# ray-project/xgboost_ray

Hardware: NVIDIA H100
Metric: boosting rounds/sec (higher is better)
Workload: dtype int64 fixed-point histograms (int32 shared-memory cells), f64 gain

## Files before the change

### xgboost_ray_b200/build.py

```python
import os
import subprocess
import sys
from concurrent.futures import ThreadPoolExecutor

HERE = os.path.dirname(os.path.abspath(__file__))
CSRC = os.path.join(HERE, "csrc")
OUT = os.path.join(HERE, "libb2hist.so")
OBJ_DIR = os.path.join(CSRC, "build")

NVCC = os.environ.get("NVCC", "/usr/local/cuda/bin/nvcc")
COMMON = ["-gencode", "arch=compute_90a,code=sm_90a", "-O3", "-lineinfo", "-std=c++17",
          "-Xcompiler", "-fPIC,-ffp-contract=off", "-ccbin", "/usr/bin/g++"]
SOURCES = {
    "hist_kernel.cu": [],
    "hist_tma_kernel.cu": [],
    "split_kernel.cu": ["--fmad=false"],
    "partition_kernel.cu": ["--fmad=false"],
    "control_kernel.cu": ["--fmad=false"],
    "objective_kernel.cu": ["--fmad=false"],
    "sketch.cu": ["--fmad=false"],
    "auc_kernel.cu": ["--fmad=false"],
    "p2p_exchange.cu": [],
    "shap_kernel.cu": [],
    "engine.cu": [],
}


def _stale(target, deps):
    if not os.path.exists(target):
        return True
    t = os.path.getmtime(target)
    return any(os.path.getmtime(d) > t for d in deps)


def build(force=False, verbose=False):
    os.makedirs(OBJ_DIR, exist_ok=True)
    headers = [os.path.join(CSRC, "common.cuh"), os.path.join(CSRC, "hist_common.cuh"), os.path.join(CSRC, "sampling.cuh"), os.path.join(CSRC, "p2p.cuh"), os.path.join(HERE, "..", "include", "b2hist.h"), __file__]
    jobs = []
    objs = []
    for src, extra in SOURCES.items():
        sp = os.path.join(CSRC, src)
        op = os.path.join(OBJ_DIR, src.replace(".cu", ".o"))
        objs.append(op)
        if force or _stale(op, [sp] + headers):
            jobs.append([NVCC] + COMMON + extra + ["-c", sp, "-o", op])

    def run(cmd):
        if verbose:
            print(" ".join(cmd), flush=True)
        r = subprocess.run(cmd, capture_output=True, text=True)
        if r.returncode != 0:
            raise RuntimeError("nvcc failed:\n%s\n%s\n%s" % (" ".join(cmd), r.stdout, r.stderr))
        return r

    with ThreadPoolExecutor(max_workers=6) as ex:
        list(ex.map(run, jobs))
    if force or jobs or _stale(OUT, objs):
        run([NVCC, "-shared", "-o", OUT] + objs + ["-ldl", "-ccbin", "/usr/bin/g++"])
    return OUT


if __name__ == "__main__":
    print(build(force="--force" in sys.argv, verbose=True))
```

### xgboost_ray_b200/csrc/common.cuh

```cuda
#pragma once
#include <cuda_runtime.h>
#include <stdint.h>

#define B2_GROUP_SLOTS 32
#define B2_BINS 256
#define B2_MISSING_BIN 255
#define B2_PLANE_ELEMS (B2_BINS * B2_GROUP_SLOTS)
#define B2_GROUP_ELEMS (2 * B2_PLANE_ELEMS)

struct B2HistWork {
  int32_t seg_begin;
  int32_t seg_count;
  int32_t hist_index;
  int32_t chunk_begin;
};

#define B2_HIST_MAX_TYPES 8
struct B2HistPlan {
  int32_t n_types;
  int32_t cta_begin[B2_HIST_MAX_TYPES + 1];
  int32_t narrow_w;
};

struct B2SplitWork {
  int32_t seg_begin, seg_count;
  int32_t feature;
  int32_t split_bin;
  int32_t default_left;
  int32_t has_missing;
  int32_t chunk_begin;
  int32_t is_cat;
  uint32_t cat_bits[8];
};

struct B2SplitCand {
  float loss_chg;
  int32_t feature;
  int32_t bin;
  int32_t default_left;
  int64_t left_g, left_h;
  uint32_t order;
  int32_t is_cat;
  uint32_t cat_bits[8];
};

struct B2EvalNode {
  int64_t sum_g, sum_h;
  int32_t hist_index;
  float root_gain;
};

struct B2TreeNodeDev {
  int32_t left, right;
  int32_t feature;
  float cond;
  float value;
  int32_t default_left;
  int32_t cat_slot;
  int32_t pad;
};

#define B2_SHAP_MAX_PATH 16
#define B2_PATH_MISSING_OK 1u
#define B2_PATH_HAS_HI 2u
#define B2_PATH_OUTSIDE_OK 4u
struct B2PathElem {
  int32_t feature;
  int32_t cat_slot;
  float lo, hi;
  uint32_t flags;
  uint32_t pad;
  double zero_fraction;
};
struct B2PathInfo {
  int32_t elem_begin;
  int32_t len;
  int32_t cls;
  int32_t pad;
  double value;
};

__device__ __forceinline__ int b2_tree_step(const B2TreeNodeDev& nd, float v, float missing, int missing_is_nan,
                                            const uint32_t* __restrict__ cat_table) {
  const bool miss = isnan(v) || (!missing_is_nan && v == missing);
  if (miss) return nd.default_left ? nd.left : nd.right;
  if (nd.cat_slot >= 0) {
    bool in_set = false;
    if (v >= 0.0f && v < 256.0f) { const int c = (int)v; in_set = (cat_table[(size_t)nd.cat_slot * 8 + (c >> 5)] >> (c & 31)) & 1u; }
    return in_set ? nd.right : nd.left;
  }
  return v < nd.cond ? nd.left : nd.right;
}

__device__ __forceinline__ int b2_tree_leaf(const B2TreeNodeDev* __restrict__ tn, const float* __restrict__ x, float missing,
                                            int missing_is_nan, const uint32_t* __restrict__ cat_table, float* leaf_value) {
  int nid = 0;
  B2TreeNodeDev nd = tn[0];
  while (nd.feature >= 0) {
    nid = b2_tree_step(nd, x[nd.feature], missing, missing_is_nan, cat_table);
    nd = tn[nid];
  }
  *leaf_value = nd.value;
  return nid;
}

struct B2LevelCtl {
  int32_t n_nodes;
  int32_t n_split;
  int32_t part_chunks;
  int32_t hist_n_work;
  int32_t hist_total_chunks;
  int32_t hist_chunk_rows;
  int32_t n_pairs;
  int32_t leaf_base_next;
};
struct B2NodeSeg { int32_t nid, begin, count, buf; };
struct B2LeafDev { int32_t nid, buf, begin, count; };
struct B2SegWork {
  int32_t seg_begin, seg_count, id, chunk_begin;
  int32_t buf, pad0, pad1, pad2;
};
struct B2TreeDev {
  int32_t *left, *right, *parent, *feature, *split_bin, *default_left, *split_type;
  uint32_t* cat_bits;
  float* loss_chg;
  long long *sum_g, *sum_h;
  float *leaf_weight, *leaf_value;
  int32_t* n_nodes;
};
struct B2CtlParams { double mcw, lambda, alpha, max_delta_step; float gamma, eta; };

struct B2ColSample {
  const uint8_t* level_mask;
  const uint32_t* fwq;
  double bynode;
  int32_t n_level;
  int32_t n_features;
  uint32_t seed, tree;
};

#define B2_P2P_MAX_WORLD 8
enum { kSlotHist = 0, kSlotCand = 1, kSlotAbsmax = 2, kSlotLeaf = 3, kSlotClose = 4, kP2PSlots = 5 };
struct B2P2P {
  long long* build[B2_P2P_MAX_WORLD];
  B2SplitCand* cands[B2_P2P_MAX_WORLD];
  long long* misc[B2_P2P_MAX_WORLD];
  uint32_t* flags[B2_P2P_MAX_WORLD];
  uint32_t* epoch;
  uint32_t* done;
  uint32_t* err;
  const uint32_t* abort_flag;
  int32_t world, rank;
  int32_t cand_cap, misc_stride;
  long long spin_limit;
};

struct B2TrainParamDev {
  double min_child_weight, lambda, alpha;
  double inv_scale_g, inv_scale_h;
  double max_delta_step;
  int32_t max_cat_to_onehot, max_cat_threshold;
};

#ifdef __CUDACC__
__device__ __forceinline__ double b2_thr_l1(double g, double a) {
  if (g > a) return __dadd_rn(g, -a);
  if (g < -a) return __dadd_rn(g, a);
  return 0.0;
}
__device__ __forceinline__ double b2_calc_weight(double G, double H, double mcw, double lambda, double alpha, double mds) {
  if (H < mcw || H <= 0.0) return 0.0;
  const double t = (alpha == 0.0) ? G : b2_thr_l1(G, alpha);
  double dw = __ddiv_rn(-t, __dadd_rn(H, lambda));
  if (mds != 0.0 && fabs(dw) > mds) dw = copysign(mds, dw);
  return dw;
}
__device__ __forceinline__ double b2_calc_gain(double G, double H, double mcw, double lambda, double alpha, double mds) {
  if (H < mcw || H <= 0.0) return 0.0;
  if (mds == 0.0) {
    const double t = (alpha == 0.0) ? G : b2_thr_l1(G, alpha);
    return __ddiv_rn(__dmul_rn(t, t), __dadd_rn(H, lambda));
  }
  const double w = b2_calc_weight(G, H, mcw, lambda, alpha, mds);
  const double ret = -__dadd_rn(__dmul_rn(__dmul_rn(2.0, G), w), __dmul_rn(__dadd_rn(H, lambda), __dmul_rn(w, w)));
  return alpha == 0.0 ? ret : __dadd_rn(ret, __dmul_rn(alpha, fabs(w)));
}
#endif
```

### xgboost_ray_b200/csrc/control_kernel.cu

```cuda
#include <string.h>

#include <cub/block/block_scan.cuh>

#include "common.cuh"
#include "p2p.cuh"

namespace b2 {

constexpr int kCtlThreads = 1024;
constexpr int kPartChunkRows = 2048;
constexpr int kSplitChunkRows = 8192;

__device__ __forceinline__ double c_calc_gain(double G, double H, const B2CtlParams& p) {
  return b2_calc_gain(G, H, p.mcw, p.lambda, p.alpha, p.max_delta_step);
}
__device__ __forceinline__ float c_calc_weight(double G, double H, const B2CtlParams& p) {
  return __double2float_rn(b2_calc_weight(G, H, p.mcw, p.lambda, p.alpha, p.max_delta_step));
}

struct TileScan {
  typedef cub::BlockScan<int, kCtlThreads> Scan;
  Scan::TempStorage* tmp;
  int carry;
  __device__ TileScan(Scan::TempStorage* t) : tmp(t), carry(0) {}
  __device__ int step(int v) {
    int ex, total;
    Scan(*tmp).ExclusiveSum(v, ex, total);
    __syncthreads();
    int r = carry + ex;
    carry += total;
    return r;
  }
};

__global__ void __launch_bounds__(kCtlThreads)
decide_kernel(B2LevelCtl* __restrict__ ctl_cur, B2LevelCtl* __restrict__ ctl_nxt, const B2NodeSeg* __restrict__ seg_cur,
              B2NodeSeg* __restrict__ seg_nxt, const B2EvalNode* __restrict__ ev_cur, B2EvalNode* __restrict__ ev_nxt,
              const B2SplitCand* __restrict__ cands, int cands_per_node, int cand_ranks, int cand_rank_stride, int can_split,
              B2TreeDev tree,
              B2SplitWork* __restrict__ split_work, int32_t* __restrict__ pair_parent_hist, B2LeafDev* __restrict__ leaves,
              int32_t* __restrict__ n_leaves, const uint8_t* __restrict__ has_missing, const int32_t* __restrict__ qexp,
              int qbits, B2CtlParams p, int32_t* __restrict__ part_counters, const B2SplitCand* __restrict__ local_cands,
              int use_p2p, B2P2P pp) {
  __shared__ typename TileScan::Scan::TempStorage tmp;
  __shared__ int s_node_base, s_leaf_base;
  const int n = ctl_cur->n_nodes;
  if (part_counters) for (int i = threadIdx.x; i < 2 * n; i += kCtlThreads) part_counters[i] = 0;
  if (use_p2p && can_split) {
    constexpr int kWords = sizeof(B2SplitCand) / 8;
    static_assert(sizeof(B2SplitCand) % 8 == 0, "candidates are copied as 64-bit words");
    const uint32_t epoch = p2p_next_epoch(pp, kSlotCand);
    const int total = n * cands_per_node * kWords;
    for (int w = 0; w < pp.world; ++w) {
      long long* dst = reinterpret_cast<long long*>(pp.cands[w] + (size_t)pp.rank * pp.cand_cap);
      for (int t = threadIdx.x; t < total; t += kCtlThreads) st_volatile_u64(dst + t, reinterpret_cast<const long long*>(local_cands)[t]);
    }
    __syncthreads();
    p2p_signal(pp, kSlotCand, epoch);
    p2p_wait(pp, kSlotCand, epoch);
    p2p_finish_single(pp, kSlotCand, epoch);
  }
  const double inv_sg = ldexp(1.0, qexp[0] - qbits), inv_sh = ldexp(1.0, qexp[1] - qbits);
  if (threadIdx.x == 0) { s_node_base = *tree.n_nodes; s_leaf_base = *n_leaves; }
  __syncthreads();
  TileScan scan_split(&tmp), scan_leaf(&tmp), scan_chunks(&tmp);
  for (int base = 0; base < n; base += kCtlThreads) {
    const int i = base + threadIdx.x;
    const bool in = i < n;
    B2SplitCand best; best.feature = -1; best.loss_chg = 0.f; best.order = 0xffffffffu; best.bin = 0; best.default_left = 0;
    best.left_g = 0; best.left_h = 0; best.is_cat = 0;
    B2EvalNode nd; nd.sum_g = 0; nd.sum_h = 0; nd.hist_index = 0; nd.root_gain = 0.f;
    B2NodeSeg sg; sg.nid = 0; sg.begin = 0; sg.count = 0; sg.buf = 0;
    bool expand = false;
    if (in) {
      nd = ev_cur[i]; sg = seg_cur[i];
      if (can_split) {
        for (int w = 0; w < cand_ranks; ++w)
          for (int g = 0; g < cands_per_node; ++g) {
            B2SplitCand c;
            if (use_p2p) {
              constexpr int kW = sizeof(B2SplitCand) / 8;
              const long long* src = reinterpret_cast<const long long*>(cands + (size_t)w * cand_rank_stride + (size_t)i * cands_per_node + g);
#pragma unroll
              for (int t = 0; t < kW; ++t) reinterpret_cast<unsigned long long*>(&c)[t] = ld_volatile_u64(src + t);
            } else c = cands[(size_t)w * cand_rank_stride + (size_t)i * cands_per_node + g];
            if (c.feature < 0) continue;
            if (best.feature < 0 || c.loss_chg > best.loss_chg || (c.loss_chg == best.loss_chg && c.order < best.order)) best = c;
          }
        if (best.feature >= 0)
          expand = best.loss_chg > 1e-6f && best.left_h != 0 && (nd.sum_h - best.left_h) != 0 && !(best.loss_chg < p.gamma);
      }
    }
    const int rank = scan_split.step(expand ? 1 : 0);
    const int lrank = scan_leaf.step((in && !expand) ? 1 : 0);
    const int chunks = expand ? (sg.count + kSplitChunkRows - 1) / kSplitChunkRows : 0;
    const int chunk_begin = scan_chunks.step(chunks);
    if (in && !expand) {
      B2LeafDev lf; lf.nid = sg.nid; lf.buf = sg.buf; lf.begin = sg.begin; lf.count = sg.count;
      leaves[s_leaf_base + lrank] = lf;
    }
    if (expand) {
      const int l = s_node_base + 2 * rank, r = l + 1;
      const int nid = sg.nid;
      tree.left[nid] = l; tree.right[nid] = r; tree.feature[nid] = best.feature; tree.split_bin[nid] = best.bin;
      tree.default_left[nid] = best.default_left; tree.loss_chg[nid] = best.loss_chg;
      tree.split_type[nid] = best.is_cat;
      if (best.is_cat) {
#pragma unroll
        for (int w8 = 0; w8 < 8; ++w8) tree.cat_bits[(size_t)nid * 8 + w8] = best.cat_bits[w8];
      }
      tree.left[l] = -1; tree.right[l] = -1; tree.feature[l] = -1; tree.parent[l] = nid;
      tree.left[r] = -1; tree.right[r] = -1; tree.feature[r] = -1; tree.parent[r] = nid;
      const long long lg = best.left_g, lh = best.left_h, rg = nd.sum_g - lg, rh = nd.sum_h - lh;
      tree.sum_g[l] = lg; tree.sum_h[l] = lh; tree.sum_g[r] = rg; tree.sum_h[r] = rh;
      B2SplitWork sw;
      sw.seg_begin = sg.begin; sw.seg_count = sg.count; sw.feature = best.feature; sw.split_bin = best.bin;
      sw.default_left = best.default_left; sw.has_missing = has_missing[best.feature]; sw.chunk_begin = chunk_begin;
      sw.is_cat = best.is_cat;
#pragma unroll
      for (int w8 = 0; w8 < 8; ++w8) sw.cat_bits[w8] = best.is_cat ? best.cat_bits[w8] : 0u;
      split_work[rank] = sw;
      pair_parent_hist[rank] = nd.hist_index;
      const double GL = __dmul_rn(__ll2double_rn(lg), inv_sg), HL = __dmul_rn(__ll2double_rn(lh), inv_sh);
      const double GR = __dmul_rn(__ll2double_rn(rg), inv_sg), HR = __dmul_rn(__ll2double_rn(rh), inv_sh);
      B2EvalNode el, er;
      el.sum_g = lg; el.sum_h = lh; el.hist_index = -1; el.root_gain = __double2float_rn(c_calc_gain(GL, HL, p));
      er.sum_g = rg; er.sum_h = rh; er.hist_index = -1; er.root_gain = __double2float_rn(c_calc_gain(GR, HR, p));
      ev_nxt[2 * rank] = el; ev_nxt[2 * rank + 1] = er;
      B2NodeSeg sl, sr;
      sl.nid = l; sl.buf = sg.buf ^ 1; sl.begin = sg.begin; sl.count = 0;
      sr.nid = r; sr.buf = sg.buf ^ 1; sr.begin = sg.begin; sr.count = sg.count;
      seg_nxt[2 * rank] = sl; seg_nxt[2 * rank + 1] = sr;
    }
  }
  __syncthreads();
  if (threadIdx.x == 0) {
    const int n_split = scan_split.carry;
    ctl_cur->n_split = n_split; ctl_cur->part_chunks = scan_chunks.carry;
    ctl_cur->leaf_base_next = s_leaf_base + scan_leaf.carry;
    ctl_nxt->n_nodes = 2 * n_split; ctl_nxt->n_split = 0; ctl_nxt->part_chunks = 0;
    ctl_nxt->hist_n_work = 0; ctl_nxt->hist_total_chunks = 0; ctl_nxt->n_pairs = 0;
    *tree.n_nodes = s_node_base + 2 * n_split;
    *n_leaves = s_leaf_base + scan_leaf.carry;
  }
}

__global__ void __launch_bounds__(kCtlThreads)
finalize_level_kernel(const B2LevelCtl* __restrict__ ctl_cur, B2LevelCtl* __restrict__ ctl_nxt, B2NodeSeg* __restrict__ seg_nxt,
                      B2EvalNode* __restrict__ ev_nxt, const B2SplitWork* __restrict__ split_work,
                      const int32_t* __restrict__ counters, const int32_t* __restrict__ pair_parent_hist,
                      B2HistWork* __restrict__ hist_work, int32_t* __restrict__ triples, int max_pairs, int need_hist,
                      int n_streams, int window_rows, int chunk_rows_override, long long* __restrict__ stat_rows) {
  __shared__ typename TileScan::Scan::TempStorage tmp;
  __shared__ long long s_rows;
  __shared__ int s_chunk_rows;
  const int ns = ctl_cur->n_split;
  if (threadIdx.x == 0) s_rows = 0;
  __syncthreads();
  long long my_rows = 0;
  for (int j = threadIdx.x; j < ns; j += kCtlThreads) {
    const B2SplitWork sw = split_work[j];
    const int cl = counters[2 * j];
    B2NodeSeg sl = seg_nxt[2 * j], sr = seg_nxt[2 * j + 1];
    sl.begin = sw.seg_begin; sl.count = cl;
    sr.begin = sw.seg_begin + cl; sr.count = sw.seg_count - cl;
    seg_nxt[2 * j] = sl; seg_nxt[2 * j + 1] = sr;
    if (need_hist) {
      const bool build_left = ev_nxt[2 * j].sum_h < ev_nxt[2 * j + 1].sum_h;
      my_rows += build_left ? sl.count : sr.count;
    }
  }
  if (need_hist) {
    atomicAdd((unsigned long long*)&s_rows, (unsigned long long)my_rows);
    __syncthreads();
    if (threadIdx.x == 0) {
      int c = chunk_rows_override;
      if (c <= 0) {
        const long long per_stream = s_rows / n_streams;
        const long long target = per_stream >= 16384 ? per_stream / 4 : per_stream;
        c = 512;
        while (c < target && c < 8192) c <<= 1;
      }
      if (c > window_rows) c = window_rows;
      s_chunk_rows = c;
      if (stat_rows) *stat_rows = s_rows;
    }
    __syncthreads();
    const int chunk_rows = s_chunk_rows;
    TileScan scan(&tmp);
    for (int base = 0; base < ns; base += kCtlThreads) {
      const int j = base + threadIdx.x;
      int chunks = 0, begin = 0, count = 0;
      if (j < ns) {
        const bool build_left = ev_nxt[2 * j].sum_h < ev_nxt[2 * j + 1].sum_h;
        const int b = build_left ? 2 * j : 2 * j + 1, s = b ^ 1;
        begin = seg_nxt[b].begin; count = seg_nxt[b].count;
        chunks = (count + chunk_rows - 1) / chunk_rows;
        ev_nxt[b].hist_index = j; ev_nxt[s].hist_index = max_pairs + j;
        triples[3 * j] = pair_parent_hist[j]; triples[3 * j + 1] = j; triples[3 * j + 2] = max_pairs + j;
      }
      const int cb = scan.step(chunks);
      if (j < ns) { B2HistWork w; w.seg_begin = begin; w.seg_count = count; w.hist_index = j; w.chunk_begin = cb; hist_work[j] = w; }
    }
    __syncthreads();
    if (threadIdx.x == 0) {
      ctl_nxt->hist_n_work = ns; ctl_nxt->hist_total_chunks = scan.carry; ctl_nxt->hist_chunk_rows = chunk_rows;
      ctl_nxt->n_pairs = ns;
    }
  }
}

__global__ void __launch_bounds__(kCtlThreads)
leaf_plan_kernel(const B2LeafDev* __restrict__ leaves, const int32_t* __restrict__ n_leaves, B2SegWork* __restrict__ work,
                 B2LevelCtl* __restrict__ leaf_ctl) {
  __shared__ typename TileScan::Scan::TempStorage tmp;
  const int n = *n_leaves;
  TileScan scan(&tmp);
  for (int base = 0; base < n; base += kCtlThreads) {
    const int i = base + threadIdx.x;
    int chunks = 0; B2LeafDev lf; lf.nid = 0; lf.buf = 0; lf.begin = 0; lf.count = 0;
    if (i < n) { lf = leaves[i]; chunks = (lf.count + kPartChunkRows - 1) / kPartChunkRows; }
    const int cb = scan.step(chunks);
    if (i < n) {
      B2SegWork w; w.seg_begin = lf.begin; w.seg_count = lf.count; w.id = i; w.chunk_begin = cb; w.buf = lf.buf;
      w.pad0 = lf.nid == 0 ? 1 : 0;
      w.pad1 = w.pad2 = 0; work[i] = w;
    }
  }
  __syncthreads();
  if (threadIdx.x == 0) { leaf_ctl->hist_n_work = n; leaf_ctl->hist_total_chunks = scan.carry; }
}

__global__ void leaf_values_kernel(const B2LeafDev* __restrict__ leaves, const int32_t* __restrict__ n_leaves,
                                   const long long* __restrict__ sums, const int32_t* __restrict__ qexp, int leaf_bits,
                                   B2CtlParams p, float* __restrict__ leaf_value, B2TreeDev tree) {
  const int n = *n_leaves;
  const double kg = ldexp(1.0, leaf_bits - qexp[0]), kh = ldexp(1.0, leaf_bits - qexp[1]);
  for (int i = blockIdx.x * blockDim.x + threadIdx.x; i < n; i += gridDim.x * blockDim.x) {
    const double G = __ddiv_rn(__ll2double_rn(sums[2 * i]), kg), H = __ddiv_rn(__ll2double_rn(sums[2 * i + 1]), kh);
    const float w = c_calc_weight(G, H, p);
    const float v = __fmul_rn(w, p.eta);
    leaf_value[i] = v;
    tree.leaf_weight[leaves[i].nid] = w;
    tree.leaf_value[leaves[i].nid] = v;
  }
}

__global__ void tree_init_kernel(B2TreeDev tree, B2LevelCtl* ctl0, B2NodeSeg* seg0, B2EvalNode* ev0, int32_t* n_leaves,
                                 int n_rows, B2HistWork* hist_work0) {
  if (threadIdx.x == 0 && blockIdx.x == 0) {
    B2HistWork hw; hw.seg_begin = 0; hw.seg_count = n_rows; hw.hist_index = 0; hw.chunk_begin = 0; hist_work0[0] = hw;
    ctl0->leaf_base_next = 0;
    *tree.n_nodes = 1; *n_leaves = 0;
    tree.left[0] = -1; tree.right[0] = -1; tree.parent[0] = -1; tree.feature[0] = -1;
    ctl0->n_nodes = 1; ctl0->n_split = 0; ctl0->part_chunks = 0; ctl0->hist_n_work = 0; ctl0->hist_total_chunks = 0;
    ctl0->n_pairs = 0;
    B2NodeSeg s; s.nid = 0; s.buf = 0; s.begin = 0; s.count = n_rows; seg0[0] = s;
    B2EvalNode e; e.sum_g = 0; e.sum_h = 0; e.hist_index = 0; e.root_gain = 0.f; ev0[0] = e;
  }
}
__global__ void root_record_kernel(B2TreeDev tree, const B2EvalNode* ev0) {
  if (threadIdx.x == 0 && blockIdx.x == 0) { tree.sum_g[0] = ev0[0].sum_g; tree.sum_h[0] = ev0[0].sum_h; }
}

}

extern "C" {
int b2_launch_decide(B2LevelCtl* ctl_cur, B2LevelCtl* ctl_nxt, const B2NodeSeg* seg_cur, B2NodeSeg* seg_nxt,
                     const B2EvalNode* ev_cur, B2EvalNode* ev_nxt, const B2SplitCand* cands, int cands_per_node, int cand_ranks,
                     int cand_rank_stride, int can_split, B2TreeDev tree, B2SplitWork* split_work, int32_t* pair_parent_hist, B2LeafDev* leaves, int32_t* n_leaves,
                     const uint8_t* has_missing, const int32_t* qexp, int qbits, B2CtlParams p, int32_t* part_counters,
                     const B2SplitCand* local_cands, const void* p2p, cudaStream_t s) {
  B2P2P pp;
  if (p2p) pp = *reinterpret_cast<const B2P2P*>(p2p); else memset(&pp, 0, sizeof(pp));
  b2::decide_kernel<<<1, b2::kCtlThreads, 0, s>>>(ctl_cur, ctl_nxt, seg_cur, seg_nxt, ev_cur, ev_nxt, cands, cands_per_node,
                                                 cand_ranks, cand_rank_stride, can_split, tree, split_work, pair_parent_hist, leaves, n_leaves, has_missing, qexp, qbits, p,
                                                 part_counters, local_cands, p2p ? 1 : 0, pp);
  return (int)cudaGetLastError();
}
int b2_launch_finalize_level(const B2LevelCtl* ctl_cur, B2LevelCtl* ctl_nxt, B2NodeSeg* seg_nxt, B2EvalNode* ev_nxt,
                             const B2SplitWork* split_work, const int32_t* counters, const int32_t* pair_parent_hist,
                             B2HistWork* hist_work, int32_t* triples, int max_pairs, int need_hist, int n_streams,
                             int window_rows, int chunk_rows_override, long long* stat_rows, cudaStream_t s) {
  b2::finalize_level_kernel<<<1, b2::kCtlThreads, 0, s>>>(ctl_cur, ctl_nxt, seg_nxt, ev_nxt, split_work, counters,
                                                         pair_parent_hist, hist_work, triples, max_pairs, need_hist, n_streams,
                                                         window_rows, chunk_rows_override, stat_rows);
  return (int)cudaGetLastError();
}
int b2_launch_leaf_plan(const B2LeafDev* leaves, const int32_t* n_leaves, B2SegWork* work, B2LevelCtl* leaf_ctl, cudaStream_t s) {
  b2::leaf_plan_kernel<<<1, b2::kCtlThreads, 0, s>>>(leaves, n_leaves, work, leaf_ctl);
  return (int)cudaGetLastError();
}
int b2_launch_leaf_values(const B2LeafDev* leaves, const int32_t* n_leaves, const long long* sums, const int32_t* qexp,
                          int leaf_bits, B2CtlParams p, float* leaf_value, B2TreeDev tree, cudaStream_t s) {
  b2::leaf_values_kernel<<<8, 256, 0, s>>>(leaves, n_leaves, sums, qexp, leaf_bits, p, leaf_value, tree);
  return (int)cudaGetLastError();
}
int b2_launch_tree_init(B2TreeDev tree, B2LevelCtl* ctl0, B2NodeSeg* seg0, B2EvalNode* ev0, int32_t* n_leaves, int n_rows,
                        B2HistWork* hist_work0, cudaStream_t s) {
  b2::tree_init_kernel<<<1, 32, 0, s>>>(tree, ctl0, seg0, ev0, n_leaves, n_rows, hist_work0);
  return (int)cudaGetLastError();
}
int b2_launch_root_record(B2TreeDev tree, const B2EvalNode* ev0, cudaStream_t s) {
  b2::root_record_kernel<<<1, 32, 0, s>>>(tree, ev0);
  return (int)cudaGetLastError();
}
}
```

### xgboost_ray_b200/csrc/engine.cu

```cuda
#include <cuda_runtime.h>
#include <dlfcn.h>
#include <errno.h>
#include <sys/types.h>
#include <sys/uio.h>
#include <math.h>
#include <stdarg.h>
#include <stdio.h>
#include <stdlib.h>
#include <string.h>

#include <algorithm>
#include <atomic>
#include <chrono>
#include <map>
#include <mutex>
#include <set>
#include <string>
#include <thread>
#include <vector>

#include "../../include/b2hist.h"
#include "common.cuh"
#include "sampling.cuh"

extern "C" {
int b2_launch_hist(const uint8_t*, int, const int2*, const int32_t*, const B2HistWork*, int, int, int, int, int, long long*,
                   const B2LevelCtl*, int, int, int, int, cudaStream_t);
int b2_make_bins_tensor_map(void*, const uint8_t*, int64_t, int, int);
int b2_launch_hist_tma(const uint8_t*, int, const void*, const int2*, const int32_t*, const B2HistWork*, int, int, int, int, int, long long*,
                       const B2LevelCtl*, int, int, int64_t, int, cudaStream_t);
int b2_launch_hist_subtract(const long long*, long long*, const int32_t*, int, int64_t, const B2LevelCtl*, cudaStream_t);
int b2_launch_eval_splits(const long long*, int, const B2EvalNode*, int, const int32_t*, const int32_t*, const int32_t*,
                          const uint8_t*, const uint8_t*, const int32_t*, int, B2TrainParamDev, B2SplitCand*, int, const B2LevelCtl*,
                          int, int, B2ColSample, const B2NodeSeg*, cudaStream_t);
int b2_launch_subsample(float2*, int64_t, uint32_t, uint32_t, uint32_t, double, int, cudaStream_t);
int b2_p2p_flag_words(int);
int b2_launch_p2p_reduce_subtract(const void*, const long long*, long long*, const int32_t*, const B2LevelCtl*, int, int, int64_t, int,
                                  cudaStream_t);
int b2_launch_p2p_quant_exponent(const void*, const uint32_t*, int32_t*, cudaStream_t);
int b2_launch_p2p_leaf_sums(const void*, const int32_t*, long long*, cudaStream_t);
int b2_hist_variant();
int b2_launch_p2p_close(const void*, cudaStream_t);
int b2_launch_gather_interleaved_rows(const void*, float*, int, cudaStream_t);
int b2_launch_final_assign(const uint8_t*, int64_t, const int32_t*, const B2SplitWork*, const B2LevelCtl*, int, const float2*,
                           const int32_t*, int, long long*, uint16_t*, int, int, cudaStream_t);
int b2_launch_margin_update(float*, int, int, const uint16_t*, const float*, int64_t, int, cudaStream_t);
int b2_gradient_fused_max_classes();
int b2_launch_sum_fixed(const float2*, int64_t, const int32_t*, int, long long*, int, cudaStream_t);
int b2_cat_ctas();
int b2_launch_eval_cat_splits(const long long*, int, const B2EvalNode*, int, const int32_t*, int, const int32_t*, const int32_t*,
                              const int32_t*, int, B2TrainParamDev, B2SplitCand*, int, int, const B2LevelCtl*, int, int,
                              B2ColSample, const B2NodeSeg*, cudaStream_t);
int b2_launch_cat_stats(const float*, int64_t, int, float, const int32_t*, int, int32_t*, int, cudaStream_t);
int b2_launch_root_totals(const long long*, int, B2EvalNode*, const int32_t*, int, B2TrainParamDev, int, cudaStream_t);
int b2_part_chunk_rows();
int b2_split_chunk_rows();
int b2_launch_partition(const uint8_t*, int64_t, const int32_t*, int32_t*, const B2SplitWork*, const B2LevelCtl*, int, int32_t*,
                        int, int, cudaStream_t);
int b2_launch_leaf_sums(const float2*, const int32_t*, const int32_t*, const void*, const B2LevelCtl*, int, const int32_t*, int,
                        long long*, uint16_t*, int, cudaStream_t);
int b2_launch_pred_update(float*, int, int, const int32_t*, const int32_t*, const void*, const B2LevelCtl*, int, const float*, int,
                          cudaStream_t);
int b2_launch_decide(B2LevelCtl*, B2LevelCtl*, const B2NodeSeg*, B2NodeSeg*, const B2EvalNode*, B2EvalNode*, const B2SplitCand*,
                     int, int, int, int, B2TreeDev, B2SplitWork*, int32_t*, B2LeafDev*, int32_t*, const uint8_t*, const int32_t*, int,
                     B2CtlParams, int32_t*, const B2SplitCand*, const void*, cudaStream_t);
int b2_launch_finalize_level(const B2LevelCtl*, B2LevelCtl*, B2NodeSeg*, B2EvalNode*, const B2SplitWork*, const int32_t*,
                             const int32_t*, B2HistWork*, int32_t*, int, int, int, int, int, long long*, cudaStream_t);
int b2_launch_leaf_plan(const B2LeafDev*, const int32_t*, B2SegWork*, B2LevelCtl*, cudaStream_t);
int b2_launch_leaf_values(const B2LeafDev*, const int32_t*, const long long*, const int32_t*, int, B2CtlParams, float*, B2TreeDev,
                          cudaStream_t);
int b2_launch_tree_init(B2TreeDev, B2LevelCtl*, B2NodeSeg*, B2EvalNode*, int32_t*, int, B2HistWork*, cudaStream_t);
int b2_launch_root_record(B2TreeDev, const B2EvalNode*, cudaStream_t);
int b2_launch_iota(int32_t*, int64_t, cudaStream_t);
int b2_launch_gradient(int, int, const float*, const float*, const float*, int64_t, float, float, float2*, uint32_t*, uint32_t*, int,
                       cudaStream_t);
int b2_launch_label_check(int, const float*, int64_t, uint32_t*, int, cudaStream_t);
int b2_launch_pack_custom(const float*, const float*, int, int64_t, float2*, int, cudaStream_t);
int b2_launch_absmax(const float2*, int64_t, uint32_t*, int, cudaStream_t);
int b2_launch_quant_exponent(const uint32_t*, int32_t*, cudaStream_t);
int b2_launch_quantize(const float2*, int64_t, const int32_t*, int, int2*, int, cudaStream_t);
int b2_launch_metric(int, int, int, float, const float*, const float*, const float*, int64_t, double*, int, cudaStream_t);
int b2_launch_predict(const float*, int64_t, int, float, const B2TreeNodeDev*, const int32_t*, const uint32_t*, int, int, int, int,
                      float*, int, cudaStream_t);
int b2_launch_fill(float*, int64_t, float, int, cudaStream_t);
size_t b2_shap_contribs_smem(int, int, int);
int b2_launch_shap_contribs(const float*, int64_t, int64_t, int, float, const B2PathElem*, const B2PathInfo*, int, int,
                            const uint32_t*, int, const double*, const float*, float, double*, int, size_t, float*, int, cudaStream_t);
int b2_launch_shap_interactions(const float*, int64_t, int64_t, int, float, const B2PathElem*, const B2PathInfo*, int, int,
                                const uint32_t*, int, const double*, const float*, float, double*, float*, int, cudaStream_t);
int b2_launch_leaf_index(const float*, int64_t, int64_t, int, float, const B2TreeNodeDev*, const int32_t*, const uint32_t*, int, int,
                         float*, int, cudaStream_t);
size_t b2_auc_temp_bytes(int64_t);
int b2_auc_binary(const float*, const float*, const float*, int64_t, void*, size_t, double*, int, cudaStream_t);
int b2_launch_transform(int, int, float*, int64_t, int, cudaStream_t);
int b2_extract_batch();
int b2_launch_extract_keys(const float*, int64_t, int, int, int, float, uint32_t*, int64_t, int, cudaStream_t);
size_t b2_sort_temp_bytes(int64_t);
int b2_sketch_column(const uint32_t*, const int32_t*, uint32_t*, int32_t*, long long*, int64_t, long long, void*, size_t, int32_t*,
                     int32_t*, float*, long long*, int32_t*, long long*, int, float*, int32_t*, float*, int32_t*, int, cudaStream_t);
int b2_launch_weight_absmax(const float*, int64_t, uint32_t*, int, cudaStream_t);
int b2_launch_weight_quantize(const float*, int64_t, int64_t, const uint32_t*, int32_t*, int, cudaStream_t);
int b2_launch_bin(const float*, int64_t, int, float, const int32_t*, const float*, const int32_t*, const uint8_t*, int, uint8_t*,
                  uint8_t*, int64_t, int, cudaStream_t);
}

namespace {

thread_local std::string g_last_error;
struct B2Error { std::string msg; };
[[noreturn]] void fail(const char* fmt, ...) {
  char buf[1024];
  va_list ap; va_start(ap, fmt); vsnprintf(buf, sizeof(buf), fmt, ap); va_end(ap);
  throw B2Error{buf};
}
#define CUDA_CHECK(expr)                                                                       \
  do {                                                                                         \
    cudaError_t e_ = (expr);                                                                   \
    if (e_ != cudaSuccess) fail("CUDA error %s at %s:%d: %s", cudaGetErrorName(e_), __FILE__, __LINE__, cudaGetErrorString(e_)); \
  } while (0)
#define LAUNCH_CHECK(expr)                                                                     \
  do {                                                                                         \
    int e_ = (expr);                                                                           \
    if (e_ != 0) fail("kernel launch failed (%s) at %s:%d", cudaGetErrorString((cudaError_t)e_), __FILE__, __LINE__); \
  } while (0)
#define API_BEGIN try {
#define API_END                                            \
  }                                                        \
  catch (const B2Error& e) { g_last_error = e.msg; return -1; } \
  catch (const std::exception& e) { g_last_error = e.what(); return -1; } \
  return 0;

struct Ctx {
  int device = -1;
  cudaStream_t stream = nullptr;
  int num_sms = 0;
};
std::mutex g_ctx_mu;
std::map<int, Ctx*> g_ctx;
Ctx* get_ctx(int device) {
  std::lock_guard<std::mutex> lk(g_ctx_mu);
  auto it = g_ctx.find(device);
  if (it != g_ctx.end()) { CUDA_CHECK(cudaSetDevice(device)); return it->second; }
  int n = 0;
  cudaError_t e = cudaGetDeviceCount(&n);
  if (e != cudaSuccess || n == 0) fail("no CUDA device available (%s): libb2hist has no CPU fallback", cudaGetErrorString(e));
  if (device < 0 || device >= n) fail("invalid device %d (have %d)", device, n);
  CUDA_CHECK(cudaSetDevice(device));
  Ctx* c = new Ctx();
  c->device = device;
  CUDA_CHECK(cudaStreamCreateWithFlags(&c->stream, cudaStreamNonBlocking));
  cudaDeviceProp prop;
  CUDA_CHECK(cudaGetDeviceProperties(&prop, device));
  if (prop.major != 9 || prop.minor != 0)
    fail("device %d is sm_%d%d; this engine is built for sm_90a (H100) only", device, prop.major, prop.minor);
  c->num_sms = prop.multiProcessorCount;
  g_ctx[device] = c;
  return c;
}

struct DevPool {
  std::mutex mu;
  std::multimap<size_t, void*> free_blocks;
  size_t cached = 0;
};
DevPool g_dev_pool[64];
size_t pool_cap_bytes() {
  static size_t cap = 0;
  if (!cap) { const char* e = getenv("B2_POOL_MAX_GB"); double gb = e ? atof(e) : 24.0; cap = (size_t)(gb < 0 ? 0 : gb * 1e9) + 1; }
  return cap;
}
void pool_trim(DevPool& pool, size_t keep) {
  while (pool.cached > keep && !pool.free_blocks.empty()) {
    auto it = std::prev(pool.free_blocks.end());
    cudaFree(it->second);
    pool.cached -= it->first;
    pool.free_blocks.erase(it);
  }
}
void* pool_alloc(size_t bytes, size_t* got, int* dev_out) {
  int dev = 0; cudaGetDevice(&dev);
  if (dev < 0 || dev >= 64) dev = 0;
  *dev_out = dev;
  bytes = (bytes + 511) & ~(size_t)511;
  DevPool& pool = g_dev_pool[dev];
  {
    std::lock_guard<std::mutex> lk(pool.mu);
    auto it = pool.free_blocks.lower_bound(bytes);
    if (it != pool.free_blocks.end() && it->first <= bytes + bytes / 4 + ((size_t)1 << 20)) {
      void* p = it->second; *got = it->first;
      pool.cached -= it->first;
      pool.free_blocks.erase(it);
      return p;
    }
  }
  void* p = nullptr;
  cudaError_t e = cudaMalloc(&p, bytes);
  if (e != cudaSuccess) {
    cudaGetLastError();
    { std::lock_guard<std::mutex> lk(pool.mu); pool_trim(pool, 0); }
    e = cudaMalloc(&p, bytes);
  }
  if (e != cudaSuccess) { cudaGetLastError(); fail("cudaMalloc of %zu bytes failed: %s", bytes, cudaGetErrorString(e)); }
  *got = bytes;
  return p;
}
void pool_free(void* p, size_t bytes, int dev) {
  if (!p) return;
  if (dev < 0 || dev >= 64) dev = 0;
  DevPool& pool = g_dev_pool[dev];
  std::lock_guard<std::mutex> lk(pool.mu);
  if (bytes > pool_cap_bytes()) { cudaFree(p); return; }
  pool.free_blocks.emplace(bytes, p);
  pool.cached += bytes;
  if (pool.cached > pool_cap_bytes()) pool_trim(pool, pool_cap_bytes() / 2);
}

template <typename T>
struct DevBuf {
  T* p = nullptr;
  size_t cap = 0;
  size_t block_bytes = 0;
  int dev = 0;
  void ensure(size_t n) {
    if (n <= cap) return;
    release();
    size_t got = 0;
    p = (T*)pool_alloc(n * sizeof(T), &got, &dev);
    block_bytes = got;
    cap = n;
  }
  void release() { if (p) pool_free(p, block_bytes, dev); p = nullptr; cap = 0; block_bytes = 0; }
  ~DevBuf() { release(); }
};

struct PinnedPool {
  static constexpr int kWorkers = 16, kSlots = 2;
  static constexpr size_t kSlice = (size_t)8 << 20;
  void* buf[kWorkers][kSlots] = {};
  cudaStream_t stream[kWorkers] = {};
  cudaEvent_t done[kWorkers][kSlots] = {};
  bool ready = false;
  std::mutex mu;
  int n_init = 0;
  void init(int n) {
    for (int w = n_init; w < n; ++w) {
      CUDA_CHECK(cudaStreamCreateWithFlags(&stream[w], cudaStreamNonBlocking));
      for (int k = 0; k < kSlots; ++k) {
        CUDA_CHECK(cudaMallocHost(&buf[w][k], kSlice));
        CUDA_CHECK(cudaEventCreateWithFlags(&done[w][k], cudaEventDisableTiming));
      }
      n_init = w + 1;
    }
  }
};
std::map<int, PinnedPool*> g_pools;

struct UploadSource {
  const void* src = nullptr;
  long long pid = 0;
  uint64_t remote_addr = 0;
  size_t row_bytes = 0, row_stride = 0;
};
bool fetch_slice(const UploadSource& u, void* dst, size_t off, size_t len, std::string* err) {
  if (u.pid == 0) { memcpy(dst, (const char*)u.src + off, len); return true; }
  if (u.row_stride == u.row_bytes) {
    size_t done = 0;
    while (done < len) {
      struct iovec l = {(char*)dst + done, len - done}, r = {(void*)(uintptr_t)(u.remote_addr + off + done), len - done};
      const ssize_t got = process_vm_readv((pid_t)u.pid, &l, 1, &r, 1, 0);
      if (got <= 0) { if (err) *err = std::string("process_vm_readv: ") + strerror(errno); return false; }
      done += (size_t)got;
    }
    return true;
  }
  constexpr size_t kSpan = (size_t)4 << 20;
  static thread_local std::vector<char> scratch;
  if (scratch.size() < kSpan + u.row_stride) scratch.resize(kSpan + u.row_stride);
  const size_t rows_per_batch = std::max<size_t>(1, kSpan / u.row_stride);
  size_t done = 0;
  while (done < len) {
    const size_t pos = off + done, row0 = pos / u.row_bytes;
    const size_t last_byte = std::min(off + len, (row0 + rows_per_batch) * u.row_bytes) - 1;
    const size_t row1 = last_byte / u.row_bytes;
    const size_t span = (row1 - row0) * u.row_stride + u.row_bytes;
    size_t got_total = 0;
    while (got_total < span) {
      struct iovec l = {scratch.data() + got_total, span - got_total};
      struct iovec r = {(void*)(uintptr_t)(u.remote_addr + row0 * u.row_stride + got_total), span - got_total};
      const ssize_t got = process_vm_readv((pid_t)u.pid, &l, 1, &r, 1, 0);
      if (got <= 0) { if (err) *err = std::string("process_vm_readv: ") + strerror(errno); return false; }
      got_total += (size_t)got;
    }
    for (size_t row = row0; row <= row1; ++row) {
      const size_t b0 = std::max(pos, row * u.row_bytes), b1 = std::min(off + len, (row + 1) * u.row_bytes);
      memcpy((char*)dst + (b0 - off), scratch.data() + (row - row0) * u.row_stride + (b0 - row * u.row_bytes), b1 - b0);
    }
    done = std::min(off + len, (row1 + 1) * u.row_bytes) - off;
  }
  return true;
}

void upload_pipelined(Ctx* ctx, void* dst, const UploadSource& u, size_t bytes);
void upload_pipelined(Ctx* ctx, void* dst, const void* src, size_t bytes) {
  UploadSource u; u.src = src;
  upload_pipelined(ctx, dst, u, bytes);
}
void upload_pipelined(Ctx* ctx, void* dst, const UploadSource& u, size_t bytes) {
  const void* src = u.src;
  if (u.pid == 0 && bytes < ((size_t)64 << 20)) {
    if (bytes) CUDA_CHECK(cudaMemcpyAsync(dst, src, bytes, cudaMemcpyHostToDevice, ctx->stream));
    CUDA_CHECK(cudaStreamSynchronize(ctx->stream));
    return;
  }
  PinnedPool* pool;
  {
    std::lock_guard<std::mutex> lk(g_ctx_mu);
    PinnedPool*& p = g_pools[ctx->device];
    if (!p) p = new PinnedPool();
    pool = p;
  }
  std::lock_guard<std::mutex> lk(pool->mu);
  CUDA_CHECK(cudaStreamSynchronize(ctx->stream));
  const size_t n_slices = (bytes + PinnedPool::kSlice - 1) / PinnedPool::kSlice;
  static int n_workers = 0;
  if (n_workers == 0) {
    const char* e = getenv("B2_UPLOAD_WORKERS");
    n_workers = e ? atoi(e) : 8;
    if (n_workers < 1) n_workers = 1;
    if (n_workers > PinnedPool::kWorkers) n_workers = PinnedPool::kWorkers;
  }
  const int W = n_workers;
  pool->init(W);
  std::atomic<int> failed{0};
  std::mutex err_mu; std::string fetch_err;
  auto worker = [&](int w) {
    if (cudaSetDevice(ctx->device) != cudaSuccess) { failed = 1; return; }
    int use = 0;
    for (size_t i = w; i < n_slices; i += W, ++use) {
      const int k = use % PinnedPool::kSlots;
      const size_t off = i * PinnedPool::kSlice, len = std::min(PinnedPool::kSlice, bytes - off);
      if (use >= PinnedPool::kSlots && cudaEventSynchronize(pool->done[w][k]) != cudaSuccess) { failed = 1; return; }
      std::string e;
      if (!fetch_slice(u, pool->buf[w][k], off, len, &e)) { std::lock_guard<std::mutex> lk(err_mu); fetch_err = e; failed = 2; return; }
      if (cudaMemcpyAsync((char*)dst + off, pool->buf[w][k], len, cudaMemcpyHostToDevice, pool->stream[w]) != cudaSuccess ||
          cudaEventRecord(pool->done[w][k], pool->stream[w]) != cudaSuccess) { failed = 1; return; }
    }
    if (cudaStreamSynchronize(pool->stream[w]) != cudaSuccess) failed = 1;
  };
  std::vector<std::thread> th;
  for (int w = 0; w < W; ++w) th.emplace_back(worker, w);
  for (auto& t : th) t.join();
  if (failed.load() == 2) fail("reading the shard out of the driver process failed: %s", fetch_err.c_str());
  if (failed.load()) fail("pipelined host->device upload failed: %s", cudaGetErrorString(cudaGetLastError()));
}

typedef struct ncclComm* ncclComm_t;
typedef struct { char internal[128]; } ncclUniqueId;
enum { kNcclSum = 0, kNcclMax = 2, kNcclMin = 3 };
enum { kNcclUint8 = 1, kNcclInt32 = 2, kNcclUint32 = 3, kNcclInt64 = 4, kNcclUint64 = 5, kNcclFloat32 = 7, kNcclFloat64 = 8 };
struct NcclApi {
  void* lib = nullptr;
  int (*GetUniqueId)(ncclUniqueId*) = nullptr;
  int (*CommInitRank)(ncclComm_t*, int, ncclUniqueId, int) = nullptr;
  int (*AllReduce)(const void*, void*, size_t, int, int, ncclComm_t, cudaStream_t) = nullptr;
  int (*AllGather)(const void*, void*, size_t, int, ncclComm_t, cudaStream_t) = nullptr;
  int (*ReduceScatter)(const void*, void*, size_t, int, int, ncclComm_t, cudaStream_t) = nullptr;
  int (*CommAbort)(ncclComm_t) = nullptr;
  int (*CommDestroy)(ncclComm_t) = nullptr;
  const char* (*GetErrorString)(int) = nullptr;
};
NcclApi* nccl() {
  static NcclApi api;
  static std::once_flag once;
  static std::string err;
  std::call_once(once, [] {
// ... 55 lines not shown
  int F = 0;
  float missing = NAN;
  DevBuf<float> raw;
  bool has_raw = false;
  DevBuf<uint8_t> bins;
  alignas(64) unsigned char tmap_tile[128];
  bool has_tmap = false;
  DevBuf<uint8_t> bins_col;
  int64_t col_stride = 0;
  bool quantized = false;
  int n_groups = 0, row_stride = 0, max_bin = 0;
  int narrow_w = 0;
  std::vector<int32_t> group_first, group_size, feat_byte;
  std::vector<int32_t> cut_ptrs;
  std::vector<float> cut_vals, min_vals;
  std::vector<uint8_t> has_missing;
  std::vector<int32_t> nbins;
  std::vector<uint8_t> is_cat;
  std::vector<int32_t> cat_feats;
  DevBuf<int32_t> d_group_first, d_group_size, d_feat_byte, d_cut_ptrs, d_nbins, d_cat_feats;
  DevBuf<float> d_cut_vals;
  DevBuf<uint8_t> d_has_missing, d_is_cat;
  bool any_cat() const { return !cat_feats.empty(); }
  DevBuf<float> label, weight, base_margin;
  int64_t n_label = 0, n_weight = 0, n_base_margin = 0;
  std::vector<uint32_t> fwq;
  DevBuf<uint32_t> d_fwq;
};

int g_hist_narrow = -1;
void setup_groups(Matrix* m) {
  const int F = m->F;
  if (g_hist_narrow < 0) { const char* e = getenv("B2_HIST_NARROW"); g_hist_narrow = (e && atoi(e) != 0) ? 1 : 0; }
  const int narrow_on = g_hist_narrow;
  m->n_groups = (F + B2_GROUP_SLOTS - 1) / B2_GROUP_SLOTS;
  if (m->n_groups < 1) m->n_groups = 1;
  m->row_stride = m->n_groups * B2_GROUP_SLOTS;
  m->group_first.assign(m->n_groups, 0);
  m->group_size.assign(m->n_groups, 0);
  m->feat_byte.assign(F, 0);
  m->narrow_w = 0;
  const int r = F % B2_GROUP_SLOTS;
  const bool v4_layout = b2_hist_variant() == 4 && F > 96 && F <= 112;
  const bool narrow = (narrow_on || v4_layout) && r > 0 && r <= 16;
  if (narrow) { m->narrow_w = 1; while (m->narrow_w < r) m->narrow_w <<= 1; }
  const int base = F / m->n_groups, rem = F % m->n_groups;
  int f = 0;
  for (int g = 0; g < m->n_groups; ++g) {
    const int sz = narrow ? (g + 1 < m->n_groups ? B2_GROUP_SLOTS : r) : base + (g < rem ? 1 : 0);
    m->group_first[g] = f; m->group_size[g] = sz;
    for (int s = 0; s < sz; ++s) m->feat_byte[f + s] = g * B2_GROUP_SLOTS + s;
    f += sz;
  }
}

template <typename T>
void upload(DevBuf<T>& d, const std::vector<T>& h, cudaStream_t s) {
  d.ensure(h.size() ? h.size() : 1);
  if (!h.empty()) CUDA_CHECK(cudaMemcpyAsync(d.p, h.data(), h.size() * sizeof(T), cudaMemcpyHostToDevice, s));
}

void upload_cuts(Matrix* m) {
  cudaStream_t s = m->ctx->stream;
  m->nbins.resize(m->F);
  for (int f = 0; f < m->F; ++f) m->nbins[f] = m->cut_ptrs[f + 1] - m->cut_ptrs[f];
  upload(m->d_group_first, m->group_first, s); upload(m->d_group_size, m->group_size, s);
  upload(m->d_feat_byte, m->feat_byte, s); upload(m->d_cut_ptrs, m->cut_ptrs, s);
  upload(m->d_cut_vals, m->cut_vals, s); upload(m->d_nbins, m->nbins, s);
  upload(m->d_has_missing, m->has_missing, s);
  if (m->is_cat.empty()) m->is_cat.assign(m->F, 0);
  upload(m->d_is_cat, m->is_cat, s); upload(m->d_cat_feats, m->cat_feats, s);
  CUDA_CHECK(cudaStreamSynchronize(s));
}

void make_cuts(Matrix* m, Comm* comm, int max_bin) {
  Ctx* ctx = m->ctx; cudaStream_t s = ctx->stream;
  if (max_bin < 2 || max_bin > 256) fail("max_bin must be in [2, 256] (uint8 bin matrix), got %d", max_bin);
  if (!m->has_raw) fail("matrix has no raw data to sketch");
  const int world = comm ? comm->world : 1, rank = comm ? comm->rank : 0;
  DevBuf<long long> d_cnt; d_cnt.ensure(2);
  long long h_cnt[2] = {m->n, m->n};
  if (world > 1) {
    CUDA_CHECK(cudaMemcpyAsync(d_cnt.p, h_cnt, sizeof(h_cnt), cudaMemcpyHostToDevice, s));
    allreduce(comm, d_cnt.p, 1, kNcclInt64, kNcclMax, s);
    allreduce(comm, d_cnt.p + 1, 1, kNcclInt64, kNcclSum, s);
    CUDA_CHECK(cudaMemcpyAsync(h_cnt, d_cnt.p, sizeof(h_cnt), cudaMemcpyDeviceToHost, s));
    CUDA_CHECK(cudaStreamSynchronize(s));
  }
  const int64_t n_pad = h_cnt[0], n_total = n_pad * world; const long long n_global = h_cnt[1];
  const int B = b2_extract_batch(); const int F = m->F;
  DevBuf<uint32_t> keys_local, keys_all, keys_sorted;
  DevBuf<int32_t> flags, idx, m_scratch; DevBuf<float> uval; DevBuf<long long> rmin, nvalid;
  DevBuf<int32_t> d_tab;
  DevBuf<uint8_t> temp;
  const size_t nt = (size_t)std::max<int64_t>(n_total, 1);
  keys_local.ensure((size_t)std::max<int64_t>(n_pad, 1) * B);
  if (world > 1) keys_all.ensure(nt);
  keys_sorted.ensure(nt); flags.ensure(nt); idx.ensure(nt); uval.ensure(nt); rmin.ensure(nt); m_scratch.ensure(1); nvalid.ensure(2);
  DevBuf<int32_t> wq_local, wq_all, wq_sorted; DevBuf<long long> wpre; DevBuf<uint32_t> d_wmax;
  const int32_t* wq = nullptr;
  {
    long long h_has[1] = {m->n_weight > 0 ? 1 : 0};
    if (world > 1) {
      CUDA_CHECK(cudaMemcpyAsync(d_cnt.p, h_has, sizeof(h_has), cudaMemcpyHostToDevice, s));
      allreduce(comm, d_cnt.p, 1, kNcclInt64, kNcclMax, s);
      CUDA_CHECK(cudaMemcpyAsync(h_has, d_cnt.p, sizeof(h_has), cudaMemcpyDeviceToHost, s));
      CUDA_CHECK(cudaStreamSynchronize(s));
    }
    if (h_has[0]) {
      if (m->n_weight != m->n) fail("sample weights are set on some ranks only (this rank has %lld for %lld rows)", (long long)m->n_weight, (long long)m->n);
      d_wmax.ensure(2);
      CUDA_CHECK(cudaMemsetAsync(d_wmax.p, 0, 2 * sizeof(uint32_t), s));
      LAUNCH_CHECK(b2_launch_weight_absmax(m->weight.p, m->n, d_wmax.p, ctx->num_sms, s));
      allreduce(comm, d_wmax.p, 2, kNcclUint32, kNcclMax, s);
      uint32_t h_w[2];
      CUDA_CHECK(cudaMemcpyAsync(h_w, d_wmax.p, sizeof(h_w), cudaMemcpyDeviceToHost, s));
      CUDA_CHECK(cudaStreamSynchronize(s));
      if (h_w[1]) fail("sample weights must be finite and non-negative");
      wq_local.ensure((size_t)std::max<int64_t>(n_pad, 1));
      LAUNCH_CHECK(b2_launch_weight_quantize(m->weight.p, m->n, n_pad, d_wmax.p, wq_local.p, ctx->num_sms, s));
      wq = wq_local.p;
      if (world > 1) {
        wq_all.ensure(nt);
        NCCL_CHECK(nccl()->AllGather(wq_local.p, wq_all.p, (size_t)n_pad, kNcclInt32, comm->comm, s));
        wq = wq_all.p;
      }
      wq_sorted.ensure(nt); wpre.ensure(nt);
    }
  }
  const size_t temp_bytes = b2_sort_temp_bytes(n_total > 0 ? n_total : 1);
  temp.ensure(temp_bytes ? temp_bytes : 1);
  const size_t tab_n = (size_t)F * 256 + 3 * (size_t)F;
  d_tab.ensure(tab_n);
  CUDA_CHECK(cudaMemsetAsync(d_tab.p, 0, tab_n * sizeof(int32_t), s));
  float* d_cuts = (float*)d_tab.p; int32_t* d_ncuts = d_tab.p + (size_t)F * 256;
  float* d_mins = (float*)(d_ncuts + F); int32_t* d_hasmiss = d_ncuts + 2 * (size_t)F;
  if (m->is_cat.empty()) m->is_cat.assign(F, 0);
  for (int f0 = 0; f0 < F; f0 += B) {
    const int nf = std::min(B, F - f0);
    bool any_numeric = false;
    for (int j = 0; j < nf; ++j) any_numeric = any_numeric || !m->is_cat[f0 + j];
    if (!any_numeric) continue;
    LAUNCH_CHECK(b2_launch_extract_keys(m->raw.p, m->n, F, f0, nf, m->missing, keys_local.p, n_pad, ctx->num_sms, s));
    for (int j = 0; j < nf; ++j) {
      const int f = f0 + j;
      if (m->is_cat[f]) continue;
      const uint32_t* kin = keys_local.p + (size_t)j * n_pad;
      if (world > 1) {
        NCCL_CHECK(nccl()->AllGather(kin, keys_all.p, (size_t)n_pad, kNcclUint32, comm->comm, s));
        kin = keys_all.p;
        if (f % world != rank) continue;
      }
      LAUNCH_CHECK(b2_sketch_column(kin, wq, keys_sorted.p, wq_sorted.p, wpre.p, n_total, n_global, temp.p, temp_bytes, flags.p, idx.p, uval.p, rmin.p,
                                    m_scratch.p, nvalid.p, max_bin, d_cuts + (size_t)f * 256, d_ncuts + f, d_mins + f,
                                    d_hasmiss + f, ctx->num_sms, s));
    }
  }
  allreduce(comm, d_tab.p, tab_n, kNcclInt32, kNcclSum, s);
  std::vector<int32_t> h_tab(tab_n);
  CUDA_CHECK(cudaMemcpyAsync(h_tab.data(), d_tab.p, tab_n * sizeof(int32_t), cudaMemcpyDeviceToHost, s));
  const int n_cat = (int)m->cat_feats.size();
  std::vector<int32_t> h_cat((size_t)std::max(n_cat, 1) * 3, 0);
  DevBuf<int32_t> d_cat, d_catf;
  if (n_cat > 0) {
    for (int i = 0; i < n_cat; ++i) { h_cat[i * 3] = -1; h_cat[i * 3 + 1] = 0; h_cat[i * 3 + 2] = 0; }
    d_cat.ensure((size_t)n_cat * 3); d_catf.ensure((size_t)n_cat);
    CUDA_CHECK(cudaMemcpyAsync(d_cat.p, h_cat.data(), (size_t)n_cat * 3 * sizeof(int32_t), cudaMemcpyHostToDevice, s));
    CUDA_CHECK(cudaMemcpyAsync(d_catf.p, m->cat_feats.data(), (size_t)n_cat * sizeof(int32_t), cudaMemcpyHostToDevice, s));
    LAUNCH_CHECK(b2_launch_cat_stats(m->raw.p, m->n, F, m->missing, d_catf.p, n_cat, d_cat.p, ctx->num_sms, s));
    allreduce(comm, d_cat.p, (size_t)n_cat * 3, kNcclInt32, kNcclMax, s);
    CUDA_CHECK(cudaMemcpyAsync(h_cat.data(), d_cat.p, (size_t)n_cat * 3 * sizeof(int32_t), cudaMemcpyDeviceToHost, s));
  }
  CUDA_CHECK(cudaStreamSynchronize(s));
  for (int i = 0; i < n_cat; ++i) {
    const int f = m->cat_feats[i], mx = h_cat[i * 3], miss = h_cat[i * 3 + 1];
    if (h_cat[i * 3 + 2] || (miss && mx > 254))
      fail("categorical feature %d: category codes must be integers in [0, %d]%s", f, miss ? 254 : 255,
           miss ? " (the feature has missing values; bin 255 is the missing sentinel)" : "");
    int32_t* t = h_tab.data();
    float* cuts_f = (float*)t + (size_t)f * 256;
    const int nc = mx < 0 ? 1 : mx + 1;
    for (int k = 0; k < nc; ++k) cuts_f[k] = (float)k;
    t[(size_t)F * 256 + f] = nc;
    ((float*)(t + (size_t)F * 256 + F))[f] = -1e-5f;
    t[(size_t)F * 256 + 2 * (size_t)F + f] = miss;
  }
  const float* h_cuts = (const float*)h_tab.data(); const int32_t* h_nc = h_tab.data() + (size_t)F * 256;
  const float* h_mins = (const float*)(h_nc + F); const int32_t* h_hm = h_nc + 2 * (size_t)F;
  m->cut_ptrs.assign(F + 1, 0);
  m->cut_vals.clear(); m->min_vals.assign(h_mins, h_mins + F); m->has_missing.assign(F, 0);
  for (int f = 0; f < F; ++f) {
    if (h_nc[f] < 1 || h_nc[f] > 256) fail("sketch produced %d cuts for feature %d", h_nc[f], f);
    m->cut_ptrs[f + 1] = m->cut_ptrs[f] + h_nc[f];
    m->cut_vals.insert(m->cut_vals.end(), h_cuts + (size_t)f * 256, h_cuts + (size_t)f * 256 + h_nc[f]);
    m->has_missing[f] = h_hm[f] ? 1 : 0;
  }
  m->max_bin = max_bin;
}

void bin_matrix(Matrix* m) {
  Ctx* ctx = m->ctx; cudaStream_t s = ctx->stream;
  setup_groups(m);
  upload_cuts(m);
  m->bins.ensure((size_t)std::max<int64_t>(m->n, 1) * m->row_stride);
  CUDA_CHECK(cudaMemsetAsync(m->bins.p, 0, (size_t)std::max<int64_t>(m->n, 1) * m->row_stride, s));
  m->col_stride = (std::max<int64_t>(m->n, 1) + 127) & ~(int64_t)127;
  m->bins_col.ensure((size_t)m->col_stride * m->F);
  LAUNCH_CHECK(b2_launch_bin(m->raw.p, m->n, m->F, m->missing, m->d_cut_ptrs.p, m->d_cut_vals.p, m->d_feat_byte.p,
                             m->any_cat() ? m->d_is_cat.p : nullptr, m->row_stride, m->bins.p, m->bins_col.p, m->col_stride,
                             ctx->num_sms, s));
  CUDA_CHECK(cudaStreamSynchronize(s));
  m->has_tmap = b2_make_bins_tensor_map(m->tmap_tile, m->bins.p, m->n, m->row_stride, 64) == 0;
  m->quantized = true;
}

enum { kObjSquaredError = 0, kObjLogistic = 1, kObjSoftprob = 2, kObjRegLogistic = 3, kObjLogitRaw = 4, kObjSquaredLog = 5,
       kObjPseudoHuber = 6, kObjPoisson = 7, kObjGamma = 8, kObjTweedie = 9 };
bool obj_log_link(int o) { return o == kObjPoisson || o == kObjGamma || o == kObjTweedie; }
bool obj_sigmoid(int o) { return o == kObjLogistic || o == kObjRegLogistic; }
bool obj_checks_finite(int o) { return o >= kObjSquaredLog; }
struct Params {
  int objective = kObjSquaredError;
  std::string objective_name = "reg:squarederror";
  int num_class = 1;
  int num_parallel_tree = 1;
  int max_depth = 6;
  float eta = 0.3f, gamma = 0.0f, min_child_weight = 1.0f, lambda = 1.0f, alpha = 0.0f, base_score = 0.5f;
  int qbits = 18;
  int hist_chunk_rows = 0;
  int profile = 1;
  int num_feature = 0;
  int device = 0;
  int max_cat_to_onehot = 4, max_cat_threshold = 64;
  float scale_pos_weight = 1.0f, max_delta_step = 0.0f;
  bool max_delta_step_set = false;
  float huber_slope = 1.0f;
  float tweedie_variance_power = 1.5f;
  float subsample = 1.0f, colsample_bytree = 1.0f, colsample_bylevel = 1.0f, colsample_bynode = 1.0f;
  int seed = 0;
  bool base_score_set = false;
  bool use_cols() const { return colsample_bytree < 1.0f || colsample_bylevel < 1.0f || colsample_bynode < 1.0f; }
};

struct TreeHost {
  std::vector<int32_t> left, right, parent, feature, split_bin;
  std::vector<float> cond, value, base_weight, loss_chg;
  std::vector<double> sum_hess;
  std::vector<uint8_t> default_left;
  std::vector<uint8_t> split_type;
  std::vector<uint32_t> cat_bits;
  bool any_cat = false;
  int add(int par) {
    int id = (int)left.size();
    left.push_back(-1); right.push_back(-1); parent.push_back(par); feature.push_back(-1); split_bin.push_back(-1);
    cond.push_back(0.f); value.push_back(0.f); base_weight.push_back(0.f); loss_chg.push_back(0.f); sum_hess.push_back(0.0);
    default_left.push_back(0); split_type.push_back(0); cat_bits.insert(cat_bits.end(), 8, 0u);
    return id;
  }
  int size() const { return (int)left.size(); }
};


struct Timers {
  double hist_ms = 0, round_ms = 0;
  double shap_ms = 0;
  long long shap_rows = 0;
  double phase_ms[8] = {0, 0, 0, 0, 0, 0, 0, 0};
  long long hist_launches = 0, hist_rows = 0, kernel_launches = 0, rounds = 0;
  double hist_bytes = 0, allreduce_bytes = 0;
  void reset() { *this = Timers(); }
};

struct EvalCache { DevBuf<float> margin; int n_trees_applied = 0; int64_t n = 0; uint64_t margin_version = 0; };

struct Booster : HandleBase {
  Ctx* ctx = nullptr;
  Params p;
  Matrix* train = nullptr;
  int n_features = 0;
  Comm* comm = nullptr;
  std::vector<TreeHost> trees;
  std::atomic<bool> cancel{false};
  DevBuf<B2TreeNodeDev> d_nodes; DevBuf<int32_t> d_tree_offset; int d_trees_synced = 0;
  std::vector<B2TreeNodeDev> h_nodes; std::vector<int32_t> h_tree_offset;
  DevBuf<uint32_t> d_cat_table; std::vector<uint32_t> h_cat_table;
  DevBuf<B2PathElem> d_path_elems; DevBuf<B2PathInfo> d_paths; DevBuf<uint32_t> d_path_cats;
  std::vector<int32_t> tree_path_offset;
  std::vector<double> tree_expected;
  int paths_synced = -1;
  bool margin_ready = false;
  DevBuf<float> margin;
  DevBuf<float2> gh;
  DevBuf<float2> gh_round;
  DevBuf<int2> q;
  DevBuf<int32_t> ridx[2];
  DevBuf<long long> hist[2];
  template <typename T> struct View { T* p = nullptr; };
  DevBuf<uint8_t> xarena;
  size_t xoff_cands = 0, xoff_misc = 0, xoff_flags = 0, x_misc_stride = 0;
  View<long long> hist_build;
  View<B2SplitCand> d_cands_all;
  int shards = 1, log2_shards = 0, sp = 32, cpn = 1;
  int cpn_num = 1;
  DevBuf<uint32_t> t_cat;
  DevBuf<uint8_t> d_col_masks;
  struct P2PState {
    bool enabled = false, tried = false;
    B2P2P pp;
    DevBuf<uint32_t> words;
    uint32_t* flags = nullptr;
    long long* misc = nullptr;
    std::vector<void*> opened;
    int cand_cap = 0;
  } p2p;
  struct TreeGraph {
    cudaGraphExec_t exec = nullptr;
    std::vector<std::pair<cudaEvent_t, cudaEvent_t>> hist_ev;
    long long hist_launches = 0, kernel_launches = 0;
    double allreduce_bytes = 0;
  };
  std::map<int, TreeGraph> graphs;
  std::map<int, int> direct_trees;
  bool graph_failed = false;
  bool absmax_fused = false;
  bool labels_checked = false;
  DevBuf<uint32_t> d_grad_err;
  uint32_t* h_grad_err = nullptr;
  DevBuf<uint16_t> pos;
  size_t slice_elems = 0;
  size_t node_elems = 0;
  DevBuf<uint32_t> d_absmax; DevBuf<int32_t> d_qexp;
  int ctl_depth = 0;
  DevBuf<int32_t> t_i32;
  DevBuf<float> t_f32;
  DevBuf<long long> t_i64;
  DevBuf<B2LevelCtl> d_ctl;
  DevBuf<B2NodeSeg> d_seg[2]; DevBuf<B2EvalNode> d_ev[2];
  DevBuf<B2HistWork> d_hist_work; DevBuf<B2SplitWork> d_split_work; DevBuf<B2SegWork> d_seg_work;
  DevBuf<B2SplitCand> d_cands; DevBuf<int32_t> d_counters, d_triples, d_pair_parent;
  DevBuf<B2LeafDev> d_leaves;
  DevBuf<long long> d_leaf_sums; DevBuf<float> d_leaf_values; DevBuf<double> d_metric;
  std::vector<void*> staging;
  size_t staging_bytes = 0;
  DevBuf<float> d_custom_g, d_custom_h;
  std::map<uint64_t, EvalCache*> eval_cache;
  Timers t;
  std::vector<cudaEvent_t> ev_pool; size_t ev_used = 0;
  std::vector<std::pair<cudaEvent_t, cudaEvent_t>> hist_events;
  std::vector<std::pair<int, cudaEvent_t>> phase_marks;
  cudaEvent_t round_start = nullptr, round_stop = nullptr;
  ~Booster() {
    for (auto& kv : graphs) {
      if (kv.second.exec) cudaGraphExecDestroy(kv.second.exec);
      for (auto& pr : kv.second.hist_ev) { cudaEventDestroy(pr.first); cudaEventDestroy(pr.second); }
    }
    if (ctx) cudaStreamSynchronize(ctx->stream);
    for (void* q : p2p.opened) cudaIpcCloseMemHandle(q);
    for (auto e : ev_pool) cudaEventDestroy(e);
    if (round_start) cudaEventDestroy(round_start);
    if (round_stop) cudaEventDestroy(round_stop);
    for (auto& kv : eval_cache) delete kv.second;
    for (void* h : staging) cudaFreeHost(h);
    if (h_grad_err) cudaFreeHost(h_grad_err);
  }
};

cudaEvent_t get_event(Booster* b) {
  if (b->ev_used == b->ev_pool.size()) { cudaEvent_t e; CUDA_CHECK(cudaEventCreate(&e)); b->ev_pool.push_back(e); }
  return b->ev_pool[b->ev_used++];
}
void mark_phase(Booster* b, int phase) {
  if (b->p.profile < 2) return;
  cudaEvent_t e = get_event(b);
  CUDA_CHECK(cudaEventRecord(e, b->ctx->stream));
  b->phase_marks.push_back({phase, e});
}
void resolve_events(Booster* b) {
  for (size_t i = 1; i < b->phase_marks.size(); ++i) {
    float ms = 0.f;
    if (b->phase_marks[i].first >= 0 && cudaEventElapsedTime(&ms, b->phase_marks[i - 1].second, b->phase_marks[i].second) == cudaSuccess)
      b->t.phase_ms[b->phase_marks[i].first] += ms;
  }
  b->phase_marks.clear();
  for (auto& pr : b->hist_events) {
    float ms = 0.f;
    if (cudaEventElapsedTime(&ms, pr.first, pr.second) == cudaSuccess) b->t.hist_ms += ms;
  }
  b->hist_events.clear();
  b->ev_used = 0;
}

void parse_params(const char* text, Params* p, int* max_bin_out) {
  std::string s(text ? text : "");
  size_t pos = 0;
  while (pos < s.size()) {
    size_t nl = s.find('\n', pos);
    if (nl == std::string::npos) nl = s.size();
    std::string line = s.substr(pos, nl - pos);
    pos = nl + 1;
    size_t eq = line.find('=');
    if (eq == std::string::npos) continue;
    std::string k = line.substr(0, eq), v = line.substr(eq + 1);
    auto f = [&]() { return (float)atof(v.c_str()); };
    auto i = [&]() { return atoi(v.c_str()); };
    if (k == "objective") {
      p->objective_name = v;
      if (v == "reg:squarederror" || v == "reg:linear") p->objective = kObjSquaredError;
      else if (v == "binary:logistic") p->objective = kObjLogistic;
      else if (v == "multi:softprob" || v == "multi:softmax") p->objective = kObjSoftprob;
      else if (v == "reg:logistic") p->objective = kObjRegLogistic;
      else if (v == "binary:logitraw") p->objective = kObjLogitRaw;
      else if (v == "reg:squaredlogerror") p->objective = kObjSquaredLog;
      else if (v == "reg:pseudohubererror") p->objective = kObjPseudoHuber;
      else if (v == "count:poisson") p->objective = kObjPoisson;
      else if (v == "reg:gamma") p->objective = kObjGamma;
      else if (v == "reg:tweedie") p->objective = kObjTweedie;
      else fail("unsupported objective '%s' (supported: reg:squarederror, reg:logistic, binary:logistic, binary:logitraw, "
                "reg:squaredlogerror, reg:pseudohubererror, count:poisson, reg:gamma, reg:tweedie, multi:softprob, "
                "multi:softmax)", v.c_str());
    } else if (k == "num_class") p->num_class = i();
    else if (k == "num_parallel_tree") p->num_parallel_tree = i();
    else if (k == "max_depth") p->max_depth = i();
    else if (k == "eta" || k == "learning_rate") p->eta = f();
    else if (k == "gamma" || k == "min_split_loss") p->gamma = f();
    else if (k == "min_child_weight") p->min_child_weight = f();
    else if (k == "lambda" || k == "reg_lambda") p->lambda = f();
    else if (k == "alpha" || k == "reg_alpha") p->alpha = f();
    else if (k == "base_score") { p->base_score = f(); p->base_score_set = true; }
    else if (k == "hist_qbits") p->qbits = i();
    else if (k == "hist_chunk_rows") p->hist_chunk_rows = i();
    else if (k == "profile") p->profile = i();
    else if (k == "num_feature") p->num_feature = i();
    else if (k == "device") p->device = i();
    else if (k == "subsample") p->subsample = f();
    else if (k == "colsample_bytree") p->colsample_bytree = f();
    else if (k == "colsample_bylevel") p->colsample_bylevel = f();
    else if (k == "colsample_bynode") p->colsample_bynode = f();
    else if (k == "seed" || k == "random_state") p->seed = i();
    else if (k == "scale_pos_weight") p->scale_pos_weight = f();
    else if (k == "max_delta_step") { p->max_delta_step = f(); p->max_delta_step_set = true; }
    else if (k == "huber_slope") p->huber_slope = f();
    else if (k == "tweedie_variance_power") p->tweedie_variance_power = f();
    else if (k == "max_cat_to_onehot") p->max_cat_to_onehot = i();
    else if (k == "max_cat_threshold") p->max_cat_threshold = i();
    else if (k == "max_bin") { if (max_bin_out) *max_bin_out = i(); }
  }
  if (p->objective != kObjSoftprob) p->num_class = 1;
  if (p->objective == kObjSoftprob && p->num_class < 2) fail("multi:softprob needs num_class >= 2");
  if (p->max_depth < 1 || p->max_depth > 14) fail("max_depth must be in [1, 14], got %d", p->max_depth);
  if (p->num_parallel_tree < 1 || p->num_parallel_tree > 4096) fail("num_parallel_tree must be in [1, 4096], got %d", p->num_parallel_tree);
  if (p->qbits < 8 || p->qbits > 24) fail("hist_qbits must be in [8, 24], got %d", p->qbits);
  for (float v : {p->subsample, p->colsample_bytree, p->colsample_bylevel, p->colsample_bynode})
    if (!(v > 0.0f && v <= 1.0f)) fail("subsample / colsample_* must be in (0, 1], got %g", (double)v);
  if (p->max_cat_to_onehot < 1) fail("max_cat_to_onehot must be >= 1, got %d", p->max_cat_to_onehot);
  if (p->max_cat_threshold < 1) fail("max_cat_threshold must be >= 1, got %d", p->max_cat_threshold);
  if (p->objective == kObjPoisson) {
    if (!p->max_delta_step_set) p->max_delta_step = 0.7f;
    if (!(p->max_delta_step >= 0.0f)) fail("max_delta_step must be >= 0 for count:poisson, got %g", (double)p->max_delta_step);
  }
  if (p->objective == kObjPseudoHuber && !(p->huber_slope > 0.0f))
    fail("huber_slope must be > 0 for reg:pseudohubererror, got %g", (double)p->huber_slope);
  if (p->objective == kObjTweedie && !(p->tweedie_variance_power >= 1.0f && p->tweedie_variance_power < 2.0f))
    fail("tweedie_variance_power must be in [1, 2), got %g", (double)p->tweedie_variance_power);
  if (p->base_score_set) {
    if (p->objective == kObjRegLogistic && !(p->base_score > 0.0f && p->base_score < 1.0f))
      fail("base_score must be in (0, 1) for reg:logistic, got %g", (double)p->base_score);
    if (obj_log_link(p->objective) && !(p->base_score > 0.0f))
      fail("base_score must be > 0 for %s, got %g", p->objective_name.c_str(), (double)p->base_score);
  }
}

float objective_param(const Params& p) {
  if (p.objective == kObjPseudoHuber) return p.huber_slope;
  if (p.objective == kObjPoisson) return p.max_delta_step;
  if (p.objective == kObjTweedie) return p.tweedie_variance_power;
  return 0.0f;
}

float base_margin_value(const Params& p) {
  if (obj_sigmoid(p.objective)) return -logf(1.0f / p.base_score - 1.0f);
  if (obj_log_link(p.objective)) return logf(p.base_score);
  return p.base_score;
}

double h_thr_l1(double g, double a) { if (g > a) return g - a; if (g < -a) return g + a; return 0.0; }
float h_calc_weight(const Params& p, double G, double H) {
  if (H < (double)p.min_child_weight || H <= 0.0) return 0.0f;
  double t = p.alpha == 0.0f ? G : h_thr_l1(G, (double)p.alpha);
  double dw = -t / (H + (double)p.lambda);
  if (p.max_delta_step != 0.0f && fabs(dw) > (double)p.max_delta_step) dw = copysign((double)p.max_delta_step, dw);
  return (float)dw;
}

int window_rows_for(int qbits) {
  return 1 << (30 - qbits);
}

int pick_chunk_rows(Booster* b, int64_t rows) {
  if (b->p.hist_chunk_rows > 0) return b->p.hist_chunk_rows;
  const int n_streams = std::max(1, b->ctx->num_sms * 3 / b->train->n_groups);
  const int64_t per_stream = rows / n_streams;
  int64_t target = per_stream >= 16384 ? per_stream / 4 : per_stream;
  int c = 512;
  while (c < target && c < 8192) c <<= 1;
  const int w = window_rows_for(b->p.qbits);
  if (c > w) c = w;
  return c;
}

struct TreeLayout {
  size_t max_nodes, i32_count, f32_count, i64_count, bytes;
  size_t off_f32, off_i64, off_qexp, off_cat;
};
TreeLayout tree_layout(int max_depth) {
  TreeLayout L;
  L.max_nodes = ((size_t)1 << (max_depth + 1));
  L.i32_count = 7 * L.max_nodes + 2;
  L.f32_count = 3 * L.max_nodes;
  L.i64_count = 2 * L.max_nodes + (size_t)max_depth + 2;
  L.off_f32 = L.i32_count * 4;
  L.off_i64 = (L.off_f32 + L.f32_count * 4 + 7) & ~(size_t)7;
  L.off_qexp = L.off_i64 + L.i64_count * 8;
  L.off_cat = L.off_qexp + 16;
  L.bytes = L.off_cat + L.max_nodes * 8 * sizeof(uint32_t);
  return L;
}
B2TreeDev tree_dev(Booster* b) {
  const TreeLayout L = tree_layout(b->ctl_depth);
  B2TreeDev t;
  int32_t* i = b->t_i32.p; const size_t m = L.max_nodes;
  t.left = i; t.right = i + m; t.parent = i + 2 * m; t.feature = i + 3 * m; t.split_bin = i + 4 * m; t.default_left = i + 5 * m;
  t.split_type = i + 6 * m;
  t.n_nodes = i + 7 * m;
  t.cat_bits = b->t_cat.p;
  t.loss_chg = b->t_f32.p; t.leaf_weight = b->t_f32.p + m; t.leaf_value = b->t_f32.p + 2 * m;
  t.sum_g = b->t_i64.p; t.sum_h = b->t_i64.p + m;
  return t;
}

int p2p_timeout_seconds() {
  const char* e = getenv("B2_P2P_TIMEOUT_S");
  int v = e ? atoi(e) : 60;
  return v < 1 ? 1 : v;
}
void p2p_setup(Booster* b) {
  Booster::P2PState& st = b->p2p;
  if (st.tried || b->shards <= 1) return;
  st.tried = true;
  const char* env = getenv("B2_EXCHANGE");
  if (env && (strcmp(env, "nccl") == 0 || strcmp(env, "NCCL") == 0)) return;
  Comm* c = b->comm; cudaStream_t s = b->ctx->stream; const int W = c->world;
  if (W > B2_P2P_MAX_WORLD) return;
  const size_t misc_stride = b->x_misc_stride;
  const size_t n_flags = (size_t)b2_p2p_flag_words(W), n_words = 2 * (size_t)kP2PSlots + 2;
  st.words.ensure(n_words);
  CUDA_CHECK(cudaMemsetAsync(st.flags, 0, n_flags * sizeof(uint32_t), s));
  CUDA_CHECK(cudaMemsetAsync(st.words.p, 0, n_words * sizeof(uint32_t), s));
  CUDA_CHECK(cudaMemsetAsync(st.misc, 0, (size_t)W * misc_stride * sizeof(long long), s));
  cudaIpcMemHandle_t mine; int ok = 1;
  if (cudaIpcGetMemHandle(&mine, b->xarena.p) != cudaSuccess) { ok = 0; cudaGetLastError(); memset(&mine, 0, sizeof(mine)); }
  DevBuf<uint8_t> d_mine, d_all; d_mine.ensure(sizeof(mine)); d_all.ensure(sizeof(mine) * (size_t)W);
  CUDA_CHECK(cudaMemcpyAsync(d_mine.p, &mine, sizeof(mine), cudaMemcpyHostToDevice, s));
  NCCL_CHECK(nccl()->AllGather(d_mine.p, d_all.p, sizeof(mine), kNcclUint8, c->comm, s));
  std::vector<cudaIpcMemHandle_t> all((size_t)W);
  CUDA_CHECK(cudaMemcpyAsync(all.data(), d_all.p, sizeof(mine) * (size_t)W, cudaMemcpyDeviceToHost, s));
  CUDA_CHECK(cudaStreamSynchronize(s));
  memset(&st.pp, 0, sizeof(st.pp));
  st.pp.world = W; st.pp.rank = c->rank; st.pp.cand_cap = st.cand_cap; st.pp.misc_stride = (int32_t)misc_stride;
  st.pp.epoch = st.words.p; st.pp.done = st.words.p + kP2PSlots; st.pp.err = st.words.p + 2 * kP2PSlots;
  st.pp.abort_flag = c->d_abort ? c->d_abort : st.words.p + 2 * kP2PSlots + 1;
  st.pp.spin_limit = (long long)p2p_timeout_seconds() * 1000000LL;
  for (int w = 0; w < W && ok; ++w) {
    uint8_t* base = b->xarena.p;
    if (w != c->rank) {
      void* q = nullptr;
      if (cudaIpcOpenMemHandle(&q, all[w], cudaIpcMemLazyEnablePeerAccess) != cudaSuccess) { ok = 0; cudaGetLastError(); break; }
      st.opened.push_back(q);
      base = (uint8_t*)q;
    }
    st.pp.build[w] = (long long*)base; st.pp.cands[w] = (B2SplitCand*)(base + b->xoff_cands);
    st.pp.misc[w] = (long long*)(base + b->xoff_misc); st.pp.flags[w] = (uint32_t*)(base + b->xoff_flags);
  }
  DevBuf<int32_t> d_ok; d_ok.ensure(1);
  int32_t neg = ok ? 0 : 1;
  CUDA_CHECK(cudaMemcpyAsync(d_ok.p, &neg, sizeof(neg), cudaMemcpyHostToDevice, s));
  allreduce(c, d_ok.p, 1, kNcclInt32, kNcclMax, s);
  CUDA_CHECK(cudaMemcpyAsync(&neg, d_ok.p, sizeof(neg), cudaMemcpyDeviceToHost, s));
  CUDA_CHECK(cudaStreamSynchronize(s));
  if (neg) {
    for (void* q : st.opened) cudaIpcCloseMemHandle(q);
    st.opened.clear();
    if (getenv("B2_EXCHANGE")) fprintf(stderr, "[b2hist] peer mapping failed on some rank; histogram exchange stays on NCCL\n");
    return;
  }
  st.enabled = true;
}

void ensure_ctl_tables(Booster* b) {
  const int D = b->p.max_depth; const int G = b->train->n_groups;
  if (b->ctl_depth == D) return;
  if (b->ctl_depth != 0 && b->p2p.enabled) fail("max_depth cannot change while the peer-memory exchange is mapped");
  for (auto& kv : b->graphs) {
    if (kv.second.exec) cudaGraphExecDestroy(kv.second.exec);
    for (auto& pr : kv.second.hist_ev) { cudaEventDestroy(pr.first); cudaEventDestroy(pr.second); }
  }
  b->graphs.clear(); b->direct_trees.clear();
  b->ctl_depth = D;
  const TreeLayout L = tree_layout(D);
  const size_t lcap = (size_t)1 << D, half = (size_t)1 << (D > 0 ? D - 1 : 0);
  b->t_i32.ensure(L.i32_count); b->t_f32.ensure(L.f32_count); b->t_i64.ensure(L.i64_count);
  b->t_cat.ensure(b->train->any_cat() ? L.max_nodes * 8 : 8);
  b->d_ctl.ensure(3);
  for (int k = 0; k < 2; ++k) { b->d_seg[k].ensure(lcap); b->d_ev[k].ensure(lcap); }
  b->d_hist_work.ensure(half); b->d_split_work.ensure(half);
  b->d_counters.ensure(2 * half); b->d_triples.ensure(3 * half); b->d_pair_parent.ensure(half);
  b->d_leaves.ensure(L.max_nodes); b->d_seg_work.ensure(L.max_nodes);
  b->d_leaf_sums.ensure(2 * lcap); b->d_leaf_values.ensure(lcap);
  b->node_elems = (size_t)G * B2_GROUP_ELEMS;
  const int world = b->comm ? b->comm->world : 1;
  b->shards = (world > 1 && world <= 32 && (32 % world) == 0) ? world : 1;
  b->log2_shards = 0; while ((1 << b->log2_shards) < b->shards) b->log2_shards++;
  b->sp = B2_GROUP_SLOTS / b->shards;
  b->slice_elems = (size_t)G * 2 * B2_BINS * b->sp;
  b->cpn_num = (G * b->sp + 31) / 32;
  b->cpn = b->cpn_num + (b->train->any_cat() ? b2_cat_ctas() : 0);
  b->hist[0].ensure(half * b->slice_elems); b->hist[1].ensure(half * b->slice_elems);
  if (b->shards > 1) {
    auto up = [](size_t v) { return (v + 255) & ~(size_t)255; };
    const size_t build_bytes = up(half * b->node_elems * sizeof(long long));
    const size_t cands_bytes = up(half * b->cpn * b->shards * sizeof(B2SplitCand));
    b->x_misc_stride = 2 + 2 * lcap;
    const size_t misc_bytes = up((size_t)b->shards * b->x_misc_stride * sizeof(long long));
    const size_t flag_bytes = up((size_t)b2_p2p_flag_words(b->shards) * sizeof(uint32_t));
    b->xoff_cands = build_bytes; b->xoff_misc = b->xoff_cands + cands_bytes; b->xoff_flags = b->xoff_misc + misc_bytes;
    b->xarena.ensure(b->xoff_flags + flag_bytes);
    b->hist_build.p = (long long*)b->xarena.p;
    b->d_cands_all.p = (B2SplitCand*)(b->xarena.p + b->xoff_cands);
    b->p2p.misc = (long long*)(b->xarena.p + b->xoff_misc);
    b->p2p.flags = (uint32_t*)(b->xarena.p + b->xoff_flags);
  }
  b->d_cands.ensure(half * b->cpn);
  CUDA_CHECK(cudaMemsetAsync(b->t_i64.p, 0, L.i64_count * 8, b->ctx->stream));
  b->p2p.cand_cap = (int)(half * b->cpn);
  p2p_setup(b);
}

struct TreeStats {
  long long hist_launches = 0, kernel_launches = 0;
  double allreduce_bytes = 0;
  std::vector<std::pair<cudaEvent_t, cudaEvent_t>> hist_ev;
  bool capturing = false;
};
void record_hist_launch(Booster* b, TreeStats& st, cudaEvent_t& e0, cudaEvent_t& e1, bool begin) {
  if (!b->p.profile) return;
  cudaStream_t s = b->ctx->stream;
  if (begin) {
    if (st.capturing) { CUDA_CHECK(cudaEventCreate(&e0)); CUDA_CHECK(cudaEventCreate(&e1)); }
    else { e0 = get_event(b); e1 = get_event(b); }
    CUDA_CHECK(cudaEventRecordWithFlags(e0, s, st.capturing ? cudaEventRecordExternal : cudaEventRecordDefault));
  } else {
    CUDA_CHECK(cudaEventRecordWithFlags(e1, s, st.capturing ? cudaEventRecordExternal : cudaEventRecordDefault));
    st.hist_ev.push_back({e0, e1});
  }
}

bool use_tma_hist() {
  static int v = -1;
  if (v < 0) { const char* e = getenv("B2_HIST_TMA"); v = (e && atoi(e) != 0) ? 1 : 0; }
  return v == 1;
}
bool env_flag(const char* name, bool dflt) {
  const char* e = getenv(name);
  return e ? atoi(e) != 0 : dflt;
}

long long* build_target(Booster* b, long long* level_buf) { return b->shards > 1 ? b->hist_build.p : level_buf; }

void exchange_and_subtract(Booster* b, TreeStats& st, const long long* parent_level, long long* level_buf, const int32_t* triples,
                           const B2LevelCtl* ctl_nxt, int nb, int node_cap) {
  cudaStream_t s = b->ctx->stream;
  const bool multi = b->comm && b->comm->world > 1;
  if (multi && b->comm->aborted.load()) fail("communicator aborted");
  if (multi && b->p2p.enabled) {
    LAUNCH_CHECK(b2_launch_p2p_reduce_subtract(&b->p2p.pp, parent_level, level_buf, triples, ctl_nxt, nb, node_cap,
                                               (int64_t)b->slice_elems, b->ctx->num_sms, s));
    st.allreduce_bytes += (double)nb * b->node_elems * 8 * (b->shards - 1) / b->shards;
    st.kernel_launches++;
    mark_phase(b, 2);
    return;
  }
  if (multi && b->shards > 1) {
    NCCL_CHECK(nccl()->ReduceScatter(b->hist_build.p, level_buf, (size_t)nb * b->slice_elems, kNcclInt64, kNcclSum, b->comm->comm, s));
    st.allreduce_bytes += (double)nb * b->node_elems * 8 * (b->shards - 1) / b->shards;
  } else if (multi) {
    NCCL_CHECK(nccl()->AllReduce(level_buf, level_buf, (size_t)nb * b->node_elems, kNcclInt64, kNcclSum, b->comm->comm, s));
    st.allreduce_bytes += (double)nb * b->node_elems * 8;
  }
  mark_phase(b, 2);
  if (triples) {
    LAUNCH_CHECK(b2_launch_hist_subtract(parent_level, level_buf, triples, nb, (int64_t)b->slice_elems, ctl_nxt, s));
    st.kernel_launches++;
  }
  mark_phase(b, 3);
}

void grow_tree(Booster* b, int k, int slot, TreeStats& st) {
  Matrix* m = b->train; Ctx* ctx = b->ctx; cudaStream_t s = ctx->stream; const Params& p = b->p;
  const int64_t n = m->n; const int K = p.num_class; const int G = m->n_groups; const int D = p.max_depth;
  const float2* gh = b->gh.p + (size_t)k * n;
  ensure_ctl_tables(b);
  const TreeLayout L = tree_layout(D);
  const bool multi = b->comm && b->comm->world > 1;
  const bool p2p = multi && b->p2p.enabled;
  static const bool leaf_fused = env_flag("B2_LEAF_FUSED", true);
  mark_phase(b, -1);
  const uint32_t tree_index = (uint32_t)b->trees.size() + (uint32_t)slot;
  uint32_t* d_absmax = b->d_absmax.p + 2 * k;
  if (p.subsample < 1.0f) {
    LAUNCH_CHECK(b2_launch_subsample(b->gh.p + (size_t)k * n, n, (uint32_t)p.seed, tree_index, b->comm ? (uint32_t)b->comm->rank : 0u,
                                     (double)p.subsample, ctx->num_sms, s));
    st.kernel_launches++;
  }
  std::vector<int> n_level_feats(D > 0 ? D : 1, m->F);
  if (p.use_cols()) {
    const int F = m->F;
    const uint32_t* fwq = m->fwq.empty() ? nullptr : m->fwq.data();
    std::vector<uint8_t> mask_tree(F), masks((size_t)std::max(D, 1) * F);
    for (int f = 0; f < F; ++f)
      mask_tree[f] = b2_col_selected((uint32_t)p.seed, tree_index, B2_SCOPE_TREE, f, nullptr, fwq, F, b2_sample_count((double)p.colsample_bytree, F));
    int n_tree = 0; for (int f = 0; f < F; ++f) n_tree += mask_tree[f];
    for (int d = 0; d < D; ++d) {
      int cnt = 0;
      for (int f = 0; f < F; ++f) {
        masks[(size_t)d * F + f] = b2_col_selected((uint32_t)p.seed, tree_index, B2_SCOPE_LEVEL(d), f, mask_tree.data(), fwq, F,
                                                   b2_sample_count((double)p.colsample_bylevel, n_tree));
        cnt += masks[(size_t)d * F + f];
      }
      n_level_feats[d] = cnt;
    }
    b->d_col_masks.ensure(masks.size());
    CUDA_CHECK(cudaMemcpyAsync(b->d_col_masks.p, masks.data(), masks.size(), cudaMemcpyHostToDevice, s));
  }
  if (!b->absmax_fused) {
    CUDA_CHECK(cudaMemsetAsync(d_absmax, 0, 2 * sizeof(uint32_t), s));
    LAUNCH_CHECK(b2_launch_absmax(gh, n, d_absmax, ctx->num_sms, s));
    st.kernel_launches++;
  }
  if (p2p) LAUNCH_CHECK(b2_launch_p2p_quant_exponent(&b->p2p.pp, d_absmax, b->d_qexp.p, s));
  else {
    allreduce(b->comm, d_absmax, 2, kNcclUint32, kNcclMax, s);
    LAUNCH_CHECK(b2_launch_quant_exponent(d_absmax, b->d_qexp.p, s));
  }
  LAUNCH_CHECK(b2_launch_quantize(gh, n, b->d_qexp.p, p.qbits, b->q.p, ctx->num_sms, s));
  st.kernel_launches += 2;

  B2TrainParamDev dp;
  dp.min_child_weight = (double)p.min_child_weight; dp.lambda = (double)p.lambda; dp.alpha = (double)p.alpha;
  dp.inv_scale_g = dp.inv_scale_h = 1.0;
  dp.max_cat_to_onehot = p.max_cat_to_onehot; dp.max_cat_threshold = p.max_cat_threshold;
  dp.max_delta_step = (double)p.max_delta_step;
  B2CtlParams cp; cp.mcw = dp.min_child_weight; cp.lambda = dp.lambda; cp.alpha = dp.alpha; cp.max_delta_step = dp.max_delta_step; cp.gamma = p.gamma; cp.eta = p.eta / (float)p.num_parallel_tree;
  const B2TreeDev tree = tree_dev(b);
  int32_t* d_n_leaves = tree.n_nodes + 1;
  long long* d_level_rows = b->t_i64.p + 2 * L.max_nodes;
  B2LevelCtl* ctl = b->d_ctl.p;
  const int window = window_rows_for(p.qbits);
  const int n_streams = std::max(1, ctx->num_sms * 3 / G);
  const int pchunk = b2_split_chunk_rows(), lchunk = b2_part_chunk_rows();
  const int max_part_chunks_total = (int)((n + pchunk - 1) / pchunk);
  const size_t lcap = (size_t)1 << D;
  const int max_leaf_chunks = (int)((n + lchunk - 1) / lchunk) + (int)lcap;

  LAUNCH_CHECK(b2_launch_tree_init(tree, ctl, b->d_seg[0].p, b->d_ev[0].p, d_n_leaves, (int)n, b->d_hist_work.p, s));
  CUDA_CHECK(cudaMemsetAsync(b->d_leaf_sums.p, 0, 2 * lcap * sizeof(long long), s));
  mark_phase(b, 0);
  const int sh = b->log2_shards;
  const int shard_rank = b->shards > 1 ? b->comm->rank : 0;
  CUDA_CHECK(cudaMemsetAsync(build_target(b, b->hist[0].p), 0, b->node_elems * sizeof(long long), s));
  {
    const int chunk_rows = pick_chunk_rows(b, n);
    const int chunks = (int)((n + chunk_rows - 1) / chunk_rows);
    if (n > 0) {
      cudaEvent_t e0 = nullptr, e1 = nullptr;
      record_hist_launch(b, st, e0, e1, true);
      if (use_tma_hist() && m->has_tmap)
        LAUNCH_CHECK(b2_launch_hist_tma(m->bins.p, m->row_stride, m->tmap_tile, b->q.p, nullptr, b->d_hist_work.p, 1, chunks, chunk_rows, window, G,
                                        build_target(b, b->hist[0].p), nullptr, sh, 1, n, ctx->num_sms, s));
      else
        LAUNCH_CHECK(b2_launch_hist(m->bins.p, m->row_stride, b->q.p, nullptr, b->d_hist_work.p, 1, chunks, chunk_rows, window, G,
                                    build_target(b, b->hist[0].p), nullptr, sh, 1, m->narrow_w, ctx->num_sms, s));
      record_hist_launch(b, st, e0, e1, false);
      st.hist_launches++; st.kernel_launches++;
    }
  }
  mark_phase(b, 1);
  exchange_and_subtract(b, st, nullptr, b->hist[0].p, nullptr, nullptr, 1, 1);
  LAUNCH_CHECK(b2_launch_root_totals(b->hist[0].p, G, b->d_ev[0].p, b->d_qexp.p, p.qbits, dp, sh, s));
  LAUNCH_CHECK(b2_launch_root_record(tree, b->d_ev[0].p, s));
  st.kernel_launches += 3;
  int hb = 0;
  for (int d = 0; d <= D; ++d) {
    const int cur = d & 1, nxt = cur ^ 1;
    const int max_nodes_level = 1 << d;
    const bool can_split = d < D;
    const bool last_split_level = d == D - 1;
    const B2SplitCand* cands_for_decide = b->d_cands.p;
    int cand_rank_stride = max_nodes_level * b->cpn;
    if (can_split) {
      B2ColSample cs;
      cs.level_mask = p.use_cols() ? b->d_col_masks.p + (size_t)d * m->F : nullptr;
      cs.fwq = m->fwq.empty() ? nullptr : m->d_fwq.p;
      cs.bynode = (double)p.colsample_bynode; cs.n_level = n_level_feats[d]; cs.n_features = m->F;
      cs.seed = (uint32_t)p.seed; cs.tree = p.use_cols() ? tree_index : 0u;
      LAUNCH_CHECK(b2_launch_eval_splits(b->hist[hb].p, G, b->d_ev[cur].p, max_nodes_level, m->d_group_first.p, m->d_group_size.p,
                                         m->d_nbins.p, m->d_has_missing.p, m->any_cat() ? m->d_is_cat.p : nullptr, b->d_qexp.p,
                                         p.qbits, dp, b->d_cands.p, b->cpn, ctl + cur, sh, shard_rank, cs, b->d_seg[cur].p, s));
      st.kernel_launches++;
      if (m->any_cat()) {
        LAUNCH_CHECK(b2_launch_eval_cat_splits(b->hist[hb].p, G, b->d_ev[cur].p, max_nodes_level, m->d_cat_feats.p,
                                               (int)m->cat_feats.size(), m->d_feat_byte.p, m->d_nbins.p, b->d_qexp.p, p.qbits, dp,
                                               b->d_cands.p, b->cpn, b->cpn_num, ctl + cur, sh, shard_rank, cs, b->d_seg[cur].p, s));
        st.kernel_launches++;
      }
      if (p2p) {
        cands_for_decide = b->d_cands_all.p;
        cand_rank_stride = b->p2p.cand_cap;
      } else if (b->shards > 1) {
        const size_t bytes = (size_t)max_nodes_level * b->cpn * sizeof(B2SplitCand);
        NCCL_CHECK(nccl()->AllGather(b->d_cands.p, b->d_cands_all.p, bytes, kNcclUint8, b->comm->comm, s));
        cands_for_decide = b->d_cands_all.p;
      }
    }
    LAUNCH_CHECK(b2_launch_decide(ctl + cur, ctl + nxt, b->d_seg[cur].p, b->d_seg[nxt].p, b->d_ev[cur].p, b->d_ev[nxt].p,
                                  cands_for_decide, b->cpn, b->shards, cand_rank_stride, can_split ? 1 : 0, tree,
                                  b->d_split_work.p, b->d_pair_parent.p, b->d_leaves.p,
                                  d_n_leaves, m->d_has_missing.p, b->d_qexp.p, p.qbits, cp, can_split ? b->d_counters.p : nullptr, b->d_cands.p,
                                  (p2p && can_split) ? &b->p2p.pp : nullptr, s));
    st.kernel_launches++;
    mark_phase(b, 4);
    if (!can_split) break;
    const int32_t* ridx_in = d == 0 ? nullptr : b->ridx[cur].p;
    if (last_split_level && leaf_fused) {
      LAUNCH_CHECK(b2_launch_leaf_plan(b->d_leaves.p, &ctl[cur].leaf_base_next, b->d_seg_work.p, ctl + 2, s));
      LAUNCH_CHECK(b2_launch_leaf_sums(gh, b->ridx[0].p, b->ridx[1].p, b->d_seg_work.p, ctl + 2, max_leaf_chunks, b->d_qexp.p, 40,
                                       b->d_leaf_sums.p, b->pos.p, ctx->num_sms, s));
      LAUNCH_CHECK(b2_launch_final_assign(m->bins_col.p, m->col_stride, ridx_in, b->d_split_work.p, ctl + cur,
                                          max_part_chunks_total + max_nodes_level, gh, b->d_qexp.p, 40, b->d_leaf_sums.p, b->pos.p,
                                          m->any_cat() ? 1 : 0, ctx->num_sms, s));
      st.kernel_launches += 3;
      mark_phase(b, 5);
      continue;
    }
    LAUNCH_CHECK(b2_launch_partition(m->bins_col.p, m->col_stride, ridx_in, b->ridx[nxt].p, b->d_split_work.p, ctl + cur,
                                     max_part_chunks_total + max_nodes_level, b->d_counters.p, m->any_cat() ? 1 : 0,
                                     ctx->num_sms, s));
    const bool need_hist = d + 1 < D;
    LAUNCH_CHECK(b2_launch_finalize_level(ctl + cur, ctl + nxt, b->d_seg[nxt].p, b->d_ev[nxt].p, b->d_split_work.p, b->d_counters.p,
                                          b->d_pair_parent.p, b->d_hist_work.p, b->d_triples.p, max_nodes_level, need_hist ? 1 : 0,
                                          n_streams, window, p.hist_chunk_rows, d_level_rows + d + 1, s));
    st.kernel_launches += 2;
    mark_phase(b, 5);
    if (need_hist) {
      const int nh = hb ^ 1;
      long long* tgt = build_target(b, b->hist[nh].p);
      CUDA_CHECK(cudaMemsetAsync(tgt, 0, (size_t)max_nodes_level * b->node_elems * sizeof(long long), s));
      cudaEvent_t e0 = nullptr, e1 = nullptr;
      record_hist_launch(b, st, e0, e1, true);
      if (use_tma_hist() && m->has_tmap)
        LAUNCH_CHECK(b2_launch_hist_tma(m->bins.p, m->row_stride, m->tmap_tile, b->q.p, b->ridx[nxt].p, b->d_hist_work.p, 0, 0, 0, window, G, tgt, ctl + nxt, sh,
                                        max_nodes_level, n, ctx->num_sms, s));
      else
        LAUNCH_CHECK(b2_launch_hist(m->bins.p, m->row_stride, b->q.p, b->ridx[nxt].p, b->d_hist_work.p, 0, 0, 0, window, G, tgt,
                                    ctl + nxt, sh, max_nodes_level, m->narrow_w, ctx->num_sms, s));
      record_hist_launch(b, st, e0, e1, false);
      st.hist_launches++; st.kernel_launches++;
      mark_phase(b, 1);
      exchange_and_subtract(b, st, b->hist[hb].p, b->hist[nh].p, b->d_triples.p, ctl + nxt, max_nodes_level, max_nodes_level);
      hb = nh;
    }
  }
  if (!leaf_fused) {
    LAUNCH_CHECK(b2_launch_leaf_plan(b->d_leaves.p, d_n_leaves, b->d_seg_work.p, ctl + 2, s));
    LAUNCH_CHECK(b2_launch_leaf_sums(gh, b->ridx[0].p, b->ridx[1].p, b->d_seg_work.p, ctl + 2, max_leaf_chunks, b->d_qexp.p, 40,
                                     b->d_leaf_sums.p, nullptr, ctx->num_sms, s));
    st.kernel_launches += 2;
  }
  if (p2p) { LAUNCH_CHECK(b2_launch_p2p_leaf_sums(&b->p2p.pp, d_n_leaves, b->d_leaf_sums.p, s)); st.kernel_launches++; }
  else allreduce(b->comm, b->d_leaf_sums.p, 2 * lcap, kNcclInt64, kNcclSum, s);
  LAUNCH_CHECK(b2_launch_leaf_values(b->d_leaves.p, d_n_leaves, b->d_leaf_sums.p, b->d_qexp.p, 40, cp, b->d_leaf_values.p, tree, s));
  if (leaf_fused)
    LAUNCH_CHECK(b2_launch_margin_update(b->margin.p, K, k, b->pos.p, b->d_leaf_values.p, n, ctx->num_sms, s));
  else
    LAUNCH_CHECK(b2_launch_pred_update(b->margin.p, K, k, b->ridx[0].p, b->ridx[1].p, b->d_seg_work.p, ctl + 2, max_leaf_chunks,
                                       b->d_leaf_values.p, ctx->num_sms, s));
  st.kernel_launches += 2;
  mark_phase(b, 6);
  char* stg = (char*)b->staging[slot];
  CUDA_CHECK(cudaMemcpyAsync(stg, b->t_i32.p, L.i32_count * 4, cudaMemcpyDeviceToHost, s));
  CUDA_CHECK(cudaMemcpyAsync(stg + L.off_f32, b->t_f32.p, L.f32_count * 4, cudaMemcpyDeviceToHost, s));
  CUDA_CHECK(cudaMemcpyAsync(stg + L.off_i64, b->t_i64.p, L.i64_count * 8, cudaMemcpyDeviceToHost, s));
  CUDA_CHECK(cudaMemcpyAsync(stg + L.off_qexp, b->d_qexp.p, 2 * sizeof(int32_t), cudaMemcpyDeviceToHost, s));
  if (m->any_cat()) CUDA_CHECK(cudaMemcpyAsync(stg + L.off_cat, b->t_cat.p, L.max_nodes * 8 * sizeof(uint32_t), cudaMemcpyDeviceToHost, s));
}

void apply_tree_stats(Booster* b, long long hist_launches, long long kernel_launches, double allreduce_bytes,
                      const std::vector<std::pair<cudaEvent_t, cudaEvent_t>>& ev) {
  b->t.hist_launches += hist_launches; b->t.kernel_launches += kernel_launches; b->t.allreduce_bytes += allreduce_bytes;
  for (auto& pr : ev) b->hist_events.push_back(pr);
}

void prepare_tree_buffers(Booster* b, int slot) {
  Matrix* m = b->train; const int64_t n = m->n;
  ensure_ctl_tables(b);
  const TreeLayout L = tree_layout(b->p.max_depth);
  const size_t rows = (size_t)std::max<int64_t>(n, 1);
  b->d_absmax.ensure(2 * (size_t)b->p.num_class); b->d_qexp.ensure(2);
  b->q.ensure(rows); b->ridx[0].ensure(rows); b->ridx[1].ensure(rows); b->pos.ensure(rows);
  if (b->staging_bytes != L.bytes) {
    for (void* h : b->staging) cudaFreeHost(h);
    b->staging.clear(); b->staging_bytes = L.bytes;
  }
  while ((int)b->staging.size() <= slot) { void* h = nullptr; CUDA_CHECK(cudaMallocHost(&h, L.bytes)); b->staging.push_back(h); }
}

void run_tree(Booster* b, int k, int slot) {
  cudaStream_t s = b->ctx->stream; const Params& p = b->p;
  prepare_tree_buffers(b, slot);
  static const bool want_graph = env_flag("B2_GRAPH", true);
  const bool eligible = want_graph && !b->graph_failed && b->absmax_fused && p.subsample >= 1.0f && !p.use_cols() &&
                        p.profile < 2 && !use_tma_hist() && p.num_parallel_tree == 1;
  auto direct = [&]() {
    TreeStats st;
    grow_tree(b, k, slot, st);
    apply_tree_stats(b, st.hist_launches, st.kernel_launches, st.allreduce_bytes, st.hist_ev);
    b->direct_trees[k]++;
  };
  if (!eligible) { direct(); return; }
  auto it = b->graphs.find(k);
  if (it == b->graphs.end()) {
    if (b->direct_trees[k] == 0) { direct(); return; }
    TreeStats st; st.capturing = true;
    cudaGraph_t graph = nullptr; cudaGraphExec_t exec = nullptr;
    bool ok = cudaStreamBeginCapture(s, cudaStreamCaptureModeThreadLocal) == cudaSuccess;
    if (ok) {
      try { grow_tree(b, k, slot, st); }
      catch (const B2Error& e) { cudaStreamEndCapture(s, &graph); if (graph) cudaGraphDestroy(graph); cudaGetLastError(); throw; }
      ok = cudaStreamEndCapture(s, &graph) == cudaSuccess && graph != nullptr;
    }
    if (ok) ok = cudaGraphInstantiate(&exec, graph, 0) == cudaSuccess;
    if (graph) cudaGraphDestroy(graph);
    if (!ok) {
      cudaGetLastError();
      for (auto& pr : st.hist_ev) { cudaEventDestroy(pr.first); cudaEventDestroy(pr.second); }
      b->graph_failed = true;
      fprintf(stderr, "[b2hist] CUDA graph capture of the tree failed; continuing with direct launches\n");
      direct();
      return;
    }
    Booster::TreeGraph g;
    g.exec = exec; g.hist_ev = st.hist_ev; g.hist_launches = st.hist_launches; g.kernel_launches = st.kernel_launches;
    g.allreduce_bytes = st.allreduce_bytes;
    it = b->graphs.emplace(k, std::move(g)).first;
  }
  CUDA_CHECK(cudaGraphLaunch(it->second.exec, s));
  apply_tree_stats(b, it->second.hist_launches, it->second.kernel_launches, it->second.allreduce_bytes, it->second.hist_ev);
}

void materialize_tree(Booster* b, int slot) {
  Matrix* m = b->train; const Params& p = b->p;
  const TreeLayout L = tree_layout(p.max_depth);
  const char* st = (const char*)b->staging[slot];
  const int32_t* i32 = (const int32_t*)st; const size_t mx = L.max_nodes;
  const float* f32 = (const float*)(st + L.off_f32);
  const long long* i64 = (const long long*)(st + L.off_i64);
  const int32_t* qexp = (const int32_t*)(st + L.off_qexp);
  const int nn = i32[7 * mx];
  const uint32_t* cat = (const uint32_t*)(st + L.off_cat);
  if (nn < 1 || (size_t)nn > mx) fail("corrupt tree read-back (n_nodes=%d)", nn);
  const double inv_sg = ldexp(1.0, qexp[0] - p.qbits), inv_sh = ldexp(1.0, qexp[1] - p.qbits);
  TreeHost t;
  for (int i = 0; i < nn; ++i) {
    t.add(i32[2 * mx + i]);
    t.left[i] = i32[i]; t.right[i] = i32[mx + i]; t.feature[i] = i32[3 * mx + i];
    const double G = (double)i64[i] * inv_sg, H = (double)i64[mx + i] * inv_sh;
    t.sum_hess[i] = H;
    if (t.feature[i] >= 0) {
      const int f = t.feature[i], bin = i32[4 * mx + i];
      t.split_bin[i] = bin; t.default_left[i] = (uint8_t)i32[5 * mx + i]; t.loss_chg[i] = f32[i];
      if (m->any_cat() && i32[6 * mx + i]) {
        t.split_type[i] = 1; t.any_cat = true;
        for (int w8 = 0; w8 < 8; ++w8) t.cat_bits[(size_t)i * 8 + w8] = cat[(size_t)i * 8 + w8];
        t.cond[i] = bin >= 0 ? (float)bin : NAN;
      } else
      t.cond[i] = bin < 0 ? m->min_vals[f] : m->cut_vals[m->cut_ptrs[f] + bin];
      t.base_weight[i] = h_calc_weight(p, G, H);
      t.value[i] = t.base_weight[i];
    } else {
      t.base_weight[i] = f32[mx + i];
      t.value[i] = f32[2 * mx + i];
    }
  }
  const long long* level_rows = i64 + 2 * mx;
  long long rows = m->n; int launches_nonempty = m->n > 0 ? 1 : 0;
  for (int d = 1; d < p.max_depth; ++d) { rows += level_rows[d]; if (level_rows[d] > 0) launches_nonempty++; }
  long long gathered = rows - m->n;
  int built_nodes = 0;
  for (int i = 0; i < nn; ++i) if (t.feature[i] >= 0) built_nodes++;
  b->t.hist_rows += rows;
  b->t.hist_bytes += (double)rows * (m->F + 8) + (double)gathered * 4 + (double)(built_nodes + 1) * m->F * 256.0 * 16.0;
  b->trees.push_back(std::move(t));
}

void sync_device_trees(Booster* b) {
  if (b->d_trees_synced == (int)b->trees.size()) return;
  b->h_nodes.clear(); b->h_tree_offset.clear(); b->h_cat_table.clear();
  for (auto& t : b->trees) {
    b->h_tree_offset.push_back((int32_t)b->h_nodes.size());
    for (int i = 0; i < t.size(); ++i) {
      int32_t cat_slot = -1;
      if (t.feature[i] >= 0 && t.split_type[i]) {
        cat_slot = (int32_t)(b->h_cat_table.size() / 8);
        b->h_cat_table.insert(b->h_cat_table.end(), t.cat_bits.begin() + (size_t)i * 8, t.cat_bits.begin() + (size_t)i * 8 + 8);
      }
      b->h_nodes.push_back(B2TreeNodeDev{t.left[i], t.right[i], t.feature[i], t.cond[i], t.value[i], (int32_t)t.default_left[i],
                                         cat_slot, 0});
    }
  }
  cudaStream_t s = b->ctx->stream;
  upload(b->d_nodes, b->h_nodes, s); upload(b->d_tree_offset, b->h_tree_offset, s); upload(b->d_cat_table, b->h_cat_table, s);
  CUDA_CHECK(cudaStreamSynchronize(s));
  b->d_trees_synced = (int)b->trees.size();
}

struct PathBuildElem {
  int32_t feature; bool is_cat; float lo, hi; uint32_t flags; uint32_t bits[8]; double z;
};
void walk_paths(const TreeHost& t, int nid, std::vector<PathBuildElem>& path, int tree, int cls, Booster* b,
                std::vector<B2PathElem>& elems, std::vector<B2PathInfo>& infos, std::vector<uint32_t>& cats, double* expected) {
  if (t.feature[nid] < 0) {
    if (path.size() + 1 > B2_SHAP_MAX_PATH)
      fail("tree %d has a leaf below %d distinct features; TreeSHAP supports at most %d (max_depth <= 14)", tree,
           (int)path.size(), B2_SHAP_MAX_PATH - 1);
    B2PathInfo pi{(int32_t)elems.size(), (int32_t)path.size() + 1, cls, 0, (double)t.value[nid]};
    elems.push_back(B2PathElem{-1, -1, 0.f, 0.f, 0u, 0u, 1.0});
    double zprod = 1.0;
    for (const PathBuildElem& e : path) {
      int32_t slot = -1;
      if (e.is_cat) { slot = (int32_t)(cats.size() / 8); cats.insert(cats.end(), e.bits, e.bits + 8); }
      elems.push_back(B2PathElem{e.feature, slot, e.lo, e.hi, e.flags, 0u, e.z});
      zprod *= e.z;
    }
    *expected += (double)t.value[nid] * zprod;
    infos.push_back(pi);
    return;
  }
  const int f = t.feature[nid];
  const bool is_cat = t.split_type[nid] != 0;
  const double cover = t.sum_hess[nid];
  for (int side = 0; side < 2; ++side) {
    const int child = side == 0 ? t.left[nid] : t.right[nid];
    const bool left = side == 0;
    std::vector<PathBuildElem> next = path;
    PathBuildElem* e = nullptr;
    for (auto& x : next) if (x.feature == f) e = &x;
    if (!e) {
      PathBuildElem ne;
      ne.feature = f; ne.is_cat = is_cat; ne.lo = -INFINITY; ne.hi = INFINITY;
      ne.flags = B2_PATH_MISSING_OK | B2_PATH_OUTSIDE_OK; ne.z = 1.0;
      for (int w = 0; w < 8; ++w) ne.bits[w] = 0xffffffffu;
      next.push_back(ne); e = &next.back();
    }
    e->z *= cover > 0.0 ? t.sum_hess[child] / cover : 0.0;
    if ((t.default_left[nid] != 0) != left) e->flags &= ~B2_PATH_MISSING_OK;
    if (is_cat) {
      e->is_cat = true;
      for (int w = 0; w < 8; ++w) e->bits[w] &= left ? ~t.cat_bits[(size_t)nid * 8 + w] : t.cat_bits[(size_t)nid * 8 + w];
      if (!left) e->flags &= ~B2_PATH_OUTSIDE_OK;
    } else if (left) {
      if (!(e->flags & B2_PATH_HAS_HI) || t.cond[nid] < e->hi) e->hi = t.cond[nid];
      e->flags |= B2_PATH_HAS_HI;
    } else if (t.cond[nid] > e->lo) {
      e->lo = t.cond[nid];
    }
    walk_paths(t, child, next, tree, cls, b, elems, infos, cats, expected);
  }
}

void build_paths(Booster* b) {
  if (b->paths_synced == (int)b->trees.size()) return;
  std::vector<B2PathElem> elems; std::vector<B2PathInfo> infos; std::vector<uint32_t> cats;
  b->tree_path_offset.assign(1, 0); b->tree_expected.clear();
  const int K = b->p.num_class, npt = std::max(1, b->p.num_parallel_tree);
  for (int t = 0; t < (int)b->trees.size(); ++t) {
    std::vector<PathBuildElem> path;
    double expected = 0.0;
    walk_paths(b->trees[t], 0, path, t, (t / npt) % K, b, elems, infos, cats, &expected);
    b->tree_path_offset.push_back((int32_t)infos.size());
    b->tree_expected.push_back(expected);
  }
  cudaStream_t s = b->ctx->stream;
  upload(b->d_path_elems, elems, s); upload(b->d_paths, infos, s); upload(b->d_path_cats, cats, s);
  CUDA_CHECK(cudaStreamSynchronize(s));
  b->paths_synced = (int)b->trees.size();
}

void init_margin(Booster* b, float* margin, Matrix* m) {
  const int K = b->p.num_class; cudaStream_t s = b->ctx->stream;
  if (m->n_base_margin > 0) {
    if (m->n_base_margin != m->n * K) fail("base_margin has %lld values, expected %lld", (long long)m->n_base_margin, (long long)(m->n * K));
    CUDA_CHECK(cudaMemcpyAsync(margin, m->base_margin.p, (size_t)m->n * K * sizeof(float), cudaMemcpyDeviceToDevice, s));
  } else {
    LAUNCH_CHECK(b2_launch_fill(margin, m->n * K, base_margin_value(b->p), b->ctx->num_sms, s));
  }
}

void estimate_base_score(Booster* b) {
  Matrix* m = b->train; cudaStream_t s = b->ctx->stream; Params& p = b->p;
  if (p.base_score_set || p.objective == kObjSoftprob) { p.base_score_set = true; return; }
  if (!b->trees.empty()) fail("continuing from existing trees needs an explicit base_score (the source model's intercept)");
  if (m->n_label != m->n) fail("train matrix has %lld labels for %lld rows", (long long)m->n_label, (long long)m->n);
  const int64_t n = m->n;
  DevBuf<float> zeros; DevBuf<float2> gh; DevBuf<long long> sums;
  zeros.ensure((size_t)std::max<int64_t>(n, 1)); gh.ensure((size_t)std::max<int64_t>(n, 1)); sums.ensure(2);
  CUDA_CHECK(cudaMemsetAsync(zeros.p, 0, (size_t)std::max<int64_t>(n, 1) * sizeof(float), s));
  LAUNCH_CHECK(b2_launch_gradient(p.objective, 1, zeros.p, m->label.p, m->n_weight ? m->weight.p : nullptr, n, p.scale_pos_weight,
                                  objective_param(p), gh.p, nullptr, nullptr, b->ctx->num_sms, s));
  b->d_absmax.ensure(2); b->d_qexp.ensure(2);
  CUDA_CHECK(cudaMemsetAsync(b->d_absmax.p, 0, 2 * sizeof(uint32_t), s));
  LAUNCH_CHECK(b2_launch_absmax(gh.p, n, b->d_absmax.p, b->ctx->num_sms, s));
  allreduce(b->comm, b->d_absmax.p, 2, kNcclUint32, kNcclMax, s);
  LAUNCH_CHECK(b2_launch_quant_exponent(b->d_absmax.p, b->d_qexp.p, s));
  CUDA_CHECK(cudaMemsetAsync(sums.p, 0, 2 * sizeof(long long), s));
  LAUNCH_CHECK(b2_launch_sum_fixed(gh.p, n, b->d_qexp.p, 40, sums.p, b->ctx->num_sms, s));
  allreduce(b->comm, sums.p, 2, kNcclInt64, kNcclSum, s);
  long long h_s[2]; int32_t h_e[2];
  CUDA_CHECK(cudaMemcpyAsync(h_s, sums.p, sizeof(h_s), cudaMemcpyDeviceToHost, s));
  CUDA_CHECK(cudaMemcpyAsync(h_e, b->d_qexp.p, sizeof(h_e), cudaMemcpyDeviceToHost, s));
  CUDA_CHECK(cudaStreamSynchronize(s));
  const double G = (double)h_s[0] / ldexp(1.0, 40 - h_e[0]), H = (double)h_s[1] / ldexp(1.0, 40 - h_e[1]);
  const float stump = H <= 1e-6 ? 0.0f : (float)(-G / H);
  if (obj_sigmoid(p.objective) || obj_log_link(p.objective)) {
    DevBuf<float> one; one.ensure(1);
    CUDA_CHECK(cudaMemcpyAsync(one.p, &stump, sizeof(float), cudaMemcpyHostToDevice, s));
    LAUNCH_CHECK(b2_launch_transform(p.objective, 1, one.p, 1, b->ctx->num_sms, s));
    float prob = 0.5f;
    CUDA_CHECK(cudaMemcpyAsync(&prob, one.p, sizeof(float), cudaMemcpyDeviceToHost, s));
    CUDA_CHECK(cudaStreamSynchronize(s));
    p.base_score = prob;
  } else {
    p.base_score = stump;
  }
  p.base_score_set = true;
}

void check_labels(Booster* b) {
  Matrix* m = b->train; const int o = b->p.objective; cudaStream_t s = b->ctx->stream;
  if (o == kObjSquaredError || o == kObjLogistic || o == kObjSoftprob || o == kObjPseudoHuber || b->labels_checked) return;
  if (m->n_label != m->n) fail("train matrix has %lld labels for %lld rows", (long long)m->n_label, (long long)m->n);
  DevBuf<uint32_t> bad; bad.ensure(1);
  CUDA_CHECK(cudaMemsetAsync(bad.p, 0, sizeof(uint32_t), s));
  LAUNCH_CHECK(b2_launch_label_check(o, m->label.p, m->n, bad.p, b->ctx->num_sms, s));
  allreduce(b->comm, bad.p, 1, kNcclUint32, kNcclMax, s);
  uint32_t h = 0;
  CUDA_CHECK(cudaMemcpyAsync(&h, bad.p, sizeof(h), cudaMemcpyDeviceToHost, s));
  CUDA_CHECK(cudaStreamSynchronize(s));
  if (h) {
    const char* cond = (o == kObjRegLogistic || o == kObjLogitRaw) ? "label must be in [0, 1]"
                       : o == kObjSquaredLog ? "label must be greater than -1"
                       : o == kObjGamma ? "label must be positive" : "label must be nonnegative";
    fail("%s for %s", cond, b->p.objective_name.c_str());
  }
  b->labels_checked = true;
}

void ensure_train_margin(Booster* b) {
  if (b->margin_ready) return;
  Matrix* m = b->train;
  check_labels(b);
  estimate_base_score(b);
  b->margin.ensure((size_t)std::max<int64_t>(m->n * b->p.num_class, 1));
  init_margin(b, b->margin.p, m);
  if (!b->trees.empty()) {
    if (!m->has_raw) fail("continuing training from existing trees needs the raw data of the train matrix (B2_MatrixEnsureRaw)");
    sync_device_trees(b);
    LAUNCH_CHECK(b2_launch_predict(m->raw.p, m->n, m->F, m->missing, b->d_nodes.p, b->d_tree_offset.p, b->d_cat_table.p, 0, (int)b->trees.size(),
                                   b->p.num_class, b->p.num_parallel_tree, b->margin.p, b->ctx->num_sms, b->ctx->stream));
  }
  b->margin_ready = true;
}

void boost_round(Booster* b, const float* custom_g, const float* custom_h, int64_t len) {
  if (!b->train) fail("this booster has no train matrix (prediction-only)");
  Matrix* m = b->train; cudaStream_t s = b->ctx->stream; const int K = b->p.num_class; const int64_t n = m->n;
  CUDA_CHECK(cudaSetDevice(b->ctx->device));
  if (b->cancel.load()) fail("training cancelled");
  if (!b->round_start) { CUDA_CHECK(cudaEventCreate(&b->round_start)); CUDA_CHECK(cudaEventCreate(&b->round_stop)); }
  if (b->p.profile) CUDA_CHECK(cudaEventRecord(b->round_start, s));
  ensure_train_margin(b);
  b->gh.ensure((size_t)std::max<int64_t>(n * K, 1));
  b->d_absmax.ensure(2 * (size_t)K); b->d_qexp.ensure(2);
  b->absmax_fused = false;
  bool check_finite = false;
  if (custom_g) {
    if (len != n * K) fail("custom gradient has %lld values, expected %lld", (long long)len, (long long)(n * K));
    b->d_custom_g.ensure((size_t)std::max<int64_t>(len, 1)); b->d_custom_h.ensure((size_t)std::max<int64_t>(len, 1));
// ... 885 lines not shown
```

### xgboost_ray_b200/csrc/partition_kernel.cu

```cuda
#include <stdlib.h>

#include "common.cuh"

namespace b2 {

constexpr int kPartThreads = 256;
constexpr int kPartChunk = 2048;

typedef B2SegWork SegWork;

constexpr int kSplitChunk = 8192;
constexpr int kSplitPasses = kSplitChunk / kPartChunk;

template <int kMode, bool kRoot>
__global__ void __launch_bounds__(kPartThreads)
partition_kernel(const uint8_t* __restrict__ bins_col, int64_t col_stride, const int32_t* __restrict__ ridx_in,
                 int32_t* __restrict__ ridx_out, const B2SplitWork* __restrict__ work, const B2LevelCtl* __restrict__ ctl,
                 int32_t* __restrict__ counters ) {
  const int n_work = ctl->n_split, total_chunks = ctl->part_chunks;
  constexpr int kIters = kPartChunk / kPartThreads;
  constexpr int kWarps = kPartThreads / 32;
  constexpr int kCounts = kSplitPasses * kIters * kWarps;
  __shared__ uint32_t s_rid[kSplitChunk];
  __shared__ int s_cnt[kCounts];
  __shared__ int s_base_left, s_base_right;
  __shared__ uint32_t s_cat[8];
  const int lane = threadIdx.x & 31, warp = threadIdx.x >> 5;
  for (int chunk = blockIdx.x; chunk < total_chunks; chunk += gridDim.x) {
    int lo = 0, hi = n_work - 1;
    while (lo < hi) {
      int mid = (lo + hi + 1) >> 1;
      if (__ldg(&work[mid].chunk_begin) <= chunk) lo = mid; else hi = mid - 1;
    }
    const B2SplitWork w = work[lo];
    const int row0 = (chunk - w.chunk_begin) * kSplitChunk;
    const int nrows = min(kSplitChunk, w.seg_count - row0);
    constexpr bool kCat = kMode != 0;
    if (kMode == 1) {
      if (threadIdx.x < 8) s_cat[threadIdx.x] = w.is_cat ? __ldg(&work[lo].cat_bits[threadIdx.x]) : 0u;
      __syncthreads();
    }
    const bool is_cat = kCat && w.is_cat != 0, has_missing = w.has_missing != 0, default_left = w.default_left != 0;
#pragma unroll 1
    for (int pass = 0; pass < kSplitPasses; ++pass) {
      const int pbase = pass * kPartChunk;
      if (pbase >= nrows) {
        if (threadIdx.x < kIters * kWarps) s_cnt[pass * kIters * kWarps + threadIdx.x] = 0;
        continue;
      }
      int rid[kIters]; bool left[kIters]; int bin[kIters];
      const int32_t* rsrc = kRoot ? nullptr : ridx_in + w.seg_begin + row0 + pbase + threadIdx.x;
#pragma unroll
      for (int it = 0; it < kIters; ++it) {
        const int r = pbase + it * kPartThreads + threadIdx.x;
        rid[it] = kRoot ? (r < nrows ? w.seg_begin + row0 + r : 0) : (r < nrows ? __ldg(rsrc + it * kPartThreads) : 0);
      }
      const uint8_t* col = bins_col + (int64_t)w.feature * col_stride;
#pragma unroll
      for (int it = 0; it < kIters; ++it) bin[it] = (int)__ldg(col + rid[it]);
#pragma unroll
      for (int it = 0; it < kIters; ++it) {
        const int r = pbase + it * kPartThreads + threadIdx.x;
        const bool valid = r < nrows;
        const int b = bin[it];
        bool l;
        if (kCat) {
          const uint32_t word = s_cat[b >> 5];
          const bool in_set = ((word >> (b & 31)) & 1u) != 0u;
          const bool go_left = is_cat ? !in_set : (b <= w.split_bin);
          l = (has_missing && b == B2_MISSING_BIN) ? default_left : go_left;
        } else {
          l = (w.has_missing && b == B2_MISSING_BIN) ? (w.default_left != 0) : (b <= w.split_bin);
        }
        left[it] = valid && l;
      }
#pragma unroll
      for (int it = 0; it < kIters; ++it) {
        const unsigned bal = __ballot_sync(0xffffffffu, left[it]);
        if (lane == 0) s_cnt[(pass * kIters + it) * kWarps + warp] = __popc(bal);
        s_rid[pbase + it * kPartThreads + threadIdx.x] = (uint32_t)rid[it] | (left[it] ? 0x80000000u : 0u);
      }
    }
    __syncthreads();
    if (warp == 0) {
      int c[kCounts / 32], sum = 0;
#pragma unroll
      for (int k = 0; k < kCounts / 32; ++k) { c[k] = s_cnt[lane * (kCounts / 32) + k]; sum += c[k]; }
      int incl = sum;
#pragma unroll
      for (int o = 1; o < 32; o <<= 1) { const int v = __shfl_up_sync(0xffffffffu, incl, o); if (lane >= o) incl += v; }
      int run = incl - sum;
#pragma unroll
      for (int k = 0; k < kCounts / 32; ++k) { s_cnt[lane * (kCounts / 32) + k] = run; run += c[k]; }
      if (lane == 31) {
        const unsigned long long old = atomicAdd(reinterpret_cast<unsigned long long*>(counters + 2 * lo),
                                                 ((unsigned long long)(unsigned)nrows << 32) | (unsigned long long)(unsigned)incl);
        s_base_left = (int)(unsigned)(old & 0xffffffffull);
        s_base_right = (int)(unsigned)(old >> 32) - s_base_left;
      }
    }
    __syncthreads();
    const int base_l = s_base_left, base_r = s_base_right;
#pragma unroll 1
    for (int pass = 0; pass < kSplitPasses; ++pass) {
      const int pbase = pass * kPartChunk;
      if (pbase >= nrows) break;
#pragma unroll
      for (int it = 0; it < kIters; ++it) {
        const int r = pbase + it * kPartThreads + threadIdx.x;
        const uint32_t v = s_rid[r];
        const bool l = (v & 0x80000000u) != 0u;
        const unsigned bal = __ballot_sync(0xffffffffu, l);
        if (r < nrows) {
          const int lrank = s_cnt[(pass * kIters + it) * kWarps + warp] + __popc(bal & ((1u << lane) - 1u));
          if (l) ridx_out[w.seg_begin + base_l + lrank] = (int32_t)(v & 0x7fffffffu);
          else {
            const int rrank = r - lrank;
            ridx_out[w.seg_begin + w.seg_count - 1 - (base_r + rrank)] = (int32_t)v;
          }
        }
      }
    }
    __syncthreads();
  }
}

__global__ void __launch_bounds__(256)
leaf_sums_kernel(const float2* __restrict__ gh, const int32_t* __restrict__ ridx0, const int32_t* __restrict__ ridx1,
                 const SegWork* __restrict__ work, const B2LevelCtl* __restrict__ ctl, const int32_t* __restrict__ qexp,
                 int leaf_bits, long long* __restrict__ sums ,
                 uint16_t* __restrict__ pos ) {
  const int n_work = ctl->hist_n_work, total_chunks = ctl->hist_total_chunks;
  __shared__ long long sg[8], sh[8];
  const double kg = ldexp(1.0, leaf_bits - qexp[0]), kh = ldexp(1.0, leaf_bits - qexp[1]);
  for (int chunk = blockIdx.x; chunk < total_chunks; chunk += gridDim.x) {
    int lo = 0, hi = n_work - 1;
    while (lo < hi) {
      int mid = (lo + hi + 1) >> 1;
      if (__ldg(&work[mid].chunk_begin) <= chunk) lo = mid; else hi = mid - 1;
    }
    const SegWork w = work[lo];
    const int32_t* ridx = w.pad0 ? nullptr : (w.buf ? ridx1 : ridx0);
    const int row0 = (chunk - w.chunk_begin) * kPartChunk;
    const int nrows = min(kPartChunk, w.seg_count - row0);
    long long ag = 0, ah = 0;
    for (int r = threadIdx.x; r < nrows; r += blockDim.x) {
      const int row = ridx ? __ldg(ridx + w.seg_begin + row0 + r) : (w.seg_begin + row0 + r);
      if (pos) pos[row] = (uint16_t)w.id;
      const float2 v = __ldg(gh + row);
      ag += __double2ll_rn(__dmul_rn((double)v.x, kg));
      ah += __double2ll_rn(__dmul_rn((double)v.y, kh));
    }
#pragma unroll
    for (int o = 16; o > 0; o >>= 1) { ag += __shfl_xor_sync(0xffffffffu, ag, o); ah += __shfl_xor_sync(0xffffffffu, ah, o); }
    if ((threadIdx.x & 31) == 0) { sg[threadIdx.x >> 5] = ag; sh[threadIdx.x >> 5] = ah; }
    __syncthreads();
    if (threadIdx.x == 0) {
      long long tg = 0, th = 0;
      for (int i = 0; i < 8; ++i) { tg += sg[i]; th += sh[i]; }
      atomicAdd((unsigned long long*)&sums[2 * w.id], (unsigned long long)tg);
      atomicAdd((unsigned long long*)&sums[2 * w.id + 1], (unsigned long long)th);
    }
    __syncthreads();
  }
}

__global__ void __launch_bounds__(256)
pred_update_kernel(float* __restrict__ margin, int K, int k, const int32_t* __restrict__ ridx0,
                   const int32_t* __restrict__ ridx1, const SegWork* __restrict__ work, const B2LevelCtl* __restrict__ ctl,
                   const float* __restrict__ leaf_value) {
  const int n_work = ctl->hist_n_work, total_chunks = ctl->hist_total_chunks;
  for (int chunk = blockIdx.x; chunk < total_chunks; chunk += gridDim.x) {
    int lo = 0, hi = n_work - 1;
    while (lo < hi) {
      int mid = (lo + hi + 1) >> 1;
      if (__ldg(&work[mid].chunk_begin) <= chunk) lo = mid; else hi = mid - 1;
    }
    const SegWork w = work[lo];
    const int32_t* ridx = w.pad0 ? nullptr : (w.buf ? ridx1 : ridx0);
    const int row0 = (chunk - w.chunk_begin) * kPartChunk;
    const int nrows = min(kPartChunk, w.seg_count - row0);
    const float v = __ldg(leaf_value + w.id);
    for (int r = threadIdx.x; r < nrows; r += blockDim.x) {
      const int64_t row = ridx ? __ldg(ridx + w.seg_begin + row0 + r) : (w.seg_begin + row0 + r);
      margin[row * K + k] += v;
    }
  }
}

template <bool kCat, bool kRoot>
__global__ void __launch_bounds__(kPartThreads)
final_assign_kernel(const uint8_t* __restrict__ bins_col, int64_t col_stride, const int32_t* __restrict__ ridx_in,
                    const B2SplitWork* __restrict__ work, const B2LevelCtl* __restrict__ ctl, const float2* __restrict__ gh,
                    const int32_t* __restrict__ qexp, int leaf_bits, long long* __restrict__ sums,
                    uint16_t* __restrict__ pos) {
  const int n_work = ctl->n_split, total_chunks = ctl->part_chunks, leaf_base = ctl->leaf_base_next;
  __shared__ long long s_acc[kPartThreads / 32][4];
  const double kg = ldexp(1.0, leaf_bits - qexp[0]), kh = ldexp(1.0, leaf_bits - qexp[1]);
  const int lane = threadIdx.x & 31, warp = threadIdx.x >> 5;
  for (int chunk = blockIdx.x; chunk < total_chunks; chunk += gridDim.x) {
    int lo = 0, hi = n_work - 1;
    while (lo < hi) {
      int mid = (lo + hi + 1) >> 1;
      if (__ldg(&work[mid].chunk_begin) <= chunk) lo = mid; else hi = mid - 1;
    }
    const B2SplitWork w = work[lo];
    const int row0 = (chunk - w.chunk_begin) * kSplitChunk;
    const int nrows = min(kSplitChunk, w.seg_count - row0);
    const bool is_cat = kCat && w.is_cat != 0;
    const int leaf_l = leaf_base + 2 * lo;
    long long lg = 0, lh = 0, rg = 0, rh = 0;
    constexpr int kBatch = 4;
    const uint8_t* col = bins_col + (int64_t)w.feature * col_stride;
    for (int r0 = threadIdx.x; r0 < nrows; r0 += kBatch * kPartThreads) {
      int rid[kBatch]; int bin[kBatch]; float2 v[kBatch];
#pragma unroll
      for (int k = 0; k < kBatch; ++k) {
        const int r = r0 + k * kPartThreads;
        rid[k] = r < nrows ? (kRoot ? w.seg_begin + row0 + r : __ldg(ridx_in + w.seg_begin + row0 + r)) : -1;
      }
#pragma unroll
      for (int k = 0; k < kBatch; ++k) { bin[k] = (int)__ldg(col + (rid[k] < 0 ? 0 : rid[k])); v[k] = __ldg(gh + (rid[k] < 0 ? 0 : rid[k])); }
#pragma unroll
      for (int k = 0; k < kBatch; ++k) {
        if (rid[k] < 0) continue;
        const int b = bin[k];
        bool go_left = b <= w.split_bin;
        if (kCat && is_cat) go_left = ((__ldg(&work[lo].cat_bits[b >> 5]) >> (b & 31)) & 1u) == 0u;
        const bool l = (w.has_missing && b == B2_MISSING_BIN) ? (w.default_left != 0) : go_left;
        const long long qg = __double2ll_rn(__dmul_rn((double)v[k].x, kg)), qh = __double2ll_rn(__dmul_rn((double)v[k].y, kh));
        if (l) { lg += qg; lh += qh; } else { rg += qg; rh += qh; }
        pos[rid[k]] = (uint16_t)(leaf_l + (l ? 0 : 1));
      }
    }
#pragma unroll
    for (int o = 16; o > 0; o >>= 1) {
      lg += __shfl_xor_sync(0xffffffffu, lg, o); lh += __shfl_xor_sync(0xffffffffu, lh, o);
      rg += __shfl_xor_sync(0xffffffffu, rg, o); rh += __shfl_xor_sync(0xffffffffu, rh, o);
    }
    if (lane == 0) { s_acc[warp][0] = lg; s_acc[warp][1] = lh; s_acc[warp][2] = rg; s_acc[warp][3] = rh; }
    __syncthreads();
    if (threadIdx.x < 4) {
      long long t = 0;
      for (int i = 0; i < kPartThreads / 32; ++i) t += s_acc[i][threadIdx.x];
      atomicAdd((unsigned long long*)&sums[2 * leaf_l + threadIdx.x], (unsigned long long)t);
    }
    __syncthreads();
  }
}

__global__ void __launch_bounds__(256)
margin_update_kernel(float* __restrict__ margin, int K, int k, const uint16_t* __restrict__ pos,
                     const float* __restrict__ leaf_value, int64_t n) {
  for (int64_t i = (int64_t)blockIdx.x * blockDim.x + threadIdx.x; i < n; i += (int64_t)gridDim.x * blockDim.x)
    margin[i * K + k] += __ldg(leaf_value + pos[i]);
}

__global__ void iota_kernel(int32_t* out, int64_t n) {
  for (int64_t i = (int64_t)blockIdx.x * blockDim.x + threadIdx.x; i < n; i += (int64_t)gridDim.x * blockDim.x) out[i] = (int32_t)i;
}

}

extern "C" {
int b2_part_chunk_rows() { return b2::kPartChunk; }
int b2_split_chunk_rows() { return b2::kSplitChunk; }

int b2_launch_partition(const uint8_t* bins_col, int64_t col_stride, const int32_t* ridx_in, int32_t* ridx_out,
                        const B2SplitWork* work, const B2LevelCtl* ctl, int max_chunks, int32_t* counters, int any_categorical,
                        int num_sms, cudaStream_t stream) {
  if (max_chunks <= 0) return 0;
  int grid = max_chunks < num_sms * 6 ? max_chunks : num_sms * 6;
#define B2_PART_LAUNCH(MODE)                                                                                                  \
  do {                                                                                                                        \
    if (ridx_in) b2::partition_kernel<MODE, false><<<grid, b2::kPartThreads, 0, stream>>>(bins_col, col_stride, ridx_in, ridx_out, work, ctl, counters); \
    else b2::partition_kernel<MODE, true><<<grid, b2::kPartThreads, 0, stream>>>(bins_col, col_stride, ridx_in, ridx_out, work, ctl, counters);         \
  } while (0)
  if (any_categorical) B2_PART_LAUNCH(1);
  else B2_PART_LAUNCH(0);
#undef B2_PART_LAUNCH
  return (int)cudaGetLastError();
}
int b2_launch_leaf_sums(const float2* gh, const int32_t* ridx0, const int32_t* ridx1, const void* work, const B2LevelCtl* ctl,
                        int max_chunks, const int32_t* qexp, int leaf_bits, long long* sums, uint16_t* pos, int num_sms,
                        cudaStream_t stream) {
  if (max_chunks <= 0) return 0;
  int grid = max_chunks < num_sms * 8 ? max_chunks : num_sms * 8;
  b2::leaf_sums_kernel<<<grid, 256, 0, stream>>>(gh, ridx0, ridx1, (const b2::SegWork*)work, ctl, qexp, leaf_bits, sums, pos);
  return (int)cudaGetLastError();
}
int b2_launch_final_assign(const uint8_t* bins_col, int64_t col_stride, const int32_t* ridx_in, const B2SplitWork* work,
                           const B2LevelCtl* ctl, int max_chunks, const float2* gh, const int32_t* qexp, int leaf_bits,
                           long long* sums, uint16_t* pos, int any_categorical, int num_sms, cudaStream_t stream) {
  if (max_chunks <= 0) return 0;
  int grid = max_chunks < num_sms * 8 ? max_chunks : num_sms * 8;
#define B2_FA_LAUNCH(CAT, ROOT) b2::final_assign_kernel<CAT, ROOT><<<grid, b2::kPartThreads, 0, stream>>>(bins_col, col_stride, ridx_in, work, ctl, gh, qexp, leaf_bits, sums, pos)
  if (any_categorical) { if (ridx_in) B2_FA_LAUNCH(true, false); else B2_FA_LAUNCH(true, true); }
  else { if (ridx_in) B2_FA_LAUNCH(false, false); else B2_FA_LAUNCH(false, true); }
#undef B2_FA_LAUNCH
  return (int)cudaGetLastError();
}
int b2_launch_margin_update(float* margin, int K, int k, const uint16_t* pos, const float* leaf_value, int64_t n, int num_sms,
                            cudaStream_t stream) {
  if (n <= 0) return 0;
  int64_t want = (n + 255) / 256;
  int grid = (int)(want < (int64_t)num_sms * 16 ? want : (int64_t)num_sms * 16);
  b2::margin_update_kernel<<<grid, 256, 0, stream>>>(margin, K, k, pos, leaf_value, n);
  return (int)cudaGetLastError();
}
int b2_launch_pred_update(float* margin, int K, int k, const int32_t* ridx0, const int32_t* ridx1, const void* work,
                          const B2LevelCtl* ctl, int max_chunks, const float* leaf_value, int num_sms, cudaStream_t stream) {
  if (max_chunks <= 0) return 0;
  int grid = max_chunks < num_sms * 8 ? max_chunks : num_sms * 8;
  b2::pred_update_kernel<<<grid, 256, 0, stream>>>(margin, K, k, ridx0, ridx1, (const b2::SegWork*)work, ctl, leaf_value);
  return (int)cudaGetLastError();
}
int b2_launch_iota(int32_t* out, int64_t n, cudaStream_t stream) {
  if (n <= 0) return 0;
  int grid = (int)((n + 1023) / 1024);
  if (grid > 4096) grid = 4096;
  b2::iota_kernel<<<grid, 256, 0, stream>>>(out, n);
  return (int)cudaGetLastError();
}
}
```

### xgboost_ray_b200/csrc/split_kernel.cu

```cuda
#include <cub/block/block_scan.cuh>

#include "common.cuh"
#include "sampling.cuh"

namespace b2 {

__device__ __forceinline__ double calc_gain(double G, double H, const B2TrainParamDev& p) {
  return b2_calc_gain(G, H, p.min_child_weight, p.lambda, p.alpha, p.max_delta_step);
}

struct Best {
  unsigned long long key;
  int32_t bin, default_left;
  long long lg, lh;
};

__device__ __forceinline__ void consider(Best& b, float chg, uint32_t order, int bin, int dl, long long lg, long long lh) {
  if (!(chg > 0.0f) || isinf(chg)) return;
  unsigned long long key = ((unsigned long long)__float_as_uint(chg) << 32) | (unsigned long long)(0xffffffffu - order);
  if (key > b.key) { b.key = key; b.bin = bin; b.default_left = dl; b.lg = lg; b.lh = lh; }
}

constexpr int kEvalChunks = 32;
constexpr int kEvalBinsPerChunk = 256 / kEvalChunks;

__global__ void __launch_bounds__(32 * kEvalChunks)
eval_splits_kernel(const long long* __restrict__ level_hist, int n_groups, const B2EvalNode* __restrict__ nodes,
                   const int32_t* __restrict__ group_first, const int32_t* __restrict__ group_size,
                   const int32_t* __restrict__ nbins, const uint8_t* __restrict__ has_missing,
                   const uint8_t* __restrict__ is_cat ,
                   const int32_t* __restrict__ qexp, int qbits, B2TrainParamDev p, B2SplitCand* __restrict__ cands,
                   int cand_stride, const B2LevelCtl* __restrict__ ctl, int log2_shards, int shard_rank, B2ColSample cs,
                   const B2NodeSeg* __restrict__ seg) {
  const int sp = B2_GROUP_SLOTS >> log2_shards;
  const int cpn = (n_groups * sp + 31) >> 5;
  const int node = blockIdx.x / cpn, cta_in_node = blockIdx.x % cpn;
  if (ctl && node >= ctl->n_nodes) return;
  const int s = threadIdx.x & 31, q = threadIdx.x >> 5;
  __shared__ long long cs_g[kEvalChunks][32], cs_h[kEvalChunks][32];
  __shared__ unsigned long long wkey[kEvalChunks];
  const B2EvalNode nd = nodes[node];
  p.inv_scale_g = ldexp(1.0, qexp[0] - qbits);
  p.inv_scale_h = ldexp(1.0, qexp[1] - qbits);
  const int v = cta_in_node * 32 + s;
  const bool v_ok = v < n_groups * sp;
  const int group = v_ok ? v / sp : 0, sl = v_ok ? v % sp : 0;
  const int slot = (sl << log2_shards) + shard_rank;
  const size_t slice_elems = (size_t)n_groups * 2 * B2_BINS * sp;
  const long long* hg = level_hist + (size_t)nd.hist_index * slice_elems + (size_t)(group * 2) * B2_BINS * sp + sl;
  const long long* hh = hg + (size_t)B2_BINS * sp;
  const int f = group_first[group] + slot;
  bool active = v_ok && slot < group_size[group] && !(is_cat && is_cat[f]);
  if (active && cs.level_mask) active = cs.level_mask[f] != 0;
  if (cs.bynode < 1.0) {
    __shared__ uint8_t s_allowed[32];
    if (q == 0)
      s_allowed[s] = active && b2_col_selected(cs.seed, cs.tree, B2_SCOPE_NODE(seg[node].nid), f, cs.level_mask, cs.fwq,
                                               cs.n_features, b2_sample_count(cs.bynode, cs.n_level));
    __syncthreads();
    active = active && s_allowed[s];
  }
  const int nf = active ? nbins[f] : 0;
  const bool fmiss = active ? (has_missing[f] != 0) : false;

  long long sg = 0, sh = 0;
  if (active) {
#pragma unroll
    for (int i = 0; i < kEvalBinsPerChunk; ++i) {
      int b = q * kEvalBinsPerChunk + i;
      if (b < nf) { sg += hg[b * sp]; sh += hh[b * sp]; }
    }
  }
  cs_g[q][s] = sg; cs_h[q][s] = sh;
  __syncthreads();
  long long pg = 0, ph = 0, real_g = 0, real_h = 0;
#pragma unroll 8
  for (int k = 0; k < kEvalChunks; ++k) {
    long long a = cs_g[k][s], b = cs_h[k][s];
    if (k < q) { pg += a; ph += b; }
    real_g += a; real_h += b;
  }
  const long long tot_g = nd.sum_g, tot_h = nd.sum_h;
  const double G = __dmul_rn(__ll2double_rn(tot_g), p.inv_scale_g), H = __dmul_rn(__ll2double_rn(tot_h), p.inv_scale_h);
  const double root_gain = (double)nd.root_gain;
  const bool node_has_missing = fmiss && (real_g != tot_g || real_h != tot_h);
  Best best; best.key = 0; best.bin = 0; best.default_left = 0; best.lg = 0; best.lh = 0;
  if (active) {
#pragma unroll 2
    for (int i = 0; i < kEvalBinsPerChunk; ++i) {
      const int b = q * kEvalBinsPerChunk + i;
      if (b >= nf) break;
      const long long eg_excl = pg, eh_excl = ph;
      pg += hg[b * sp]; ph += hh[b * sp];
      {
        const double lh_d = __dmul_rn(__ll2double_rn(ph), p.inv_scale_h);
        if (lh_d >= p.min_child_weight) {
          const double rh_d = __dadd_rn(H, -lh_d);
          if (rh_d >= p.min_child_weight) {
            const double lg_d = __dmul_rn(__ll2double_rn(pg), p.inv_scale_g);
            const double rg_d = __dadd_rn(G, -lg_d);
            const double gain = __dadd_rn(__dadd_rn(calc_gain(lg_d, lh_d, p), calc_gain(rg_d, rh_d, p)), -root_gain);
            consider(best, __double2float_rn(gain), (uint32_t)f * 1024u + (uint32_t)b, b, 0, pg, ph);
          }
        }
      }
      if (node_has_missing) {
        const long long rg_i = real_g - eg_excl, rh_i = real_h - eh_excl;
        const double rh_d = __dmul_rn(__ll2double_rn(rh_i), p.inv_scale_h);
        if (rh_d >= p.min_child_weight) {
          const double lh_d = __dadd_rn(H, -rh_d);
          if (lh_d >= p.min_child_weight) {
            const double rg_d = __dmul_rn(__ll2double_rn(rg_i), p.inv_scale_g);
            const double lg_d = __dadd_rn(G, -rg_d);
            const double gain = __dadd_rn(__dadd_rn(calc_gain(lg_d, lh_d, p), calc_gain(rg_d, rh_d, p)), -root_gain);
            consider(best, __double2float_rn(gain), (uint32_t)f * 1024u + 512u + (uint32_t)(255 - b), b - 1, 1,
                     tot_g - rg_i, tot_h - rh_i);
          }
        }
      }
    }
  }
  unsigned long long k = best.key;
#pragma unroll
  for (int o = 16; o > 0; o >>= 1) {
    unsigned long long other = __shfl_xor_sync(0xffffffffu, k, o);
    k = other > k ? other : k;
  }
  if (s == 0) wkey[q] = k;
  __syncthreads();
  unsigned long long kmax = 0;
#pragma unroll 8
  for (int i = 0; i < kEvalChunks; ++i) kmax = wkey[i] > kmax ? wkey[i] : kmax;
  B2SplitCand* out = cands + (size_t)node * cand_stride + cta_in_node;
  if (kmax == 0) {
    if (threadIdx.x == 0) {
      out->loss_chg = 0.0f; out->feature = -1; out->bin = 0; out->default_left = 0; out->left_g = 0; out->left_h = 0;
      out->order = 0xffffffffu; out->is_cat = 0;
    }
  } else if (best.key == kmax) {
    out->loss_chg = __uint_as_float((uint32_t)(kmax >> 32));
    out->feature = f; out->bin = best.bin; out->default_left = best.default_left;
    out->left_g = best.lg; out->left_h = best.lh; out->order = 0xffffffffu - (uint32_t)(kmax & 0xffffffffu); out->is_cat = 0;
  }
}

constexpr int kCatCtas = 4;

__device__ __forceinline__ float calc_weight_f(double G, double H, const B2TrainParamDev& p) {
  return __double2float_rn(b2_calc_weight(G, H, p.min_child_weight, p.lambda, p.alpha, p.max_delta_step));
}

__global__ void __launch_bounds__(256)
eval_cat_splits_kernel(const long long* __restrict__ level_hist, int n_groups, const B2EvalNode* __restrict__ nodes,
                       const int32_t* __restrict__ cat_feats, int n_cat, const int32_t* __restrict__ feat_byte,
                       const int32_t* __restrict__ nbins, const int32_t* __restrict__ qexp, int qbits, B2TrainParamDev p,
                       B2SplitCand* __restrict__ cands, int cand_stride, int cand_offset, const B2LevelCtl* __restrict__ ctl,
                       int log2_shards, int shard_rank, B2ColSample cs, const B2NodeSeg* __restrict__ seg) {
  const int node = blockIdx.x / kCatCtas, j = blockIdx.x % kCatCtas;
  if (ctl && node >= ctl->n_nodes) return;
  typedef cub::BlockScan<long long, 256> Scan;
  __shared__ typename Scan::TempStorage scan_tmp;
  __shared__ float s_w[256];
  __shared__ long long s_g[256], s_h[256];
  __shared__ long long s_red[2][8];
  __shared__ unsigned long long s_wkey[8];
  __shared__ unsigned long long s_best_key;
  __shared__ uint32_t s_bits[8];
  __shared__ int s_mode, s_part;
  __shared__ int s_skip;
  __shared__ B2SplitCand s_best;
  const int b = threadIdx.x, lane = b & 31, warp = b >> 5;
  const int sp = B2_GROUP_SLOTS >> log2_shards, shards = 1 << log2_shards;
  const size_t slice_elems = (size_t)n_groups * 2 * B2_BINS * sp;
  const B2EvalNode nd = nodes[node];
  p.inv_scale_g = ldexp(1.0, qexp[0] - qbits);
  p.inv_scale_h = ldexp(1.0, qexp[1] - qbits);
  const long long tot_g = nd.sum_g, tot_h = nd.sum_h;
  const double G = __dmul_rn(__ll2double_rn(tot_g), p.inv_scale_g), H = __dmul_rn(__ll2double_rn(tot_h), p.inv_scale_h);
  const double root_gain = (double)nd.root_gain;
  if (b == 0) s_best_key = 0;
  __syncthreads();
  for (int ci = j; ci < n_cat; ci += kCatCtas) {
    const int f = cat_feats[ci];
    const int fb = feat_byte[f], group = fb >> 5, slot = fb & 31;
    if ((slot & (shards - 1)) != shard_rank) continue;
    if (cs.level_mask || cs.bynode < 1.0) {
      if (b == 0) {
        bool ok = !cs.level_mask || cs.level_mask[f] != 0;
        if (ok && cs.bynode < 1.0)
          ok = b2_col_selected(cs.seed, cs.tree, B2_SCOPE_NODE(seg[node].nid), f, cs.level_mask, cs.fwq, cs.n_features,
                               b2_sample_count(cs.bynode, cs.n_level));
        s_skip = ok ? 0 : 1;
      }
      __syncthreads();
      const bool skip = s_skip != 0;
      __syncthreads();
      if (skip) continue;
    }
    const int sl = slot >> log2_shards;
    const long long* hg = level_hist + (size_t)nd.hist_index * slice_elems + (size_t)(group * 2) * B2_BINS * sp + sl;
    const long long* hh = hg + (size_t)B2_BINS * sp;
    const int nf = nbins[f];
    long long g = 0, h = 0;
    if (b < nf) { g = hg[b * sp]; h = hh[b * sp]; }
    long long rg = g, rh = h;
#pragma unroll
    for (int o = 16; o > 0; o >>= 1) { rg += __shfl_xor_sync(0xffffffffu, rg, o); rh += __shfl_xor_sync(0xffffffffu, rh, o); }
    if (lane == 0) { s_red[0][warp] = rg; s_red[1][warp] = rh; }
    __syncthreads();
    long long real_g = 0, real_h = 0;
#pragma unroll
    for (int k = 0; k < 8; ++k) { real_g += s_red[0][k]; real_h += s_red[1][k]; }
    Best best; best.key = 0; best.bin = 0; best.default_left = 0; best.lg = 0; best.lh = 0;
    int my_mode = 0, my_part = 0, rank = 0;
    if (nf < p.max_cat_to_onehot) {
      if (b < nf) {
        const long long mg = tot_g - real_g, mh = tot_h - real_h;
#pragma unroll
        for (int pass = 0; pass < 2; ++pass) {
          const long long rgi = pass ? g + mg : g, rhi = pass ? h + mh : h;
          const double rh_d = __dmul_rn(__ll2double_rn(rhi), p.inv_scale_h), lh_d = __dadd_rn(H, -rh_d);
          if (lh_d >= p.min_child_weight && rh_d >= p.min_child_weight) {
            const double rg_d = __dmul_rn(__ll2double_rn(rgi), p.inv_scale_g), lg_d = __dadd_rn(G, -rg_d);
            const double gain = __dadd_rn(__dadd_rn(calc_gain(lg_d, lh_d, p), calc_gain(rg_d, rh_d, p)), -root_gain);
            const unsigned long long before = best.key;
            consider(best, __double2float_rn(gain), (uint32_t)f * 1024u + (uint32_t)(2 * b + pass), b, pass ? 0 : 1,
                     tot_g - rgi, tot_h - rhi);
            if (best.key != before) { my_mode = 0; my_part = b; }
          }
        }
      }
    } else {
      const float w = b < nf ? calc_weight_f(__dmul_rn(__ll2double_rn(g), p.inv_scale_g), __dmul_rn(__ll2double_rn(h), p.inv_scale_h), p)
                             : 0.0f;
      s_w[b] = w; s_g[b] = 0; s_h[b] = 0;
      __syncthreads();
      if (b < nf) {
        for (int k = 0; k < nf; ++k) { const float wk = s_w[k]; rank += (wk < w || (wk == w && k < b)) ? 1 : 0; }
        s_g[rank] = g; s_h[rank] = h;
      }
      __syncthreads();
      long long pg, ph;
      Scan(scan_tmp).InclusiveSum(s_g[b], pg);
      __syncthreads();
      Scan(scan_tmp).InclusiveSum(s_h[b], ph);
      __syncthreads();
      s_g[b] = pg; s_h[b] = ph;
      __syncthreads();
      const int n_iter = min(p.max_cat_threshold, nf) - 1;
      const int k = b;
      if (k < n_iter) {
        const double rh_d = __dmul_rn(__ll2double_rn(ph), p.inv_scale_h), lh_d = __dadd_rn(H, -rh_d);
        if (lh_d >= p.min_child_weight && rh_d >= p.min_child_weight) {
          const double rg_d = __dmul_rn(__ll2double_rn(pg), p.inv_scale_g), lg_d = __dadd_rn(G, -rg_d);
          const double gain = __dadd_rn(__dadd_rn(calc_gain(lg_d, lh_d, p), calc_gain(rg_d, rh_d, p)), -root_gain);
          const unsigned long long before = best.key;
          consider(best, __double2float_rn(gain), (uint32_t)f * 1024u + (uint32_t)k, -1, 1, tot_g - pg, tot_h - ph);
          if (best.key != before) { my_mode = 1; my_part = k + 1; }
        }
      }
      if (n_iter > 0 && k >= nf - n_iter && k < nf) {
        const long long lgi = real_g - s_g[k - 1], lhi = real_h - s_h[k - 1];
        const double lh_d = __dmul_rn(__ll2double_rn(lhi), p.inv_scale_h), rh_d = __dadd_rn(H, -lh_d);
        if (lh_d >= p.min_child_weight && rh_d >= p.min_child_weight) {
          const double lg_d = __dmul_rn(__ll2double_rn(lgi), p.inv_scale_g), rg_d = __dadd_rn(G, -lg_d);
          const double gain = __dadd_rn(__dadd_rn(calc_gain(lg_d, lh_d, p), calc_gain(rg_d, rh_d, p)), -root_gain);
          const unsigned long long before = best.key;
          consider(best, __double2float_rn(gain), (uint32_t)f * 1024u + 512u + (uint32_t)(nf - 1 - k), -1, 0, lgi, lhi);
          if (best.key != before) { my_mode = 1; my_part = k; }
        }
      }
    }
    unsigned long long key = best.key;
#pragma unroll
    for (int o = 16; o > 0; o >>= 1) { unsigned long long other = __shfl_xor_sync(0xffffffffu, key, o); key = other > key ? other : key; }
    if (lane == 0) s_wkey[warp] = key;
    __syncthreads();
    unsigned long long kmax = 0;
#pragma unroll
    for (int i = 0; i < 8; ++i) kmax = s_wkey[i] > kmax ? s_wkey[i] : kmax;
    const bool better = kmax != 0 && (uint32_t)(kmax >> 32) > (uint32_t)(s_best_key >> 32);
    __syncthreads();
    if (better) {
      if (best.key == kmax) {
        s_best.loss_chg = __uint_as_float((uint32_t)(kmax >> 32)); s_best.feature = f; s_best.bin = best.bin;
        s_best.default_left = best.default_left; s_best.left_g = best.lg; s_best.left_h = best.lh;
        s_best.order = 0xffffffffu - (uint32_t)(kmax & 0xffffffffu); s_best.is_cat = 1;
        s_mode = my_mode; s_part = my_part; s_best_key = kmax;
      }
      if (b < 8) s_bits[b] = 0;
      __syncthreads();
      if (b < nf && (s_mode == 0 ? (b == s_part) : (rank < s_part))) atomicOr(&s_bits[b >> 5], 1u << (b & 31));
      __syncthreads();
    }
  }
  if (b == 0) {
    B2SplitCand* out = cands + (size_t)node * cand_stride + cand_offset + j;
    if (s_best_key == 0) {
      out->loss_chg = 0.0f; out->feature = -1; out->bin = 0; out->default_left = 0; out->left_g = 0; out->left_h = 0;
      out->order = 0xffffffffu; out->is_cat = 0;
    } else {
      *out = s_best;
#pragma unroll
      for (int i = 0; i < 8; ++i) out->cat_bits[i] = s_bits[i];
    }
  }
}

__global__ void root_totals_kernel(const long long* __restrict__ level_hist, int n_groups, B2EvalNode* nodes,
                                   const int32_t* __restrict__ qexp, int qbits, B2TrainParamDev p, int log2_shards) {
  __shared__ long long sg[256], sh[256];
  const int sp = B2_GROUP_SLOTS >> log2_shards;
  const size_t slice_elems = (size_t)n_groups * 2 * B2_BINS * sp;
  const long long* hg = level_hist + (size_t)nodes[0].hist_index * slice_elems;
  sg[threadIdx.x] = hg[(size_t)threadIdx.x * sp];
  sh[threadIdx.x] = hg[(size_t)(B2_BINS + threadIdx.x) * sp];
  __syncthreads();
  for (int o = 128; o > 0; o >>= 1) {
    if ((int)threadIdx.x < o) { sg[threadIdx.x] += sg[threadIdx.x + o]; sh[threadIdx.x] += sh[threadIdx.x + o]; }
    __syncthreads();
  }
  if (threadIdx.x == 0) {
    p.inv_scale_g = ldexp(1.0, qexp[0] - qbits);
    p.inv_scale_h = ldexp(1.0, qexp[1] - qbits);
    nodes[0].sum_g = sg[0]; nodes[0].sum_h = sh[0];
    double G = __dmul_rn(__ll2double_rn(sg[0]), p.inv_scale_g), H = __dmul_rn(__ll2double_rn(sh[0]), p.inv_scale_h);
    nodes[0].root_gain = __double2float_rn(calc_gain(G, H, p));
  }
}

}

extern "C" {
int b2_launch_eval_splits(const long long* level_hist, int n_groups, const B2EvalNode* nodes, int n_nodes,
                          const int32_t* group_first, const int32_t* group_size, const int32_t* nbins,
                          const uint8_t* has_missing, const uint8_t* is_cat, const int32_t* qexp, int qbits, B2TrainParamDev p,
                          B2SplitCand* cands, int cand_stride, const B2LevelCtl* ctl, int log2_shards, int shard_rank,
                          B2ColSample cs, const B2NodeSeg* seg, cudaStream_t stream) {
  if (n_nodes <= 0) return 0;
  const int sp = B2_GROUP_SLOTS >> log2_shards, cpn = (n_groups * sp + 31) >> 5;
  b2::eval_splits_kernel<<<n_nodes * cpn, 32 * b2::kEvalChunks, 0, stream>>>(level_hist, n_groups, nodes, group_first, group_size,
                                                                         nbins, has_missing, is_cat, qexp, qbits, p, cands,
                                                                         cand_stride, ctl, log2_shards, shard_rank, cs, seg);
  return (int)cudaGetLastError();
}
int b2_cat_ctas() { return b2::kCatCtas; }
int b2_launch_eval_cat_splits(const long long* level_hist, int n_groups, const B2EvalNode* nodes, int n_nodes,
                              const int32_t* cat_feats, int n_cat, const int32_t* feat_byte, const int32_t* nbins,
                              const int32_t* qexp, int qbits, B2TrainParamDev p, B2SplitCand* cands, int cand_stride,
                              int cand_offset, const B2LevelCtl* ctl, int log2_shards, int shard_rank, B2ColSample cs,
                              const B2NodeSeg* seg, cudaStream_t stream) {
  if (n_nodes <= 0 || n_cat <= 0) return 0;
  b2::eval_cat_splits_kernel<<<n_nodes * b2::kCatCtas, 256, 0, stream>>>(level_hist, n_groups, nodes, cat_feats, n_cat, feat_byte,
                                                                        nbins, qexp, qbits, p, cands, cand_stride, cand_offset,
                                                                        ctl, log2_shards, shard_rank, cs, seg);
  return (int)cudaGetLastError();
}
int b2_launch_root_totals(const long long* level_hist, int n_groups, B2EvalNode* nodes, const int32_t* qexp, int qbits,
                          B2TrainParamDev p, int log2_shards, cudaStream_t stream) {
  b2::root_totals_kernel<<<1, 256, 0, stream>>>(level_hist, n_groups, nodes, qexp, qbits, p, log2_shards);
  return (int)cudaGetLastError();
}
}
```

Measured before the change: 230.0.

## Fuse sibling subtraction, level finalize and leaf accumulation into existing kernels

Sibling histograms are now computed inside the split-evaluation kernel (parent minus built child) and written out only when deeper levels need them, so the separate subtraction pass goes away. The level-finalize kernel moves into the partition kernel behind a done-counter, root-record is folded into root_totals, and a streaming leaf accumulation kernel is added for shallow trees. Tree scratch buffers are merged into one block allocation. Together these cut kernel launches and extra histogram passes per level, at the cost of more complex kernels and last-block completion logic.

```diff
diff --git a/xgboost_ray_b200/build.py b/xgboost_ray_b200/build.py
--- a/xgboost_ray_b200/build.py
+++ b/xgboost_ray_b200/build.py
@@ -35,7 +35,7 @@
 
 def build(force=False, verbose=False):
     os.makedirs(OBJ_DIR, exist_ok=True)
-    headers = [os.path.join(CSRC, "common.cuh"), os.path.join(CSRC, "hist_common.cuh"), os.path.join(CSRC, "sampling.cuh"), os.path.join(CSRC, "p2p.cuh"), os.path.join(HERE, "..", "include", "b2hist.h"), __file__]
+    headers = [os.path.join(CSRC, "common.cuh"), os.path.join(CSRC, "hist_common.cuh"), os.path.join(CSRC, "sampling.cuh"), os.path.join(CSRC, "p2p.cuh"), os.path.join(CSRC, "level_finalize.cuh"), os.path.join(HERE, "..", "include", "b2hist.h"), __file__]
     jobs = []
     objs = []
     for src, extra in SOURCES.items():
diff --git a/xgboost_ray_b200/csrc/common.cuh b/xgboost_ray_b200/csrc/common.cuh
--- a/xgboost_ray_b200/csrc/common.cuh
+++ b/xgboost_ray_b200/csrc/common.cuh
@@ -137,6 +137,25 @@
   int32_t n_level;
   int32_t n_features;
   uint32_t seed, tree;
+};
+
+struct B2FinalizeArgs {
+  B2LevelCtl* ctl_nxt;
+  B2NodeSeg* seg_nxt;
+  B2EvalNode* ev_nxt;
+  const int32_t* pair_parent_hist;
+  B2HistWork* hist_work;
+  int32_t* triples;
+  long long* stat_rows;
+  uint32_t* done;
+  int32_t max_pairs, need_hist, n_streams, window_rows, chunk_rows_override;
+};
+
+struct B2SiblingSub {
+  const long long* parent_level;
+  const int32_t* triples;
+  long long* sib_out;
+  int32_t sib_base;
 };
 
 #define B2_P2P_MAX_WORLD 8
diff --git a/xgboost_ray_b200/csrc/control_kernel.cu b/xgboost_ray_b200/csrc/control_kernel.cu
--- a/xgboost_ray_b200/csrc/control_kernel.cu
+++ b/xgboost_ray_b200/csrc/control_kernel.cu
@@ -146,71 +146,6 @@
 }
 
 __global__ void __launch_bounds__(kCtlThreads)
-finalize_level_kernel(const B2LevelCtl* __restrict__ ctl_cur, B2LevelCtl* __restrict__ ctl_nxt, B2NodeSeg* __restrict__ seg_nxt,
-                      B2EvalNode* __restrict__ ev_nxt, const B2SplitWork* __restrict__ split_work,
-                      const int32_t* __restrict__ counters, const int32_t* __restrict__ pair_parent_hist,
-                      B2HistWork* __restrict__ hist_work, int32_t* __restrict__ triples, int max_pairs, int need_hist,
-                      int n_streams, int window_rows, int chunk_rows_override, long long* __restrict__ stat_rows) {
-  __shared__ typename TileScan::Scan::TempStorage tmp;
-  __shared__ long long s_rows;
-  __shared__ int s_chunk_rows;
-  const int ns = ctl_cur->n_split;
-  if (threadIdx.x == 0) s_rows = 0;
-  __syncthreads();
-  long long my_rows = 0;
-  for (int j = threadIdx.x; j < ns; j += kCtlThreads) {
-    const B2SplitWork sw = split_work[j];
-    const int cl = counters[2 * j];
-    B2NodeSeg sl = seg_nxt[2 * j], sr = seg_nxt[2 * j + 1];
-    sl.begin = sw.seg_begin; sl.count = cl;
-    sr.begin = sw.seg_begin + cl; sr.count = sw.seg_count - cl;
-    seg_nxt[2 * j] = sl; seg_nxt[2 * j + 1] = sr;
-    if (need_hist) {
-      const bool build_left = ev_nxt[2 * j].sum_h < ev_nxt[2 * j + 1].sum_h;
-      my_rows += build_left ? sl.count : sr.count;
-    }
-  }
-  if (need_hist) {
-    atomicAdd((unsigned long long*)&s_rows, (unsigned long long)my_rows);
-    __syncthreads();
-    if (threadIdx.x == 0) {
-      int c = chunk_rows_override;
-      if (c <= 0) {
-        const long long per_stream = s_rows / n_streams;
-        const long long target = per_stream >= 16384 ? per_stream / 4 : per_stream;
-        c = 512;
-        while (c < target && c < 8192) c <<= 1;
-      }
-      if (c > window_rows) c = window_rows;
-      s_chunk_rows = c;
-      if (stat_rows) *stat_rows = s_rows;
-    }
-    __syncthreads();
-    const int chunk_rows = s_chunk_rows;
-    TileScan scan(&tmp);
-    for (int base = 0; base < ns; base += kCtlThreads) {
-      const int j = base + threadIdx.x;
-      int chunks = 0, begin = 0, count = 0;
-      if (j < ns) {
-        const bool build_left = ev_nxt[2 * j].sum_h < ev_nxt[2 * j + 1].sum_h;
-        const int b = build_left ? 2 * j : 2 * j + 1, s = b ^ 1;
-        begin = seg_nxt[b].begin; count = seg_nxt[b].count;
-        chunks = (count + chunk_rows - 1) / chunk_rows;
-        ev_nxt[b].hist_index = j; ev_nxt[s].hist_index = max_pairs + j;
-        triples[3 * j] = pair_parent_hist[j]; triples[3 * j + 1] = j; triples[3 * j + 2] = max_pairs + j;
-      }
-      const int cb = scan.step(chunks);
-      if (j < ns) { B2HistWork w; w.seg_begin = begin; w.seg_count = count; w.hist_index = j; w.chunk_begin = cb; hist_work[j] = w; }
-    }
-    __syncthreads();
-    if (threadIdx.x == 0) {
-      ctl_nxt->hist_n_work = ns; ctl_nxt->hist_total_chunks = scan.carry; ctl_nxt->hist_chunk_rows = chunk_rows;
-      ctl_nxt->n_pairs = ns;
-    }
-  }
-}
-
-__global__ void __launch_bounds__(kCtlThreads)
 leaf_plan_kernel(const B2LeafDev* __restrict__ leaves, const int32_t* __restrict__ n_leaves, B2SegWork* __restrict__ work,
                  B2LevelCtl* __restrict__ leaf_ctl) {
   __shared__ typename TileScan::Scan::TempStorage tmp;
@@ -233,8 +168,9 @@
 
 __global__ void leaf_values_kernel(const B2LeafDev* __restrict__ leaves, const int32_t* __restrict__ n_leaves,
                                    const long long* __restrict__ sums, const int32_t* __restrict__ qexp, int leaf_bits,
-                                   B2CtlParams p, float* __restrict__ leaf_value, B2TreeDev tree) {
+                                   B2CtlParams p, float* __restrict__ leaf_value, B2TreeDev tree, int32_t* __restrict__ qexp_out) {
   const int n = *n_leaves;
+  if (blockIdx.x == 0 && threadIdx.x < 2) qexp_out[threadIdx.x] = qexp[threadIdx.x];
   const double kg = ldexp(1.0, leaf_bits - qexp[0]), kh = ldexp(1.0, leaf_bits - qexp[1]);
   for (int i = blockIdx.x * blockDim.x + threadIdx.x; i < n; i += gridDim.x * blockDim.x) {
     const double G = __ddiv_rn(__ll2double_rn(sums[2 * i]), kg), H = __ddiv_rn(__ll2double_rn(sums[2 * i + 1]), kh);
@@ -259,9 +195,6 @@
     B2EvalNode e; e.sum_g = 0; e.sum_h = 0; e.hist_index = 0; e.root_gain = 0.f; ev0[0] = e;
   }
 }
-__global__ void root_record_kernel(B2TreeDev tree, const B2EvalNode* ev0) {
-  if (threadIdx.x == 0 && blockIdx.x == 0) { tree.sum_g[0] = ev0[0].sum_g; tree.sum_h[0] = ev0[0].sum_h; }
-}
 
 }
 
@@ -278,22 +211,13 @@
                                                  part_counters, local_cands, p2p ? 1 : 0, pp);
   return (int)cudaGetLastError();
 }
-int b2_launch_finalize_level(const B2LevelCtl* ctl_cur, B2LevelCtl* ctl_nxt, B2NodeSeg* seg_nxt, B2EvalNode* ev_nxt,
-                             const B2SplitWork* split_work, const int32_t* counters, const int32_t* pair_parent_hist,
-                             B2HistWork* hist_work, int32_t* triples, int max_pairs, int need_hist, int n_streams,
-                             int window_rows, int chunk_rows_override, long long* stat_rows, cudaStream_t s) {
-  b2::finalize_level_kernel<<<1, b2::kCtlThreads, 0, s>>>(ctl_cur, ctl_nxt, seg_nxt, ev_nxt, split_work, counters,
-                                                         pair_parent_hist, hist_work, triples, max_pairs, need_hist, n_streams,
-                                                         window_rows, chunk_rows_override, stat_rows);
-  return (int)cudaGetLastError();
-}
 int b2_launch_leaf_plan(const B2LeafDev* leaves, const int32_t* n_leaves, B2SegWork* work, B2LevelCtl* leaf_ctl, cudaStream_t s) {
   b2::leaf_plan_kernel<<<1, b2::kCtlThreads, 0, s>>>(leaves, n_leaves, work, leaf_ctl);
   return (int)cudaGetLastError();
 }
 int b2_launch_leaf_values(const B2LeafDev* leaves, const int32_t* n_leaves, const long long* sums, const int32_t* qexp,
-                          int leaf_bits, B2CtlParams p, float* leaf_value, B2TreeDev tree, cudaStream_t s) {
-  b2::leaf_values_kernel<<<8, 256, 0, s>>>(leaves, n_leaves, sums, qexp, leaf_bits, p, leaf_value, tree);
+                          int leaf_bits, B2CtlParams p, float* leaf_value, B2TreeDev tree, int32_t* qexp_out, cudaStream_t s) {
+  b2::leaf_values_kernel<<<8, 256, 0, s>>>(leaves, n_leaves, sums, qexp, leaf_bits, p, leaf_value, tree, qexp_out);
   return (int)cudaGetLastError();
 }
 int b2_launch_tree_init(B2TreeDev tree, B2LevelCtl* ctl0, B2NodeSeg* seg0, B2EvalNode* ev0, int32_t* n_leaves, int n_rows,
@@ -301,8 +225,4 @@
   b2::tree_init_kernel<<<1, 32, 0, s>>>(tree, ctl0, seg0, ev0, n_leaves, n_rows, hist_work0);
   return (int)cudaGetLastError();
 }
-int b2_launch_root_record(B2TreeDev tree, const B2EvalNode* ev0, cudaStream_t s) {
-  b2::root_record_kernel<<<1, 32, 0, s>>>(tree, ev0);
-  return (int)cudaGetLastError();
-}
-}
+}
diff --git a/xgboost_ray_b200/csrc/engine.cu b/xgboost_ray_b200/csrc/engine.cu
--- a/xgboost_ray_b200/csrc/engine.cu
+++ b/xgboost_ray_b200/csrc/engine.cu
@@ -32,7 +32,7 @@
 int b2_launch_hist_subtract(const long long*, long long*, const int32_t*, int, int64_t, const B2LevelCtl*, cudaStream_t);
 int b2_launch_eval_splits(const long long*, int, const B2EvalNode*, int, const int32_t*, const int32_t*, const int32_t*,
                           const uint8_t*, const uint8_t*, const int32_t*, int, B2TrainParamDev, B2SplitCand*, int, const B2LevelCtl*,
-                          int, int, B2ColSample, const B2NodeSeg*, cudaStream_t);
+                          int, int, B2ColSample, const B2NodeSeg*, B2SiblingSub, cudaStream_t);
 int b2_launch_subsample(float2*, int64_t, uint32_t, uint32_t, uint32_t, double, int, cudaStream_t);
 int b2_p2p_flag_words(int);
 int b2_launch_p2p_reduce_subtract(const void*, const long long*, long long*, const int32_t*, const B2LevelCtl*, int, int, int64_t, int,
@@ -45,6 +45,8 @@
 int b2_launch_final_assign(const uint8_t*, int64_t, const int32_t*, const B2SplitWork*, const B2LevelCtl*, int, const float2*,
                            const int32_t*, int, long long*, uint16_t*, int, int, cudaStream_t);
 int b2_launch_margin_update(float*, int, int, const uint16_t*, const float*, int64_t, int, cudaStream_t);
+int b2_leaf_acc_max_depth();
+int b2_launch_leaf_accumulate(const float2*, const uint16_t*, int64_t, int, const int32_t*, int, long long*, int, cudaStream_t);
 int b2_gradient_fused_max_classes();
 int b2_launch_sum_fixed(const float2*, int64_t, const int32_t*, int, long long*, int, cudaStream_t);
 int b2_cat_ctas();
@@ -52,11 +54,12 @@
                               const int32_t*, int, B2TrainParamDev, B2SplitCand*, int, int, const B2LevelCtl*, int, int,
                               B2ColSample, const B2NodeSeg*, cudaStream_t);
 int b2_launch_cat_stats(const float*, int64_t, int, float, const int32_t*, int, int32_t*, int, cudaStream_t);
-int b2_launch_root_totals(const long long*, int, B2EvalNode*, const int32_t*, int, B2TrainParamDev, int, cudaStream_t);
+int b2_launch_root_totals(const long long*, int, B2EvalNode*, const int32_t*, int, B2TrainParamDev, int, long long*, long long*,
+                          cudaStream_t);
 int b2_part_chunk_rows();
 int b2_split_chunk_rows();
 int b2_launch_partition(const uint8_t*, int64_t, const int32_t*, int32_t*, const B2SplitWork*, const B2LevelCtl*, int, int32_t*,
-                        int, int, cudaStream_t);
+                        int, B2FinalizeArgs, int, cudaStream_t);
 int b2_launch_leaf_sums(const float2*, const int32_t*, const int32_t*, const void*, const B2LevelCtl*, int, const int32_t*, int,
                         long long*, uint16_t*, int, cudaStream_t);
 int b2_launch_pred_update(float*, int, int, const int32_t*, const int32_t*, const void*, const B2LevelCtl*, int, const float*, int,
@@ -64,13 +67,10 @@
 int b2_launch_decide(B2LevelCtl*, B2LevelCtl*, const B2NodeSeg*, B2NodeSeg*, const B2EvalNode*, B2EvalNode*, const B2SplitCand*,
                      int, int, int, int, B2TreeDev, B2SplitWork*, int32_t*, B2LeafDev*, int32_t*, const uint8_t*, const int32_t*, int,
                      B2CtlParams, int32_t*, const B2SplitCand*, const void*, cudaStream_t);
-int b2_launch_finalize_level(const B2LevelCtl*, B2LevelCtl*, B2NodeSeg*, B2EvalNode*, const B2SplitWork*, const int32_t*,
-                             const int32_t*, B2HistWork*, int32_t*, int, int, int, int, int, long long*, cudaStream_t);
 int b2_launch_leaf_plan(const B2LeafDev*, const int32_t*, B2SegWork*, B2LevelCtl*, cudaStream_t);
 int b2_launch_leaf_values(const B2LeafDev*, const int32_t*, const long long*, const int32_t*, int, B2CtlParams, float*, B2TreeDev,
-                          cudaStream_t);
+                          int32_t*, cudaStream_t);
 int b2_launch_tree_init(B2TreeDev, B2LevelCtl*, B2NodeSeg*, B2EvalNode*, int32_t*, int, B2HistWork*, cudaStream_t);
-int b2_launch_root_record(B2TreeDev, const B2EvalNode*, cudaStream_t);
 int b2_launch_iota(int32_t*, int64_t, cudaStream_t);
 int b2_launch_gradient(int, int, const float*, const float*, const float*, int64_t, float, float, float2*, uint32_t*, uint32_t*, int,
                        cudaStream_t);
@@ -732,7 +732,7 @@
   View<B2SplitCand> d_cands_all;
   int shards = 1, log2_shards = 0, sp = 32, cpn = 1;
   int cpn_num = 1;
-  DevBuf<uint32_t> t_cat;
+  View<uint32_t> t_cat;
   DevBuf<uint8_t> d_col_masks;
   struct P2PState {
     bool enabled = false, tried = false;
@@ -761,13 +761,16 @@
   size_t node_elems = 0;
   DevBuf<uint32_t> d_absmax; DevBuf<int32_t> d_qexp;
   int ctl_depth = 0;
-  DevBuf<int32_t> t_i32;
-  DevBuf<float> t_f32;
-  DevBuf<long long> t_i64;
+  DevBuf<uint8_t> t_block;
+  View<int32_t> t_i32;
+  View<float> t_f32;
+  View<long long> t_i64;
+  View<int32_t> t_qexp;
   DevBuf<B2LevelCtl> d_ctl;
   DevBuf<B2NodeSeg> d_seg[2]; DevBuf<B2EvalNode> d_ev[2];
   DevBuf<B2HistWork> d_hist_work; DevBuf<B2SplitWork> d_split_work; DevBuf<B2SegWork> d_seg_work;
   DevBuf<B2SplitCand> d_cands; DevBuf<int32_t> d_counters, d_triples, d_pair_parent;
+  DevBuf<uint32_t> d_part_done;
   DevBuf<B2LeafDev> d_leaves;
   DevBuf<long long> d_leaf_sums; DevBuf<float> d_leaf_values; DevBuf<double> d_metric;
   std::vector<void*> staging;
@@ -1038,12 +1041,15 @@
   b->ctl_depth = D;
   const TreeLayout L = tree_layout(D);
   const size_t lcap = (size_t)1 << D, half = (size_t)1 << (D > 0 ? D - 1 : 0);
-  b->t_i32.ensure(L.i32_count); b->t_f32.ensure(L.f32_count); b->t_i64.ensure(L.i64_count);
-  b->t_cat.ensure(b->train->any_cat() ? L.max_nodes * 8 : 8);
+  b->t_block.ensure(L.bytes);
+  b->t_i32.p = (int32_t*)b->t_block.p; b->t_f32.p = (float*)(b->t_block.p + L.off_f32);
+  b->t_i64.p = (long long*)(b->t_block.p + L.off_i64); b->t_qexp.p = (int32_t*)(b->t_block.p + L.off_qexp);
+  b->t_cat.p = (uint32_t*)(b->t_block.p + L.off_cat);
   b->d_ctl.ensure(3);
   for (int k = 0; k < 2; ++k) { b->d_seg[k].ensure(lcap); b->d_ev[k].ensure(lcap); }
   b->d_hist_work.ensure(half); b->d_split_work.ensure(half);
   b->d_counters.ensure(2 * half); b->d_triples.ensure(3 * half); b->d_pair_parent.ensure(half);
+  if (!b->d_part_done.p) { b->d_part_done.ensure(1); CUDA_CHECK(cudaMemsetAsync(b->d_part_done.p, 0, sizeof(uint32_t), b->ctx->stream)); }
   b->d_leaves.ensure(L.max_nodes); b->d_seg_work.ensure(L.max_nodes);
   b->d_leaf_sums.ensure(2 * lcap); b->d_leaf_values.ensure(lcap);
   b->node_elems = (size_t)G * B2_GROUP_ELEMS;
@@ -1143,6 +1149,8 @@
   const bool multi = b->comm && b->comm->world > 1;
   const bool p2p = multi && b->p2p.enabled;
   static const bool leaf_fused = env_flag("B2_LEAF_FUSED", true);
+  const bool leaf_stream = leaf_fused && D >= 1 && D <= b2_leaf_acc_max_depth();
+  const bool sub_in_scan = !p2p && !m->any_cat();
   mark_phase(b, -1);
   const uint32_t tree_index = (uint32_t)b->trees.size() + (uint32_t)slot;
   uint32_t* d_absmax = b->d_absmax.p + 2 * k;
@@ -1225,9 +1233,8 @@
   }
   mark_phase(b, 1);
   exchange_and_subtract(b, st, nullptr, b->hist[0].p, nullptr, nullptr, 1, 1);
-  LAUNCH_CHECK(b2_launch_root_totals(b->hist[0].p, G, b->d_ev[0].p, b->d_qexp.p, p.qbits, dp, sh, s));
-  LAUNCH_CHECK(b2_launch_root_record(tree, b->d_ev[0].p, s));
-  st.kernel_launches += 3;
+  LAUNCH_CHECK(b2_launch_root_totals(b->hist[0].p, G, b->d_ev[0].p, b->d_qexp.p, p.qbits, dp, sh, tree.sum_g, tree.sum_h, s));
+  st.kernel_launches += 2;
   int hb = 0;
   for (int d = 0; d <= D; ++d) {
     const int cur = d & 1, nxt = cur ^ 1;
@@ -1242,9 +1249,14 @@
       cs.fwq = m->fwq.empty() ? nullptr : m->d_fwq.p;
       cs.bynode = (double)p.colsample_bynode; cs.n_level = n_level_feats[d]; cs.n_features = m->F;
       cs.seed = (uint32_t)p.seed; cs.tree = p.use_cols() ? tree_index : 0u;
+      B2SiblingSub sub{nullptr, nullptr, nullptr, 0};
+      if (sub_in_scan && d > 0) {
+        sub.parent_level = b->hist[hb ^ 1].p; sub.triples = b->d_triples.p;
+        sub.sib_out = d + 1 < D ? b->hist[hb].p : nullptr; sub.sib_base = max_nodes_level / 2;
+      }
       LAUNCH_CHECK(b2_launch_eval_splits(b->hist[hb].p, G, b->d_ev[cur].p, max_nodes_level, m->d_group_first.p, m->d_group_size.p,
                                          m->d_nbins.p, m->d_has_missing.p, m->any_cat() ? m->d_is_cat.p : nullptr, b->d_qexp.p,
-                                         p.qbits, dp, b->d_cands.p, b->cpn, ctl + cur, sh, shard_rank, cs, b->d_seg[cur].p, s));
+                                         p.qbits, dp, b->d_cands.p, b->cpn, ctl + cur, sh, shard_rank, cs, b->d_seg[cur].p, sub, s));
       st.kernel_launches++;
       if (m->any_cat()) {
         LAUNCH_CHECK(b2_launch_eval_cat_splits(b->hist[hb].p, G, b->d_ev[cur].p, max_nodes_level, m->d_cat_feats.p,
@@ -1271,24 +1283,27 @@
     if (!can_split) break;
     const int32_t* ridx_in = d == 0 ? nullptr : b->ridx[cur].p;
     if (last_split_level && leaf_fused) {
+      long long* sums = leaf_stream ? nullptr : b->d_leaf_sums.p;
       LAUNCH_CHECK(b2_launch_leaf_plan(b->d_leaves.p, &ctl[cur].leaf_base_next, b->d_seg_work.p, ctl + 2, s));
       LAUNCH_CHECK(b2_launch_leaf_sums(gh, b->ridx[0].p, b->ridx[1].p, b->d_seg_work.p, ctl + 2, max_leaf_chunks, b->d_qexp.p, 40,
-                                       b->d_leaf_sums.p, b->pos.p, ctx->num_sms, s));
+                                       sums, b->pos.p, ctx->num_sms, s));
       LAUNCH_CHECK(b2_launch_final_assign(m->bins_col.p, m->col_stride, ridx_in, b->d_split_work.p, ctl + cur,
-                                          max_part_chunks_total + max_nodes_level, gh, b->d_qexp.p, 40, b->d_leaf_sums.p, b->pos.p,
+                                          max_part_chunks_total + max_nodes_level, gh, b->d_qexp.p, 40, sums, b->pos.p,
                                           m->any_cat() ? 1 : 0, ctx->num_sms, s));
       st.kernel_launches += 3;
       mark_phase(b, 5);
       continue;
     }
+    const bool need_hist = d + 1 < D;
+    B2FinalizeArgs fin;
+    fin.ctl_nxt = ctl + nxt; fin.seg_nxt = b->d_seg[nxt].p; fin.ev_nxt = b->d_ev[nxt].p; fin.pair_parent_hist = b->d_pair_parent.p;
+    fin.hist_work = b->d_hist_work.p; fin.triples = b->d_triples.p; fin.stat_rows = d_level_rows + d + 1; fin.done = b->d_part_done.p;
+    fin.max_pairs = max_nodes_level; fin.need_hist = need_hist ? 1 : 0; fin.n_streams = n_streams; fin.window_rows = window;
+    fin.chunk_rows_override = p.hist_chunk_rows;
     LAUNCH_CHECK(b2_launch_partition(m->bins_col.p, m->col_stride, ridx_in, b->ridx[nxt].p, b->d_split_work.p, ctl + cur,
-                                     max_part_chunks_total + max_nodes_level, b->d_counters.p, m->any_cat() ? 1 : 0,
+                                     max_part_chunks_total + max_nodes_level, b->d_counters.p, m->any_cat() ? 1 : 0, fin,
                                      ctx->num_sms, s));
-    const bool need_hist = d + 1 < D;
-    LAUNCH_CHECK(b2_launch_finalize_level(ctl + cur, ctl + nxt, b->d_seg[nxt].p, b->d_ev[nxt].p, b->d_split_work.p, b->d_counters.p,
-                                          b->d_pair_parent.p, b->d_hist_work.p, b->d_triples.p, max_nodes_level, need_hist ? 1 : 0,
-                                          n_streams, window, p.hist_chunk_rows, d_level_rows + d + 1, s));
-    st.kernel_launches += 2;
+    st.kernel_launches++;
     mark_phase(b, 5);
     if (need_hist) {
       const int nh = hb ^ 1;
@@ -1305,7 +1320,8 @@
       record_hist_launch(b, st, e0, e1, false);
       st.hist_launches++; st.kernel_launches++;
       mark_phase(b, 1);
-      exchange_and_subtract(b, st, b->hist[hb].p, b->hist[nh].p, b->d_triples.p, ctl + nxt, max_nodes_level, max_nodes_level);
+      exchange_and_subtract(b, st, b->hist[hb].p, b->hist[nh].p, sub_in_scan ? nullptr : b->d_triples.p, ctl + nxt,
+                            max_nodes_level, max_nodes_level);
       hb = nh;
     }
   }
@@ -1314,10 +1330,13 @@
     LAUNCH_CHECK(b2_launch_leaf_sums(gh, b->ridx[0].p, b->ridx[1].p, b->d_seg_work.p, ctl + 2, max_leaf_chunks, b->d_qexp.p, 40,
                                      b->d_leaf_sums.p, nullptr, ctx->num_sms, s));
     st.kernel_launches += 2;
+  } else if (leaf_stream) {
+    LAUNCH_CHECK(b2_launch_leaf_accumulate(gh, b->pos.p, n, D, b->d_qexp.p, 40, b->d_leaf_sums.p, ctx->num_sms, s));
+    st.kernel_launches++;
   }
   if (p2p) { LAUNCH_CHECK(b2_launch_p2p_leaf_sums(&b->p2p.pp, d_n_leaves, b->d_leaf_sums.p, s)); st.kernel_launches++; }
   else allreduce(b->comm, b->d_leaf_sums.p, 2 * lcap, kNcclInt64, kNcclSum, s);
-  LAUNCH_CHECK(b2_launch_leaf_values(b->d_leaves.p, d_n_leaves, b->d_leaf_sums.p, b->d_qexp.p, 40, cp, b->d_leaf_values.p, tree, s));
+  LAUNCH_CHECK(b2_launch_leaf_values(b->d_leaves.p, d_n_leaves, b->d_leaf_sums.p, b->d_qexp.p, 40, cp, b->d_leaf_values.p, tree, b->t_qexp.p, s));
   if (leaf_fused)
     LAUNCH_CHECK(b2_launch_margin_update(b->margin.p, K, k, b->pos.p, b->d_leaf_values.p, n, ctx->num_sms, s));
   else
@@ -1326,11 +1345,7 @@
   st.kernel_launches += 2;
   mark_phase(b, 6);
   char* stg = (char*)b->staging[slot];
-  CUDA_CHECK(cudaMemcpyAsync(stg, b->t_i32.p, L.i32_count * 4, cudaMemcpyDeviceToHost, s));
-  CUDA_CHECK(cudaMemcpyAsync(stg + L.off_f32, b->t_f32.p, L.f32_count * 4, cudaMemcpyDeviceToHost, s));
-  CUDA_CHECK(cudaMemcpyAsync(stg + L.off_i64, b->t_i64.p, L.i64_count * 8, cudaMemcpyDeviceToHost, s));
-  CUDA_CHECK(cudaMemcpyAsync(stg + L.off_qexp, b->d_qexp.p, 2 * sizeof(int32_t), cudaMemcpyDeviceToHost, s));
-  if (m->any_cat()) CUDA_CHECK(cudaMemcpyAsync(stg + L.off_cat, b->t_cat.p, L.max_nodes * 8 * sizeof(uint32_t), cudaMemcpyDeviceToHost, s));
+  CUDA_CHECK(cudaMemcpyAsync(stg, b->t_block.p, m->any_cat() ? L.bytes : L.off_cat, cudaMemcpyDeviceToHost, s));
 }
 
 void apply_tree_stats(Booster* b, long long hist_launches, long long kernel_launches, double allreduce_bytes,
diff --git a/xgboost_ray_b200/csrc/level_finalize.cuh b/xgboost_ray_b200/csrc/level_finalize.cuh
--- /dev/null
+++ b/xgboost_ray_b200/csrc/level_finalize.cuh
@@ -0,0 +1,85 @@
+#pragma once
+
+#include <cub/block/block_scan.cuh>
+
+#include "common.cuh"
+
+namespace b2 {
+
+template <int kThreads>
+struct FinalizeScratch {
+  typedef cub::BlockScan<int, kThreads> Scan;
+  typename Scan::TempStorage scan;
+  long long rows;
+  int chunk_rows;
+};
+
+template <int kThreads>
+__device__ void finalize_level_block(FinalizeScratch<kThreads>& sm, const B2LevelCtl* __restrict__ ctl_cur,
+                                     const B2SplitWork* __restrict__ split_work, const int32_t* counters,
+                                     const B2FinalizeArgs& a) {
+  typedef typename FinalizeScratch<kThreads>::Scan Scan;
+  B2LevelCtl* ctl_nxt = a.ctl_nxt; B2NodeSeg* seg_nxt = a.seg_nxt; B2EvalNode* ev_nxt = a.ev_nxt;
+  const int32_t* pair_parent_hist = a.pair_parent_hist; B2HistWork* hist_work = a.hist_work; int32_t* triples = a.triples;
+  const int max_pairs = a.max_pairs, need_hist = a.need_hist, n_streams = a.n_streams, window_rows = a.window_rows;
+  const int chunk_rows_override = a.chunk_rows_override;
+  long long* stat_rows = a.stat_rows;
+  const int ns = ctl_cur->n_split;
+  if (threadIdx.x == 0) sm.rows = 0;
+  __syncthreads();
+  long long my_rows = 0;
+  for (int j = threadIdx.x; j < ns; j += kThreads) {
+    const B2SplitWork sw = split_work[j];
+    const int cl = __ldcg(counters + 2 * j);
+    B2NodeSeg sl = seg_nxt[2 * j], sr = seg_nxt[2 * j + 1];
+    sl.begin = sw.seg_begin; sl.count = cl;
+    sr.begin = sw.seg_begin + cl; sr.count = sw.seg_count - cl;
+    seg_nxt[2 * j] = sl; seg_nxt[2 * j + 1] = sr;
+    if (need_hist) {
+      const bool build_left = ev_nxt[2 * j].sum_h < ev_nxt[2 * j + 1].sum_h;
+      my_rows += build_left ? sl.count : sr.count;
+    }
+  }
+  if (!need_hist) return;
+  atomicAdd((unsigned long long*)&sm.rows, (unsigned long long)my_rows);
+  __syncthreads();
+  if (threadIdx.x == 0) {
+    int c = chunk_rows_override;
+    if (c <= 0) {
+      const long long per_stream = sm.rows / n_streams;
+      const long long target = per_stream >= 16384 ? per_stream / 4 : per_stream;
+      c = 512;
+      while (c < target && c < 8192) c <<= 1;
+    }
+    if (c > window_rows) c = window_rows;
+    sm.chunk_rows = c;
+    if (stat_rows) *stat_rows = sm.rows;
+  }
+  __syncthreads();
+  const int chunk_rows = sm.chunk_rows;
+  int carry = 0;
+  for (int base = 0; base < ns; base += kThreads) {
+    const int j = base + threadIdx.x;
+    int chunks = 0, begin = 0, count = 0;
+    if (j < ns) {
+      const bool build_left = ev_nxt[2 * j].sum_h < ev_nxt[2 * j + 1].sum_h;
+      const int b = build_left ? 2 * j : 2 * j + 1, s = b ^ 1;
+      begin = seg_nxt[b].begin; count = seg_nxt[b].count;
+      chunks = (count + chunk_rows - 1) / chunk_rows;
+      ev_nxt[b].hist_index = j; ev_nxt[s].hist_index = max_pairs + j;
+      triples[3 * j] = pair_parent_hist[j]; triples[3 * j + 1] = j; triples[3 * j + 2] = max_pairs + j;
+    }
+    int ex, total;
+    Scan(sm.scan).ExclusiveSum(chunks, ex, total);
+    __syncthreads();
+    const int cb = carry + ex;
+    carry += total;
+    if (j < ns) { B2HistWork w; w.seg_begin = begin; w.seg_count = count; w.hist_index = j; w.chunk_begin = cb; hist_work[j] = w; }
+  }
+  if (threadIdx.x == 0) {
+    ctl_nxt->hist_n_work = ns; ctl_nxt->hist_total_chunks = carry; ctl_nxt->hist_chunk_rows = chunk_rows;
+    ctl_nxt->n_pairs = ns;
+  }
+}
+
+}
diff --git a/xgboost_ray_b200/csrc/partition_kernel.cu b/xgboost_ray_b200/csrc/partition_kernel.cu
--- a/xgboost_ray_b200/csrc/partition_kernel.cu
+++ b/xgboost_ray_b200/csrc/partition_kernel.cu
@@ -1,6 +1,7 @@
 #include <stdlib.h>
 
 #include "common.cuh"
+#include "level_finalize.cuh"
 
 namespace b2 {
 
@@ -16,7 +17,7 @@
 __global__ void __launch_bounds__(kPartThreads)
 partition_kernel(const uint8_t* __restrict__ bins_col, int64_t col_stride, const int32_t* __restrict__ ridx_in,
                  int32_t* __restrict__ ridx_out, const B2SplitWork* __restrict__ work, const B2LevelCtl* __restrict__ ctl,
-                 int32_t* __restrict__ counters ) {
+                 int32_t* counters , B2FinalizeArgs fin) {
   const int n_work = ctl->n_split, total_chunks = ctl->part_chunks;
   constexpr int kIters = kPartChunk / kPartThreads;
   constexpr int kWarps = kPartThreads / 32;
@@ -123,6 +124,18 @@
     }
     __syncthreads();
   }
+  __shared__ FinalizeScratch<kPartThreads> s_fin;
+  __shared__ bool s_last;
+  __syncthreads();
+  if (threadIdx.x == 0) {
+    __threadfence();
+    const unsigned prev = atomicAdd(fin.done, 1u);
+    s_last = prev == gridDim.x - 1;
+    if (s_last) { __threadfence(); *fin.done = 0u; }
+  }
+  __syncthreads();
+  if (!s_last) return;
+  finalize_level_block<kPartThreads>(s_fin, ctl, work, counters, fin);
 }
 
 __global__ void __launch_bounds__(256)
@@ -143,6 +156,11 @@
     const int32_t* ridx = w.pad0 ? nullptr : (w.buf ? ridx1 : ridx0);
     const int row0 = (chunk - w.chunk_begin) * kPartChunk;
     const int nrows = min(kPartChunk, w.seg_count - row0);
+    if (!sums) {
+      for (int r = threadIdx.x; r < nrows; r += blockDim.x)
+        pos[ridx ? __ldg(ridx + w.seg_begin + row0 + r) : (w.seg_begin + row0 + r)] = (uint16_t)w.id;
+      continue;
+    }
     long long ag = 0, ah = 0;
     for (int r = threadIdx.x; r < nrows; r += blockDim.x) {
       const int row = ridx ? __ldg(ridx + w.seg_begin + row0 + r) : (w.seg_begin + row0 + r);
@@ -188,7 +206,7 @@
   }
 }
 
-template <bool kCat, bool kRoot>
+template <bool kCat, bool kRoot, bool kSums>
 __global__ void __launch_bounds__(kPartThreads)
 final_assign_kernel(const uint8_t* __restrict__ bins_col, int64_t col_stride, const int32_t* __restrict__ ridx_in,
                     const B2SplitWork* __restrict__ work, const B2LevelCtl* __restrict__ ctl, const float2* __restrict__ gh,
@@ -196,7 +214,7 @@
                     uint16_t* __restrict__ pos) {
   const int n_work = ctl->n_split, total_chunks = ctl->part_chunks, leaf_base = ctl->leaf_base_next;
   __shared__ long long s_acc[kPartThreads / 32][4];
-  const double kg = ldexp(1.0, leaf_bits - qexp[0]), kh = ldexp(1.0, leaf_bits - qexp[1]);
+  const double kg = kSums ? ldexp(1.0, leaf_bits - qexp[0]) : 0.0, kh = kSums ? ldexp(1.0, leaf_bits - qexp[1]) : 0.0;
   const int lane = threadIdx.x & 31, warp = threadIdx.x >> 5;
   for (int chunk = blockIdx.x; chunk < total_chunks; chunk += gridDim.x) {
     int lo = 0, hi = n_work - 1;
@@ -210,7 +228,7 @@
     const bool is_cat = kCat && w.is_cat != 0;
     const int leaf_l = leaf_base + 2 * lo;
     long long lg = 0, lh = 0, rg = 0, rh = 0;
-    constexpr int kBatch = 4;
+    constexpr int kBatch = kSums ? 4 : 8;
     const uint8_t* col = bins_col + (int64_t)w.feature * col_stride;
     for (int r0 = threadIdx.x; r0 < nrows; r0 += kBatch * kPartThreads) {
       int rid[kBatch]; int bin[kBatch]; float2 v[kBatch];
@@ -220,7 +238,10 @@
         rid[k] = r < nrows ? (kRoot ? w.seg_begin + row0 + r : __ldg(ridx_in + w.seg_begin + row0 + r)) : -1;
       }
 #pragma unroll
-      for (int k = 0; k < kBatch; ++k) { bin[k] = (int)__ldg(col + (rid[k] < 0 ? 0 : rid[k])); v[k] = __ldg(gh + (rid[k] < 0 ? 0 : rid[k])); }
+      for (int k = 0; k < kBatch; ++k) {
+        bin[k] = (int)__ldg(col + (rid[k] < 0 ? 0 : rid[k]));
+        if (kSums) v[k] = __ldg(gh + (rid[k] < 0 ? 0 : rid[k]));
+      }
 #pragma unroll
       for (int k = 0; k < kBatch; ++k) {
         if (rid[k] < 0) continue;
@@ -228,11 +249,14 @@
         bool go_left = b <= w.split_bin;
         if (kCat && is_cat) go_left = ((__ldg(&work[lo].cat_bits[b >> 5]) >> (b & 31)) & 1u) == 0u;
         const bool l = (w.has_missing && b == B2_MISSING_BIN) ? (w.default_left != 0) : go_left;
-        const long long qg = __double2ll_rn(__dmul_rn((double)v[k].x, kg)), qh = __double2ll_rn(__dmul_rn((double)v[k].y, kh));
-        if (l) { lg += qg; lh += qh; } else { rg += qg; rh += qh; }
+        if (kSums) {
+          const long long qg = __double2ll_rn(__dmul_rn((double)v[k].x, kg)), qh = __double2ll_rn(__dmul_rn((double)v[k].y, kh));
+          if (l) { lg += qg; lh += qh; } else { rg += qg; rh += qh; }
+        }
         pos[rid[k]] = (uint16_t)(leaf_l + (l ? 0 : 1));
       }
     }
+    if (!kSums) continue;
 #pragma unroll
     for (int o = 16; o > 0; o >>= 1) {
       lg += __shfl_xor_sync(0xffffffffu, lg, o); lh += __shfl_xor_sync(0xffffffffu, lh, o);
@@ -256,6 +280,58 @@
     margin[i * K + k] += __ldg(leaf_value + pos[i]);
 }
 
+constexpr int kLeafAccThreads = 512;
+constexpr int kLeafAccMaxDepth = 11;
+constexpr int kLeafAccSmem = 32 * 1024;
+__device__ __forceinline__ void acc_add64(uint32_t* lo, uint32_t* hi, long long q) {
+  const uint32_t l = (uint32_t)(unsigned long long)q, h = (uint32_t)((unsigned long long)q >> 32);
+  const uint32_t old = atomicAdd(lo, l);
+  const uint32_t hadd = h + ((uint32_t)(old + l) < old ? 1u : 0u);
+  if (hadd != 0u) atomicAdd(hi, hadd);
+}
+__global__ void __launch_bounds__(kLeafAccThreads)
+leaf_accumulate_kernel(const float2* __restrict__ gh, const uint16_t* __restrict__ pos, int64_t n, int n_acc, int log2_copies,
+                       const int32_t* __restrict__ qexp, int leaf_bits, long long* __restrict__ sums ) {
+  extern __shared__ uint32_t s_acc[];
+  const int copies = 1 << log2_copies, plane = n_acc << log2_copies;
+  for (int i = threadIdx.x; i < 4 * plane; i += blockDim.x) s_acc[i] = 0u;
+  __syncthreads();
+  uint32_t *glo = s_acc, *ghi = s_acc + plane, *hlo = s_acc + 2 * plane, *hhi = s_acc + 3 * plane;
+  const int copy = threadIdx.x & (copies - 1);
+  const double kg = ldexp(1.0, leaf_bits - qexp[0]), kh = ldexp(1.0, leaf_bits - qexp[1]);
+  constexpr int kBatch = 4;
+  const int64_t stride = (int64_t)gridDim.x * blockDim.x;
+  int64_t i = (int64_t)blockIdx.x * blockDim.x + threadIdx.x;
+  for (; i + (kBatch - 1) * stride < n; i += kBatch * stride) {
+    int leaf[kBatch]; float2 v[kBatch];
+#pragma unroll
+    for (int b = 0; b < kBatch; ++b) { leaf[b] = pos[i + b * stride]; v[b] = __ldg(gh + i + b * stride); }
+#pragma unroll
+    for (int b = 0; b < kBatch; ++b) {
+      const int a = (leaf[b] << log2_copies) + copy;
+      acc_add64(glo + a, ghi + a, __double2ll_rn(__dmul_rn((double)v[b].x, kg)));
+      acc_add64(hlo + a, hhi + a, __double2ll_rn(__dmul_rn((double)v[b].y, kh)));
+    }
+  }
+  for (; i < n; i += stride) {
+    const int a = ((int)pos[i] << log2_copies) + copy;
+    const float2 v = __ldg(gh + i);
+    acc_add64(glo + a, ghi + a, __double2ll_rn(__dmul_rn((double)v.x, kg)));
+    acc_add64(hlo + a, hhi + a, __double2ll_rn(__dmul_rn((double)v.y, kh)));
+  }
+  __syncthreads();
+  for (int j = threadIdx.x; j < 2 * n_acc; j += blockDim.x) {
+    const uint32_t* lo = (j & 1) ? hlo : glo;
+    const uint32_t* hi = (j & 1) ? hhi : ghi;
+    unsigned long long t = 0ull;
+    for (int c = 0; c < copies; ++c) {
+      const int a = ((j >> 1) << log2_copies) + c;
+      t += ((unsigned long long)hi[a] << 32) | (unsigned long long)lo[a];
+    }
+    if (t != 0ull) atomicAdd((unsigned long long*)&sums[j], t);
+  }
+}
+
 __global__ void iota_kernel(int32_t* out, int64_t n) {
   for (int64_t i = (int64_t)blockIdx.x * blockDim.x + threadIdx.x; i < n; i += (int64_t)gridDim.x * blockDim.x) out[i] = (int32_t)i;
 }
@@ -268,13 +344,13 @@
 
 int b2_launch_partition(const uint8_t* bins_col, int64_t col_stride, const int32_t* ridx_in, int32_t* ridx_out,
                         const B2SplitWork* work, const B2LevelCtl* ctl, int max_chunks, int32_t* counters, int any_categorical,
-                        int num_sms, cudaStream_t stream) {
-  if (max_chunks <= 0) return 0;
+                        B2FinalizeArgs fin, int num_sms, cudaStream_t stream) {
+  if (max_chunks <= 0) max_chunks = 1;
   int grid = max_chunks < num_sms * 6 ? max_chunks : num_sms * 6;
 #define B2_PART_LAUNCH(MODE)                                                                                                  \
   do {                                                                                                                        \
-    if (ridx_in) b2::partition_kernel<MODE, false><<<grid, b2::kPartThreads, 0, stream>>>(bins_col, col_stride, ridx_in, ridx_out, work, ctl, counters); \
-    else b2::partition_kernel<MODE, true><<<grid, b2::kPartThreads, 0, stream>>>(bins_col, col_stride, ridx_in, ridx_out, work, ctl, counters);         \
+    if (ridx_in) b2::partition_kernel<MODE, false><<<grid, b2::kPartThreads, 0, stream>>>(bins_col, col_stride, ridx_in, ridx_out, work, ctl, counters, fin); \
+    else b2::partition_kernel<MODE, true><<<grid, b2::kPartThreads, 0, stream>>>(bins_col, col_stride, ridx_in, ridx_out, work, ctl, counters, fin);    \
   } while (0)
   if (any_categorical) B2_PART_LAUNCH(1);
   else B2_PART_LAUNCH(0);
@@ -294,10 +370,28 @@
                            long long* sums, uint16_t* pos, int any_categorical, int num_sms, cudaStream_t stream) {
   if (max_chunks <= 0) return 0;
   int grid = max_chunks < num_sms * 8 ? max_chunks : num_sms * 8;
-#define B2_FA_LAUNCH(CAT, ROOT) b2::final_assign_kernel<CAT, ROOT><<<grid, b2::kPartThreads, 0, stream>>>(bins_col, col_stride, ridx_in, work, ctl, gh, qexp, leaf_bits, sums, pos)
+#define B2_FA_LAUNCH(CAT, ROOT)                                                                                               \
+  do {                                                                                                                        \
+    if (sums) b2::final_assign_kernel<CAT, ROOT, true><<<grid, b2::kPartThreads, 0, stream>>>(bins_col, col_stride, ridx_in, work, ctl, gh, qexp, leaf_bits, sums, pos); \
+    else b2::final_assign_kernel<CAT, ROOT, false><<<grid, b2::kPartThreads, 0, stream>>>(bins_col, col_stride, ridx_in, work, ctl, gh, qexp, leaf_bits, sums, pos);    \
+  } while (0)
   if (any_categorical) { if (ridx_in) B2_FA_LAUNCH(true, false); else B2_FA_LAUNCH(true, true); }
   else { if (ridx_in) B2_FA_LAUNCH(false, false); else B2_FA_LAUNCH(false, true); }
 #undef B2_FA_LAUNCH
+  return (int)cudaGetLastError();
+}
+int b2_leaf_acc_max_depth() { return b2::kLeafAccMaxDepth; }
+int b2_launch_leaf_accumulate(const float2* gh, const uint16_t* pos, int64_t n, int max_depth, const int32_t* qexp, int leaf_bits,
+                              long long* sums, int num_sms, cudaStream_t stream) {
+  if (n <= 0) return 0;
+  if (max_depth > b2::kLeafAccMaxDepth) return (int)cudaErrorInvalidValue;
+  const int n_acc = 1 << max_depth;
+  int log2_copies = 0;
+  while (log2_copies < 3 && ((size_t)n_acc * 16 << (log2_copies + 1)) <= (size_t)b2::kLeafAccSmem) ++log2_copies;
+  const size_t smem = (size_t)n_acc * 16 << log2_copies;
+  const int64_t want = (n + b2::kLeafAccThreads - 1) / b2::kLeafAccThreads;
+  const int grid = (int)(want < (int64_t)num_sms * 2 ? want : (int64_t)num_sms * 2);
+  b2::leaf_accumulate_kernel<<<grid, b2::kLeafAccThreads, smem, stream>>>(gh, pos, n, n_acc, log2_copies, qexp, leaf_bits, sums);
   return (int)cudaGetLastError();
 }
 int b2_launch_margin_update(float* margin, int K, int k, const uint16_t* pos, const float* leaf_value, int64_t n, int num_sms,
diff --git a/xgboost_ray_b200/csrc/split_kernel.cu b/xgboost_ray_b200/csrc/split_kernel.cu
--- a/xgboost_ray_b200/csrc/split_kernel.cu
+++ b/xgboost_ray_b200/csrc/split_kernel.cu
@@ -31,7 +31,7 @@
                    const uint8_t* __restrict__ is_cat ,
                    const int32_t* __restrict__ qexp, int qbits, B2TrainParamDev p, B2SplitCand* __restrict__ cands,
                    int cand_stride, const B2LevelCtl* __restrict__ ctl, int log2_shards, int shard_rank, B2ColSample cs,
-                   const B2NodeSeg* __restrict__ seg) {
+                   const B2NodeSeg* __restrict__ seg, B2SiblingSub sub) {
   const int sp = B2_GROUP_SLOTS >> log2_shards;
   const int cpn = (n_groups * sp + 31) >> 5;
   const int node = blockIdx.x / cpn, cta_in_node = blockIdx.x % cpn;
@@ -47,8 +47,15 @@
   const int group = v_ok ? v / sp : 0, sl = v_ok ? v % sp : 0;
   const int slot = (sl << log2_shards) + shard_rank;
   const size_t slice_elems = (size_t)n_groups * 2 * B2_BINS * sp;
-  const long long* hg = level_hist + (size_t)nd.hist_index * slice_elems + (size_t)(group * 2) * B2_BINS * sp + sl;
+  const size_t in_slice = (size_t)(group * 2) * B2_BINS * sp + sl;
+  const bool fused = sub.parent_level != nullptr && nd.hist_index >= sub.sib_base;
+  const int pair = fused ? nd.hist_index - sub.sib_base : 0;
+  const long long* hg = level_hist + (size_t)(fused ? sub.triples[3 * pair + 1] : nd.hist_index) * slice_elems + in_slice;
   const long long* hh = hg + (size_t)B2_BINS * sp;
+  const long long* pgp = fused ? sub.parent_level + (size_t)sub.triples[3 * pair] * slice_elems + in_slice : nullptr;
+  const long long* php = fused ? pgp + (size_t)B2_BINS * sp : nullptr;
+  long long* sgp = (fused && sub.sib_out) ? sub.sib_out + (size_t)nd.hist_index * slice_elems + in_slice : nullptr;
+  long long* shp = sgp ? sgp + (size_t)B2_BINS * sp : nullptr;
   const int f = group_first[group] + slot;
   bool active = v_ok && slot < group_size[group] && !(is_cat && is_cat[f]);
   if (active && cs.level_mask) active = cs.level_mask[f] != 0;
@@ -64,7 +71,17 @@
   const bool fmiss = active ? (has_missing[f] != 0) : false;
 
   long long sg = 0, sh = 0;
-  if (active) {
+  if (fused) {
+    if (v_ok && (sgp || active)) {
+#pragma unroll
+      for (int i = 0; i < kEvalBinsPerChunk; ++i) {
+        const int b = q * kEvalBinsPerChunk + i;
+        const long long g = pgp[b * sp] - hg[b * sp], h = php[b * sp] - hh[b * sp];
+        if (sgp) { sgp[b * sp] = g; shp[b * sp] = h; }
+        if (active && b < nf) { sg += g; sh += h; }
+      }
+    }
+  } else if (active) {
 #pragma unroll
     for (int i = 0; i < kEvalBinsPerChunk; ++i) {
       int b = q * kEvalBinsPerChunk + i;
@@ -91,7 +108,9 @@
       const int b = q * kEvalBinsPerChunk + i;
       if (b >= nf) break;
       const long long eg_excl = pg, eh_excl = ph;
-      pg += hg[b * sp]; ph += hh[b * sp];
+      if (!fused) { pg += hg[b * sp]; ph += hh[b * sp]; }
+      else if (sgp) { pg += sgp[b * sp]; ph += shp[b * sp]; }
+      else { pg += pgp[b * sp] - hg[b * sp]; ph += php[b * sp] - hh[b * sp]; }
       {
         const double lh_d = __dmul_rn(__ll2double_rn(ph), p.inv_scale_h);
         if (lh_d >= p.min_child_weight) {
@@ -308,7 +327,8 @@
 }
 
 __global__ void root_totals_kernel(const long long* __restrict__ level_hist, int n_groups, B2EvalNode* nodes,
-                                   const int32_t* __restrict__ qexp, int qbits, B2TrainParamDev p, int log2_shards) {
+                                   const int32_t* __restrict__ qexp, int qbits, B2TrainParamDev p, int log2_shards,
+                                   long long* __restrict__ tree_sum_g, long long* __restrict__ tree_sum_h) {
   __shared__ long long sg[256], sh[256];
   const int sp = B2_GROUP_SLOTS >> log2_shards;
   const size_t slice_elems = (size_t)n_groups * 2 * B2_BINS * sp;
@@ -324,6 +344,7 @@
     p.inv_scale_g = ldexp(1.0, qexp[0] - qbits);
     p.inv_scale_h = ldexp(1.0, qexp[1] - qbits);
     nodes[0].sum_g = sg[0]; nodes[0].sum_h = sh[0];
+    tree_sum_g[0] = sg[0]; tree_sum_h[0] = sh[0];
     double G = __dmul_rn(__ll2double_rn(sg[0]), p.inv_scale_g), H = __dmul_rn(__ll2double_rn(sh[0]), p.inv_scale_h);
     nodes[0].root_gain = __double2float_rn(calc_gain(G, H, p));
   }
@@ -336,12 +357,12 @@
                           const int32_t* group_first, const int32_t* group_size, const int32_t* nbins,
                           const uint8_t* has_missing, const uint8_t* is_cat, const int32_t* qexp, int qbits, B2TrainParamDev p,
                           B2SplitCand* cands, int cand_stride, const B2LevelCtl* ctl, int log2_shards, int shard_rank,
-                          B2ColSample cs, const B2NodeSeg* seg, cudaStream_t stream) {
+                          B2ColSample cs, const B2NodeSeg* seg, B2SiblingSub sub, cudaStream_t stream) {
   if (n_nodes <= 0) return 0;
   const int sp = B2_GROUP_SLOTS >> log2_shards, cpn = (n_groups * sp + 31) >> 5;
   b2::eval_splits_kernel<<<n_nodes * cpn, 32 * b2::kEvalChunks, 0, stream>>>(level_hist, n_groups, nodes, group_first, group_size,
                                                                          nbins, has_missing, is_cat, qexp, qbits, p, cands,
-                                                                         cand_stride, ctl, log2_shards, shard_rank, cs, seg);
+                                                                         cand_stride, ctl, log2_shards, shard_rank, cs, seg, sub);
   return (int)cudaGetLastError();
 }
 int b2_cat_ctas() { return b2::kCatCtas; }
@@ -357,8 +378,9 @@
   return (int)cudaGetLastError();
 }
 int b2_launch_root_totals(const long long* level_hist, int n_groups, B2EvalNode* nodes, const int32_t* qexp, int qbits,
-                          B2TrainParamDev p, int log2_shards, cudaStream_t stream) {
-  b2::root_totals_kernel<<<1, 256, 0, stream>>>(level_hist, n_groups, nodes, qexp, qbits, p, log2_shards);
+                          B2TrainParamDev p, int log2_shards, long long* tree_sum_g, long long* tree_sum_h,
+                          cudaStream_t stream) {
+  b2::root_totals_kernel<<<1, 256, 0, stream>>>(level_hist, n_groups, nodes, qexp, qbits, p, log2_shards, tree_sum_g, tree_sum_h);
   return (int)cudaGetLastError();
 }
 }
```

Result: faster. 248.4, median of 6 (+8.0%).
